# baiyang4/D-LSG-Video-Caption

Hardware: AMD Instinct MI355X
Metric: clips/sec (train step, 26x(2048+4096) feats) (higher is better)
Workload: dtype f32; 1 GPU; vocab 1000, dropout on, tf eps 0.952, batch 64/GPU; MSVD-shaped 26x(2048+4096) + 16x2048 regions; train step; batch_per_gpu=64, global_batch=64, parallelism=dp1, launch=hipGraph replay, gemm_arithmetic=fp32

## Files before the change

d-lsg-video-caption_amd/csrc/rowops.hip:

```cpp
#include <type_traits>

#include "common.hpp"
#include "dlsg.h"
#include "wordpick.hpp"

using namespace dlsg;

namespace {

constexpr int LN_THREADS = 256;
constexpr int LN_MAXPT = 8;

struct RowLnPack { dlsg_rowln_args s[DLSG_ROWLN_MAXMULTI]; };
struct RowLnBwdPack { dlsg_rowln_bwd_args s[DLSG_ROWLN_MAXMULTI]; };

__global__ __launch_bounds__(LN_THREADS) void rowln_fwd_kernel(const RowLnPack pk) {
    __shared__ float red[16];
    const dlsg_rowln_args& a = pk.s[blockIdx.y];
    const int n = a.n;
    const uint64_t seed = a.seed + (a.seed_ptr ? *a.seed_ptr : 0ull);
    float gam[LN_MAXPT], bet[LN_MAXPT];
#pragma unroll
    for (int i = 0; i < LN_MAXPT; ++i) {
        const int j = threadIdx.x + i * LN_THREADS;
// ... 272 lines not shown
    const float* xp = x + o * n * inner + in;
    const float* mp = mask ? mask + o * n * inner + in : nullptr;
    float* yp = y + o * n * inner + in;
    float m = -INFINITY;
    for (int j = lane; j < n; j += 64) {
        float v = xp[(int64_t)j * inner];
        if (mp && !(mp[(int64_t)j * inner] > 0.f)) v = -9e15f;
        m = fmaxf(m, v);
    }
    m = wave_max(m);
    float s = 0.f;
    for (int j = lane; j < n; j += 64) {
        float v = xp[(int64_t)j * inner];
        if (mp && !(mp[(int64_t)j * inner] > 0.f)) v = -9e15f;
        s += __expf(v - m);
    }
    s = wave_sum(s);
    const float inv = 1.f / s;
    for (int j = lane; j < n; j += 64) {
        float v = xp[(int64_t)j * inner];
        if (mp && !(mp[(int64_t)j * inner] > 0.f)) v = -9e15f;
        yp[(int64_t)j * inner] = __expf(v - m) * inv;
    }
}

__global__ __launch_bounds__(256) void softmax_bwd_kernel(const float* __restrict__ y, const float* __restrict__ dy,
                                                          float* __restrict__ dx, int64_t outer, int n, int inner) {
    const int lane = threadIdx.x & 63;
    const int64_t line = (int64_t)blockIdx.x * 4 + (threadIdx.x >> 6);
    if (line >= outer * inner) return;
    const int64_t o = line / inner, in = line % inner;
    const int64_t base = o * n * inner + in;
    float s = 0.f;
    for (int j = lane; j < n; j += 64) s += y[base + (int64_t)j * inner] * dy[base + (int64_t)j * inner];
    s = wave_sum(s);
    for (int j = lane; j < n; j += 64) {
        const int64_t k = base + (int64_t)j * inner;
        dx[k] = y[k] * (dy[k] - s);
    }
}

struct PwFwdSet { dlsg_lstm_pw_args a[2]; };
struct PwBwdSet { dlsg_lstm_pw_bwd_args a[2]; };

__global__ __launch_bounds__(256) void lstm_pw_fwd_kernel(const PwFwdSet set) {
    const dlsg_lstm_pw_args& a = set.a[blockIdx.z];
    const int j = blockIdx.x * blockDim.x + threadIdx.x;
    const int b = blockIdx.y;
    if (j >= a.H) return;
    const int H = a.H;
    float pre[4] = {0.f, 0.f, 0.f, 0.f};
    const float* sp = a.slabs + (int64_t)b * 4 * H + j;
    int k = 0;
    for (; k + 2 <= a.nslab; k += 2) {
        float t[2][4];
#pragma unroll
        for (int u = 0; u < 2; ++u)
#pragma unroll
            for (int g = 0; g < 4; ++g) t[u][g] = sp[(k + u) * a.slab_stride + g * H];
#pragma unroll
        for (int u = 0; u < 2; ++u)
#pragma unroll
            for (int g = 0; g < 4; ++g) pre[g] += t[u][g];
    }
    if (k < a.nslab) {
#pragma unroll
        for (int g = 0; g < 4; ++g) pre[g] += sp[k * a.slab_stride + g * H];
    }
#pragma unroll
    for (int g = 0; g < 4; ++g) {
        const int col = g * H + j;
        float s = pre[g];
        if (a.addend) s += a.addend[(int64_t)b * a.ldadd + col];
        if (a.b_ih) s += a.b_ih[col];
        if (a.b_hh) s += a.b_hh[col];
        pre[g] = s;
    }
    const float ig = sigmoidf_(pre[0]), fg = sigmoidf_(pre[1]), gg = tanhf(pre[2]), og = sigmoidf_(pre[3]);
    const float cp = a.c_prev ? a.c_prev[(int64_t)b * a.ldcp + j] : 0.f;
    const float c = fg * cp + ig * gg;
    const float h = og * tanhf(c);
    a.c[(int64_t)b * a.ldc_ + j] = c;
    if (a.h) a.h[(int64_t)b * a.ldh + j] = h;
    if (a.h2) {
        float h2 = h;
        if (a.p > 0.f) h2 *= drop_scale(a.seed + (a.seed_ptr ? *a.seed_ptr : 0ull), a.site, (uint64_t)b * H + j, a.p);
        a.h2[(int64_t)b * a.ldh2 + j] = h2;
    }
    if (a.gates) {
        float* gp = a.gates + (int64_t)b * a.ldg;
        gp[j] = ig; gp[H + j] = fg; gp[2 * H + j] = gg; gp[3 * H + j] = og;
    }
}

__global__ __launch_bounds__(256) void lstm_pw_bwd_kernel(const PwBwdSet set) {
    const dlsg_lstm_pw_bwd_args& a = set.a[blockIdx.z];
    const int j = blockIdx.x * blockDim.x + threadIdx.x;
    const int b = blockIdx.y;
    if (j >= a.H) return;
    const int H = a.H;
    const float* gp = a.gates + (int64_t)b * a.ldg;
    const float ig = gp[j], fg = gp[H + j], gg = gp[2 * H + j], og = gp[3 * H + j];
    const float c = a.c[(int64_t)b * a.ldc_ + j];
    const float cp = a.c_prev ? a.c_prev[(int64_t)b * a.ldcp + j] : 0.f;
    float dh = a.dh ? a.dh[(int64_t)b * a.lddh + j] : 0.f;
    if (a.dh2 || a.dh3 || a.dh4) {
        float d2 = a.dh2 ? a.dh2[(int64_t)b * a.lddh2 + j] : 0.f;
        if (a.dh3) d2 += a.dh3[(int64_t)b * a.lddh3 + j];
        if (a.dh4) {
            const int ns4 = a.dh4_nslab > 1 ? a.dh4_nslab : 1;
            const float* hp = a.dh4 + (int64_t)b * a.lddh4 + j;
            int k = 0;
            for (; k + 4 <= ns4; k += 4) {
                const float t0 = hp[(int64_t)k * a.dh4_slab_stride], t1 = hp[(int64_t)(k + 1) * a.dh4_slab_stride],
                            t2 = hp[(int64_t)(k + 2) * a.dh4_slab_stride], t3 = hp[(int64_t)(k + 3) * a.dh4_slab_stride];
                d2 += t0; d2 += t1; d2 += t2; d2 += t3;
            }
            for (; k < ns4; ++k) d2 += hp[(int64_t)k * a.dh4_slab_stride];
        }
        if (a.p > 0.f) d2 *= drop_scale(a.seed + (a.seed_ptr ? *a.seed_ptr : 0ull), a.site, (uint64_t)b * H + j, a.p);
        dh += d2;
    }
    const float tc = tanhf(c);
    float dc = dh * og * (1.f - tc * tc);
    if (a.dc_next) dc += a.dc_next[(int64_t)b * a.lddcn + j];
    float* dgp = a.dgates + (int64_t)b * a.lddg;
    dgp[j] = dc * gg * ig * (1.f - ig);
    dgp[H + j] = dc * cp * fg * (1.f - fg);
    dgp[2 * H + j] = dc * ig * (1.f - gg * gg);
    dgp[3 * H + j] = dh * tc * og * (1.f - og);
    if (a.dc_prev) a.dc_prev[(int64_t)b * a.lddcp + j] = dc * fg;
}

__global__ void mean_rows_fwd_kernel(const float* __restrict__ x, float* __restrict__ out, int64_t ldo, int P, int H) {
    const int b = blockIdx.y;
    const int h = blockIdx.x * blockDim.x + threadIdx.x;
    if (h >= H) return;
    float s = 0.f;
    for (int p = 0; p < P; ++p) s += x[((int64_t)b * P + p) * H + h];
    out[(int64_t)b * ldo + h] = s / P;
}
__global__ void mean_rows_bwd_kernel(const float* __restrict__ dout, int64_t lddo, float* __restrict__ dx, int P, int H,
                                     int accum) {
    const int b = blockIdx.y;
    const int h = blockIdx.x * blockDim.x + threadIdx.x;
    if (h >= H) return;
    const float g = dout[(int64_t)b * lddo + h] / P;
    for (int p = 0; p < P; ++p) {
        float* d = dx + ((int64_t)b * P + p) * H + h;
        *d = accum ? *d + g : g;
    }
}

template <bool VEC>
__global__ __launch_bounds__(256) void rows_repeat_kernel(const float* __restrict__ x, float* __restrict__ y, int n, int64_t row,
                                                          int pieces) {
    const int64_t b = blockIdx.x / pieces;
    const int piece = blockIdx.x - (int)b * pieces;
    if constexpr (VEC) {
        const int64_t row4 = row >> 2;
        const int64_t j = (int64_t)piece * 256 + threadIdx.x;
        if (j >= row4) return;
        const f32x4 v = reinterpret_cast<const f32x4*>(x + b * row)[j];
        for (int i = 0; i < n; ++i) reinterpret_cast<f32x4*>(y + (b * n + i) * row)[j] = v;
    } else {
        const int64_t j = (int64_t)piece * 256 + threadIdx.x;
        if (j >= row) return;
        const float v = x[b * row + j];
        for (int i = 0; i < n; ++i) y[(b * n + i) * row + j] = v;
    }
}

template <bool VEC>
__global__ __launch_bounds__(256) void clip_fold_kernel(const float* __restrict__ dmem, const float* __restrict__ dg, int64_t lddg,
                                                        float* __restrict__ dx, int64_t total, int n, int P, int H, int accum) {
    constexpr int W = VEC ? 4 : 1;
    typedef typename std::conditional<VEC, f32x4, float>::type vec_t;
    const int64_t e = ((int64_t)blockIdx.x * 256 + threadIdx.x) * W;
    if (e >= total) return;
    const int64_t PH = (int64_t)P * H;
    const int64_t b = e / PH, ph = e - b * PH;
    const int h = (int)(ph % H);
    const float fP = (float)P;
    const float* m = dmem + b * n * PH + ph;
    const float* g = dg ? dg + b * n * lddg + h : nullptr;
    vec_t s;
    for (int i = 0; i < n; ++i) {
        vec_t t = *reinterpret_cast<const vec_t*>(m + i * PH);
        if (g) t += *reinterpret_cast<const vec_t*>(g + i * lddg) / fP;
        s = i ? s + t : t;
    }
    vec_t* d = reinterpret_cast<vec_t*>(dx + e);
    *d = accum ? *d + s : s;
}

__global__ void embed_fwd_kernel(const float* __restrict__ E, const int64_t* __restrict__ ids, float* __restrict__ out,
                                 int64_t ldo, int W, float p, uint64_t seed, uint32_t site, int64_t row0, const uint64_t* seed_ptr) {
    if (seed_ptr) seed += *seed_ptr;
    const int r = blockIdx.x;
    embed_row(E, ids[r], out, ldo, W, r, p, seed, site, row0, blockDim.x);
}
__global__ __launch_bounds__(1024) void embed_bwd_kernel(const float* __restrict__ dout, int64_t lddo, const int64_t* __restrict__ ids,
                                                         float* __restrict__ dE, int rows, int W, float p, uint64_t seed, uint32_t site,
                                                         int64_t row0, const uint64_t* seed_ptr) {
    if (seed_ptr) seed += *seed_ptr;
    const int r = blockIdx.x, lane = threadIdx.x & 63, wv = threadIdx.x >> 6, nwv = blockDim.x >> 6;
    const int64_t id = ids[r];
    for (int base = 0; base < r; base += 512) {
        int64_t v[8];
#pragma unroll
        for (int u = 0; u < 8; ++u) {
            const int i = base + 64 * u + lane;
            v[u] = (i < r) ? ids[i] : -1;
        }
        bool hit = false;
#pragma unroll
        for (int u = 0; u < 8; ++u) hit = hit || (v[u] == id);
        if (__ballot(hit)) return;
    }
    for (int c0 = 64 * wv; c0 < W; c0 += 64 * nwv) {
        const int j = c0 + lane;
        float acc = 0.f;
        for (int base = r; base < rows; base += 512) {
            int64_t v[8];
#pragma unroll
            for (int u = 0; u < 8; ++u) {
                const int i = base + 64 * u + lane;
                v[u] = (i < rows) ? ids[i] : -1;
            }
#pragma unroll
            for (int u = 0; u < 8; ++u) {
                unsigned long long m = __ballot(v[u] == id);
                while (m) {
                    int rr[8];
#pragma unroll
                    for (int x = 0; x < 8; ++x) {
                        rr[x] = m ? base + 64 * u + (__ffsll((long long)m) - 1) : -1;
                        m &= m - 1;
                    }
                    float g[8];
#pragma unroll
                    for (int x = 0; x < 8; ++x) g[x] = (rr[x] >= 0 && j < W) ? dout[(int64_t)rr[x] * lddo + j] : 0.f;
#pragma unroll
                    for (int x = 0; x < 8; ++x)
                        if (rr[x] >= 0 && j < W) {
                            float gv = g[x];
                            if (p > 0.f) gv *= drop_scale(seed, site, (uint64_t)(row0 + rr[x]) * W + j, p);
                            acc += gv;
                        }
                }
            }
        }
        if (j < W) dE[id * W + j] += acc;
    }
}

__global__ void copy2d_kernel(const float* __restrict__ src, int64_t lds_, float* __restrict__ dst, int64_t ldd, int rows,
                              int n, int accum) {
    const int64_t total = (int64_t)rows * n;
    for (int64_t i = (int64_t)blockIdx.x * blockDim.x + threadIdx.x; i < total; i += (int64_t)gridDim.x * blockDim.x) {
        const int64_t r = i / n;
        const int j = (int)(i - r * n);
        const float v = src[r * lds_ + j];
        float* d = dst + r * ldd + j;
        *d = accum ? *d + v : v;
    }
}
__global__ void dropout_kernel(const float* __restrict__ x, int64_t ldx, float* __restrict__ y, int64_t ldy, int rows, int n,
                               float p, uint64_t seed, uint32_t site, const uint64_t* seed_ptr) {
    if (seed_ptr) seed += *seed_ptr;
    const int64_t total = (int64_t)rows * n;
    for (int64_t i = (int64_t)blockIdx.x * blockDim.x + threadIdx.x; i < total; i += (int64_t)gridDim.x * blockDim.x) {
        const int64_t r = i / n;
        const int j = (int)(i - r * n);
        y[r * ldy + j] = x[r * ldx + j] * drop_scale(seed, site, (uint64_t)i, p);
    }
}
__global__ void permute_tb_kernel(const float* __restrict__ src, float* __restrict__ dst, int T, int B, int n) {
    const int64_t total = (int64_t)T * B * n;
    for (int64_t i = (int64_t)blockIdx.x * blockDim.x + threadIdx.x; i < total; i += (int64_t)gridDim.x * blockDim.x) {
        const int j = (int)(i % n);
        const int64_t rb = i / n;
        const int t = (int)(rb % T), b = (int)(rb / T);
        dst[i] = src[((int64_t)t * B + b) * n + j];
    }
}
template <bool VEC>
__global__ __launch_bounds__(256) void gather_rows_kernel(const float* __restrict__ src, int64_t lds_, const int64_t* __restrict__ idx,
                                                          float* __restrict__ dst, int64_t ldd, int n) {
    const int pieces = (n + 4095) >> 12;
    const int r = blockIdx.x / pieces, piece = blockIdx.x - r * pieces;
    const float* s = src + idx[r] * lds_;
    float* d = dst + (int64_t)r * ldd;
    if constexpr (VEC) {
        const int n4 = n >> 2;
        const int base = piece * 1024 + threadIdx.x;
        typedef float f4 __attribute__((ext_vector_type(4)));
        f4 v[4];
#pragma unroll
        for (int u = 0; u < 4; ++u)
            if (base + u * 256 < n4) v[u] = __builtin_nontemporal_load(reinterpret_cast<const f4*>(s) + base + u * 256);
#pragma unroll
        for (int u = 0; u < 4; ++u)
            if (base + u * 256 < n4) reinterpret_cast<f4*>(d)[base + u * 256] = v[u];
    } else {
        const int hi = min(n, (piece + 1) * 4096);
        for (int j = piece * 4096 + threadIdx.x; j < hi; j += 256) d[j] = s[j];
    }
}
__global__ void fill_kernel(float* __restrict__ dst, int64_t n, float v) {
    for (int64_t i = (int64_t)blockIdx.x * blockDim.x + threadIdx.x; i < n; i += (int64_t)gridDim.x * blockDim.x) dst[i] = v;
}

template <bool WEIGHTED>
__global__ __launch_bounds__(256) void ce_ragged_kernel(const float* __restrict__ logits, const int64_t* __restrict__ targets,
                                                        const int64_t* __restrict__ lens, const float* __restrict__ weights,
                                                        float* __restrict__ dlogits, float* __restrict__ row_loss, int B, int L,
                                                        int V, int tm) {
    __shared__ float red[16];
    const int row = blockIdx.x;
    const int b = tm ? row % B : row / L, t = tm ? row / B : row % L;
    const float* x = logits + (int64_t)row * V;
    float* dx = dlogits + (int64_t)row * V;
    int64_t len = lens[b];
    if (len > L) len = L;
    if (t >= len) {
        for (int j = threadIdx.x; j < V; j += blockDim.x) dx[j] = 0.f;
        if (threadIdx.x == 0) row_loss[row] = 0.f;
        return;
    }
    int64_t ntot = 0;
    for (int i = 0; i < B; ++i) ntot += (lens[i] > L ? L : lens[i]);
    float m = -INFINITY;
    for (int j = threadIdx.x; j < V; j += blockDim.x) m = fmaxf(m, x[j]);
    m = block_max(m, red);
    float s = 0.f;
    for (int j = threadIdx.x; j < V; j += blockDim.x) s += __expf(x[j] - m);
    s = block_sum(s, red);
    const int64_t tgt = targets[(int64_t)b * L + t];
    const bool bad = tgt < 0 || tgt >= V;
    const float inv = bad ? NAN : 1.f / s;
    float invn = 1.f / (float)ntot;
    if constexpr (WEIGHTED) invn = weights[b] * invn;
    for (int j = threadIdx.x; j < V; j += blockDim.x) {
        float p = __expf(x[j] - m) * inv;
        if (j == tgt) p -= 1.f;
        dx[j] = p * invn;
    }
    if (threadIdx.x == 0) row_loss[row] = bad ? NAN : (logf(s) + m - x[tgt]) * invn;
}
__global__ __launch_bounds__(256) void sum_to_scalar_kernel(const float* __restrict__ v, int n, float* __restrict__ out) {
    __shared__ float red[16];
    float s = 0.f;
    for (int i = threadIdx.x; i < n; i += blockDim.x) s += v[i];
    s = block_sum(s, red);
    if (threadIdx.x == 0) out[0] = s;
}

__global__ __launch_bounds__(256) void log_softmax_kernel(const float* __restrict__ logits, float* __restrict__ out, int V) {
    __shared__ float red[16];
    const float* x = logits + (int64_t)blockIdx.x * V;
    float* y = out + (int64_t)blockIdx.x * V;
    float m = -INFINITY;
    for (int j = threadIdx.x; j < V; j += blockDim.x) m = fmaxf(m, x[j]);
    m = block_max(m, red);
    float s = 0.f;
    for (int j = threadIdx.x; j < V; j += blockDim.x) s += expf(x[j] - m);
    s = block_sum(s, red);
    const float lse = logf(s) + m;
    for (int j = threadIdx.x; j < V; j += blockDim.x) y[j] = x[j] - lse;
}

__global__ void gather_rows_multi_kernel(const dlsg_gather_multi_args a) {
    const int i = blockIdx.y, r = blockIdx.x;
    const int n = a.n[i];
    const float* s = a.src[i] + a.rows[r] * (int64_t)n;
    float* d = a.dst[i] + (int64_t)r * n;
    if ((n & 3) == 0) {
        for (int j = threadIdx.x * 4; j < n; j += blockDim.x * 4)
            *reinterpret_cast<f32x4*>(d + j) = *reinterpret_cast<const f32x4*>(s + j);
    } else {
        for (int j = threadIdx.x; j < n; j += blockDim.x) d[j] = s[j];
    }
}

template <bool CLIP>
__device__ __forceinline__ void adam_one(float& p, float g, float& m, float& v, float lr_bc1, float b1, float b2, float eps,
                                         float bc2s, float gscale, float coef, float clipv) {
    float gi = g * gscale;
    if (CLIP) {
        gi *= coef;
        if (clipv > 0.f) gi = fminf(fmaxf(gi, -clipv), clipv);
    }
    m = b1 * m + (1.f - b1) * gi;
    v = b2 * v + (1.f - b2) * gi * gi;
    const float denom = sqrtf(v) / bc2s + eps;
    p -= lr_bc1 * (m / denom);
}
template <int NTM, bool CLIP>
__global__ __launch_bounds__(256) void adam_kernel(float* __restrict__ p, const float* __restrict__ g, float* __restrict__ m,
                                                   float* __restrict__ v, int64_t n, float lr, float b1, float b2, float eps,
                                                   float bc1, float bc2s, float gscale, const float* __restrict__ hyper,
                                                   const int32_t* __restrict__ guard, const float* __restrict__ record, float clipv) {
    if (guard && *guard != 0) return;
    float coef = 1.f;
    if (CLIP && record) {
        if (record[DLSG_CLIP_NONFINITE] != 0.f) return;
        coef = record[DLSG_CLIP_COEF];
    }
    if (hyper) { lr = hyper[0]; bc1 = 1.f; bc2s = hyper[1]; }
    const float lr_bc1 = lr / bc1;
    const int64_t tid = (int64_t)blockIdx.x * blockDim.x + threadIdx.x, nth = (int64_t)gridDim.x * blockDim.x;
    const bool same = ((reinterpret_cast<uintptr_t>(p) ^ reinterpret_cast<uintptr_t>(g)) & 15) == 0 &&
                      ((reinterpret_cast<uintptr_t>(p) ^ reinterpret_cast<uintptr_t>(m)) & 15) == 0 &&
                      ((reinterpret_cast<uintptr_t>(p) ^ reinterpret_cast<uintptr_t>(v)) & 15) == 0;
    int64_t head = same ? (int64_t)((16 - (reinterpret_cast<uintptr_t>(p) & 15)) & 15) / 4 : n;
    if (head > n) head = n;
    const int64_t nv = (n - head) / 4;
    for (int64_t i = tid; i < head; i += nth) adam_one<CLIP>(p[i], g[i], m[i], v[i], lr_bc1, b1, b2, eps, bc2s, gscale, coef, clipv);
    f32x4* p4 = reinterpret_cast<f32x4*>(p + head);
    const f32x4* g4 = reinterpret_cast<const f32x4*>(g + head);
    f32x4* m4 = reinterpret_cast<f32x4*>(m + head);
    f32x4* v4 = reinterpret_cast<f32x4*>(v + head);
    for (int64_t i = tid; i < nv; i += nth) {
        f32x4 pp, mm, vv, gg;
        if (NTM & 4) pp = __builtin_nontemporal_load(p4 + i); else pp = p4[i];
        if (NTM & 1) { mm = __builtin_nontemporal_load(m4 + i); vv = __builtin_nontemporal_load(v4 + i); gg = __builtin_nontemporal_load(g4 + i); }
        else { mm = m4[i]; vv = v4[i]; gg = g4[i]; }
#pragma unroll
        for (int e = 0; e < 4; ++e) {
            float pe = pp[e], me = mm[e], ve = vv[e];
            adam_one<CLIP>(pe, gg[e], me, ve, lr_bc1, b1, b2, eps, bc2s, gscale, coef, clipv);
            pp[e] = pe; mm[e] = me; vv[e] = ve;
        }
        if (NTM & 2) { __builtin_nontemporal_store(mm, m4 + i); __builtin_nontemporal_store(vv, v4 + i); }
        else { m4[i] = mm; v4[i] = vv; }
        if (NTM & 8) __builtin_nontemporal_store(pp, p4 + i); else p4[i] = pp;
    }
    for (int64_t i = head + 4 * nv + tid; i < n; i += nth) adam_one<CLIP>(p[i], g[i], m[i], v[i], lr_bc1, b1, b2, eps, bc2s, gscale, coef, clipv);
}

__global__ __launch_bounds__(256) void grad_sumsq_kernel(const float* __restrict__ g, int64_t n, double* __restrict__ slots) {
    __shared__ double red[4];
    const int64_t tid = (int64_t)blockIdx.x * blockDim.x + threadIdx.x, nth = (int64_t)gridDim.x * blockDim.x;
    int64_t head = (int64_t)((16 - (reinterpret_cast<uintptr_t>(g) & 15)) & 15) / 4;
    if (head > n) head = n;
    const int64_t nv = (n - head) / 4;
    double a0 = 0.0, a1 = 0.0, a2 = 0.0, a3 = 0.0;
    for (int64_t i = tid; i < head; i += nth) { const double x = g[i]; a0 += x * x; }
    const f32x4* g4 = reinterpret_cast<const f32x4*>(g + head);
#pragma unroll 4
    for (int64_t i = tid; i < nv; i += nth) {
        const f32x4 gg = g4[i];
        const double x0 = gg[0], x1 = gg[1], x2 = gg[2], x3 = gg[3];
        a0 += x0 * x0; a1 += x1 * x1; a2 += x2 * x2; a3 += x3 * x3;
    }
    for (int64_t i = head + 4 * nv + tid; i < n; i += nth) { const double x = g[i]; a0 += x * x; }
    const double s = block256_sum_f64((a0 + a1) + (a2 + a3), red);
    if (threadIdx.x == 0) slots[blockIdx.x] = s;
}
__global__ __launch_bounds__(256) void clip_coef_kernel(const double* __restrict__ slots, int count, float gscale, float max_norm,
                                                       float* __restrict__ record, int64_t* __restrict__ skipped) {
    __shared__ double red[4];
    double a = 0.0;
// ... 28 lines not shown
    }
    if (a->rows == 0) return DLSG_OK;
    int grid = a->rows < 4096 ? a->rows : 4096;
    hipLaunchKernelGGL(rowln_fwd_kernel, dim3(grid, count), dim3(LN_THREADS), 0, ST(stream), pk);
    DLSG_CHECK_LAUNCH();
    return DLSG_OK;
}
extern "C" int dlsg_rowln_fwd(const dlsg_rowln_args* a, void* stream) { return dlsg_rowln_fwd_multi(a, 1, stream); }
extern "C" int dlsg_rowln_bwd_nblk(int rows) {
    if (rows < 1) return 1;
    if (rows <= 256) return rows;
    if (rows <= 4096) return (rows + 1) / 2 < 1024 ? (rows + 1) / 2 : 1024;
    return 1024;
}
extern "C" int dlsg_rowln_bwd_multi(const dlsg_rowln_bwd_args* a, int count, void* stream) {
    if (!a || count < 1 || count > DLSG_ROWLN_MAXMULTI) return DLSG_EINVAL;
    const int grid = dlsg_rowln_bwd_nblk(a->f.rows);
    RowLnBwdPack pk;
    for (int i = 0; i < count; ++i) {
        if (a[i].f.n < 1 || a[i].f.n > LN_THREADS * LN_MAXPT || a[i].f.rows != a[0].f.rows) return DLSG_EINVAL;
        if (a[i].dgb_part && a[i].nblk != grid) return DLSG_EINVAL;
        pk.s[i] = a[i];
    }
    if (a->f.rows == 0) return DLSG_OK;
    hipLaunchKernelGGL(rowln_bwd_kernel, dim3(grid, count), dim3(LN_THREADS), 0, ST(stream), pk);
    DLSG_CHECK_LAUNCH();
    return DLSG_OK;
}
extern "C" int dlsg_rowln_bwd(const dlsg_rowln_bwd_args* a, void* stream) { return dlsg_rowln_bwd_multi(a, 1, stream); }
static int colsum_chunks(int rows) {
    if (rows < 4096) return 1;
    const int chunks = (rows + 1023) / 1024;
    return chunks > 32 ? 32 : chunks;
}
static int colsum_launch(const float* part, int64_t ld, int rows, int n, float* out, float* out2, int split, int mode, int accum,
                         float* ws, void* stream) {
    if (!part || !out || n < 1) return DLSG_EINVAL;
    const int chunks = colsum_chunks(rows);
    const int rpc = (rows + chunks - 1) / chunks;
    const bool v4 = n % 4 == 0 && ld % 4 == 0 && (reinterpret_cast<uintptr_t>(part) & 15) == 0;
    if (chunks > 1 && ws && (v4 || !out2)) {
        if (v4) hipLaunchKernelGGL(colsum_v4_kernel, dim3((n + 63) / 64, chunks), dim3(1024), 0, ST(stream), part, ld, rows, n, out,
                                   out2, out2 ? split : n, out2 ? mode : 0, accum, rpc, ws);
        else hipLaunchKernelGGL(colsum_kernel, dim3((n + 63) / 64, chunks), dim3(1024), 0, ST(stream), part, ld, rows, n, out, accum,
                                rpc, ws);
        hipLaunchKernelGGL(colsum_finish_kernel, dim3((n + 255) / 256), dim3(256), 0, ST(stream), ws, chunks, n, out, out2,
                           out2 ? split : n, out2 ? mode : 0, accum);
        DLSG_CHECK_LAUNCH();
        return DLSG_OK;
    }
    if (chunks > 1 && !accum) {
        const int n0 = (out2 && mode == 0) ? split : n;
        hipLaunchKernelGGL(fill_kernel, dim3(1), dim3(256), 0, ST(stream), out, (int64_t)n0, 0.f);
        if (out2) hipLaunchKernelGGL(fill_kernel, dim3(1), dim3(256), 0, ST(stream), out2, (int64_t)(mode == 0 ? n - split : n), 0.f);
    }
    float* none = nullptr;
    if (v4) {
        hipLaunchKernelGGL(colsum_v4_kernel, dim3((n + 63) / 64, chunks), dim3(1024), 0, ST(stream), part, ld, rows, n, out,
                           out2, out2 ? split : n, out2 ? mode : 0, accum, rpc, none);
    } else if (!out2) {
        hipLaunchKernelGGL(colsum_kernel, dim3((n + 63) / 64, chunks), dim3(1024), 0, ST(stream), part, ld, rows, n, out, accum, rpc, none);
    } else if (mode == 0) {
        hipLaunchKernelGGL(colsum_kernel, dim3((split + 63) / 64, chunks), dim3(1024), 0, ST(stream), part, ld, rows, split, out,
                           accum, rpc, none);
        hipLaunchKernelGGL(colsum_kernel, dim3((n - split + 63) / 64, chunks), dim3(1024), 0, ST(stream), part + split, ld, rows,
                           n - split, out2, accum, rpc, none);
    } else {
        hipLaunchKernelGGL(colsum_kernel, dim3((n + 63) / 64, chunks), dim3(1024), 0, ST(stream), part, ld, rows, n, out, accum, rpc, none);
        hipLaunchKernelGGL(colsum_kernel, dim3((n + 63) / 64, chunks), dim3(1024), 0, ST(stream), part, ld, rows, n, out2, accum, rpc, none);
    }
    DLSG_CHECK_LAUNCH();
    return DLSG_OK;
}
extern "C" int dlsg_colsum_multi_ok(const float* part, int64_t ld, int rows, int n) {
    return (colsum_chunks(rows) == 1 && n % 4 == 0 && ld % 4 == 0 && (reinterpret_cast<uintptr_t>(part) & 15) == 0) ? 1 : 0;
}
extern "C" int dlsg_colsum_multi(const dlsg_colsum_desc* d, int count, void* stream) {
    if (!d || count < 1 || count > DLSG_COLSUM_MAXMULTI) return DLSG_EINVAL;
    ColsumPack pk;
    int maxn = 0;
    for (int i = 0; i < count; ++i) {
        if (!d[i].part || !d[i].out_a || d[i].n < 1 || d[i].rows < 0) return DLSG_EINVAL;
        if (!dlsg_colsum_multi_ok(d[i].part, d[i].ld, d[i].rows, d[i].n)) return DLSG_EALIGN;
        if (d[i].out_b && !d[i].dup && (d[i].split < 0 || d[i].split > d[i].n)) return DLSG_EINVAL;
        pk.d[i] = d[i];
        maxn = d[i].n > maxn ? d[i].n : maxn;
    }
    hipLaunchKernelGGL(colsum_multi_kernel, dim3((maxn + 63) / 64, count), dim3(1024), 0, ST(stream), pk);
    DLSG_CHECK_LAUNCH();
    return DLSG_OK;
}
extern "C" int64_t dlsg_colsum_ws_floats(int rows, int n) {
    const int chunks = colsum_chunks(rows);
    return chunks > 1 ? (int64_t)chunks * n : 0;
}
extern "C" int dlsg_colsum(const float* part, int64_t ld, int rows, int n, float* out, int accum, float* ws, void* stream) {
    return colsum_launch(part, ld, rows, n, out, nullptr, n, 0, accum, ws, stream);
}
extern "C" int dlsg_colsum2(const float* part, int64_t ld, int rows, int n, float* out_a, float* out_b, int split, int dup,
                            int accum, float* ws, void* stream) {
    if (!out_b || (!dup && (split < 0 || split > n))) return DLSG_EINVAL;
    return colsum_launch(part, ld, rows, n, out_a, out_b, dup ? n : split, dup ? 1 : 0, accum, ws, stream);
}
extern "C" int dlsg_softmax_fwd(const float* x, const float* mask, float* y, int64_t outer, int n, int inner, void* stream) {
    const int64_t lines = outer * inner;
    if (lines == 0) return DLSG_OK;
    hipLaunchKernelGGL(softmax_fwd_kernel, dim3((unsigned)((lines + 3) / 4)), dim3(256), 0, ST(stream), x, mask, y, outer, n,
                       inner);
    DLSG_CHECK_LAUNCH();
    return DLSG_OK;
}
extern "C" int dlsg_softmax_bwd(const float* y, const float* dy, float* dx, int64_t outer, int n, int inner, void* stream) {
    const int64_t lines = outer * inner;
    if (lines == 0) return DLSG_OK;
    hipLaunchKernelGGL(softmax_bwd_kernel, dim3((unsigned)((lines + 3) / 4)), dim3(256), 0, ST(stream), y, dy, dx, outer, n,
                       inner);
    DLSG_CHECK_LAUNCH();
    return DLSG_OK;
}
extern "C" int dlsg_lstm_pw_fwd_n(const dlsg_lstm_pw_args* a, int count, void* stream) {
    if (!a || count < 1 || count > 2 || a[0].H < 1) return DLSG_EINVAL;
    if (count == 2 && (a[1].H != a[0].H || a[1].B != a[0].B)) return DLSG_EINVAL;
    if (a[0].B == 0) return DLSG_OK;
    PwFwdSet set;
    for (int i = 0; i < 2; ++i) set.a[i] = a[i < count ? i : 0];
    hipLaunchKernelGGL(lstm_pw_fwd_kernel, dim3((a[0].H + 255) / 256, a[0].B, count), dim3(256), 0, ST(stream), set);
    DLSG_CHECK_LAUNCH();
    return DLSG_OK;
}
extern "C" int dlsg_lstm_pw_fwd(const dlsg_lstm_pw_args* a, void* stream) { return dlsg_lstm_pw_fwd_n(a, 1, stream); }
extern "C" int dlsg_lstm_pw_bwd_n(const dlsg_lstm_pw_bwd_args* a, int count, void* stream) {
    if (!a || count < 1 || count > 2 || a[0].H < 1) return DLSG_EINVAL;
    if (count == 2 && (a[1].H != a[0].H || a[1].B != a[0].B)) return DLSG_EINVAL;
    if (a[0].B == 0) return DLSG_OK;
    PwBwdSet set;
    for (int i = 0; i < 2; ++i) set.a[i] = a[i < count ? i : 0];
    hipLaunchKernelGGL(lstm_pw_bwd_kernel, dim3((a[0].H + 255) / 256, a[0].B, count), dim3(256), 0, ST(stream), set);
    DLSG_CHECK_LAUNCH();
    return DLSG_OK;
}
extern "C" int dlsg_lstm_pw_bwd(const dlsg_lstm_pw_bwd_args* a, void* stream) { return dlsg_lstm_pw_bwd_n(a, 1, stream); }
extern "C" int dlsg_mean_rows_fwd(const float* x, float* out, int64_t ldo, int B, int P, int H, void* stream) {
    if (B == 0) return DLSG_OK;
    hipLaunchKernelGGL(mean_rows_fwd_kernel, dim3((H + 255) / 256, B), dim3(256), 0, ST(stream), x, out, ldo, P, H);
    DLSG_CHECK_LAUNCH();
    return DLSG_OK;
}
extern "C" int dlsg_mean_rows_bwd(const float* dout, int64_t lddo, float* dx, int B, int P, int H, int accum, void* stream) {
    if (B == 0) return DLSG_OK;
    hipLaunchKernelGGL(mean_rows_bwd_kernel, dim3((H + 255) / 256, B), dim3(256), 0, ST(stream), dout, lddo, dx, P, H, accum);
    DLSG_CHECK_LAUNCH();
    return DLSG_OK;
}
extern "C" int dlsg_rows_repeat(const float* x, float* y, int B, int n, int64_t row, void* stream) {
    if (B < 0 || n < 1 || row < 0) return DLSG_EINVAL;
    if (B == 0 || row == 0) return DLSG_OK;
    if (!x || !y) return DLSG_EINVAL;
    const bool vec = row % 4 == 0 && ((uintptr_t)x | (uintptr_t)y) % 16 == 0;
    const int64_t pieces = ((vec ? row >> 2 : row) + 255) / 256;
    if (pieces * B > 0x7fffffff) return DLSG_EINVAL;
    const dim3 grid((unsigned)(pieces * B));
    if (vec) hipLaunchKernelGGL(rows_repeat_kernel<true>, grid, dim3(256), 0, ST(stream), x, y, n, row, (int)pieces);
    else hipLaunchKernelGGL(rows_repeat_kernel<false>, grid, dim3(256), 0, ST(stream), x, y, n, row, (int)pieces);
    DLSG_CHECK_LAUNCH();
    return DLSG_OK;
}
extern "C" int dlsg_clip_fold(const float* dmem, const float* dg, int64_t lddg, float* dx, int B, int n, int P, int H, int accum,
                              void* stream) {
    if (B < 0 || n < 1 || P < 1 || H < 1 || (dg && lddg < H)) return DLSG_EINVAL;
    if (B == 0) return DLSG_OK;
    if (!dmem || !dx) return DLSG_EINVAL;
    const int64_t total = (int64_t)B * P * H;
    const bool vec = H % 4 == 0 && ((uintptr_t)dmem | (uintptr_t)dx) % 16 == 0 && (!dg || (lddg % 4 == 0 && (uintptr_t)dg % 16 == 0));
    const int64_t blocks = ((vec ? total >> 2 : total) + 255) / 256;
    if (blocks > 0x7fffffff) return DLSG_EINVAL;
    if (vec) hipLaunchKernelGGL(clip_fold_kernel<true>, dim3((unsigned)blocks), dim3(256), 0, ST(stream), dmem, dg, lddg, dx, total, n, P, H, accum);
    else hipLaunchKernelGGL(clip_fold_kernel<false>, dim3((unsigned)blocks), dim3(256), 0, ST(stream), dmem, dg, lddg, dx, total, n, P, H, accum);
    DLSG_CHECK_LAUNCH();
    return DLSG_OK;
}
extern "C" int dlsg_embed_fwd(const float* E, const int64_t* ids, float* out, int64_t ldo, int rows, int W, float p,
                              uint64_t seed, uint32_t site, int64_t row0, const uint64_t* seed_ptr, void* stream) {
    if (rows == 0) return DLSG_OK;
    hipLaunchKernelGGL(embed_fwd_kernel, dim3(rows), dim3(128), 0, ST(stream), E, ids, out, ldo, W, p, seed, site, row0, seed_ptr);
    DLSG_CHECK_LAUNCH();
    return DLSG_OK;
}
extern "C" int dlsg_embed_bwd(const float* dout, int64_t lddo, const int64_t* ids, float* dE, int rows, int W, float p,
                              uint64_t seed, uint32_t site, int64_t row0, const uint64_t* seed_ptr, void* stream) {
    if (rows == 0) return DLSG_OK;
    const int threads = W >= 1024 ? 1024 : (W + 63) / 64 * 64;
    hipLaunchKernelGGL(embed_bwd_kernel, dim3(rows), dim3(threads), 0, ST(stream), dout, lddo, ids, dE, rows, W, p, seed, site, row0,
                       seed_ptr);
    DLSG_CHECK_LAUNCH();
    return DLSG_OK;
}
extern "C" int dlsg_copy2d(const float* src, int64_t lds_, float* dst, int64_t ldd, int rows, int n, int accum, void* stream) {
    if ((int64_t)rows * n == 0) return DLSG_OK;
    hipLaunchKernelGGL(copy2d_kernel, dim3(grid_for((int64_t)rows * n)), dim3(256), 0, ST(stream), src, lds_, dst, ldd, rows, n,
                       accum);
    DLSG_CHECK_LAUNCH();
    return DLSG_OK;
}
extern "C" int dlsg_dropout(const float* x, int64_t ldx, float* y, int64_t ldy, int rows, int n, float p, uint64_t seed,
                            uint32_t site, const uint64_t* seed_ptr, void* stream) {
    if ((int64_t)rows * n == 0) return DLSG_OK;
    hipLaunchKernelGGL(dropout_kernel, dim3(grid_for((int64_t)rows * n)), dim3(256), 0, ST(stream), x, ldx, y, ldy, rows, n, p,
                       seed, site, seed_ptr);
    DLSG_CHECK_LAUNCH();
    return DLSG_OK;
}
extern "C" int dlsg_gather_rows(const float* src, int64_t lds_, const int64_t* idx, float* dst, int64_t ldd, int rows, int n,
                                void* stream) {
    if (rows == 0 || n == 0) return DLSG_OK;
    const bool vec = n % 4 == 0 && lds_ % 4 == 0 && ldd % 4 == 0 && ((uintptr_t)src | (uintptr_t)dst) % 16 == 0;
    const dim3 grid((unsigned)((int64_t)((n + 4095) / 4096) * rows));
    if (vec) hipLaunchKernelGGL(gather_rows_kernel<true>, grid, dim3(256), 0, ST(stream), src, lds_, idx, dst, ldd, n);
    else hipLaunchKernelGGL(gather_rows_kernel<false>, grid, dim3(256), 0, ST(stream), src, lds_, idx, dst, ldd, n);
    DLSG_CHECK_LAUNCH();
    return DLSG_OK;
}
extern "C" int dlsg_fill(float* dst, int64_t n, float value, void* stream) {
    if (n == 0) return DLSG_OK;
    hipLaunchKernelGGL(fill_kernel, dim3(grid_for(n)), dim3(256), 0, ST(stream), dst, n, value);
    DLSG_CHECK_LAUNCH();
    return DLSG_OK;
}
extern "C" int dlsg_permute_tb(const float* src, float* dst, int T, int B, int n, void* stream) {
    const int64_t total = (int64_t)T * B * n;
    if (total == 0) return DLSG_OK;
    hipLaunchKernelGGL(permute_tb_kernel, dim3(grid_for(total)), dim3(256), 0, ST(stream), src, dst, T, B, n);
    DLSG_CHECK_LAUNCH();
    return DLSG_OK;
}
extern "C" int dlsg_ce_ragged(const float* logits, const int64_t* targets, const int64_t* lens, float* dlogits, float* row_loss,
                              float* loss, int B, int L, int V, int time_major, void* stream) {
    if (B * L == 0) return DLSG_OK;
    hipLaunchKernelGGL(ce_ragged_kernel<false>, dim3(B * L), dim3(256), 0, ST(stream), logits, targets, lens, nullptr, dlogits, row_loss,
                       B, L, V, time_major);
    hipLaunchKernelGGL(sum_to_scalar_kernel, dim3(1), dim3(256), 0, ST(stream), row_loss, B * L, loss);
    DLSG_CHECK_LAUNCH();
    return DLSG_OK;
}
extern "C" int dlsg_ce_ragged_weighted(const float* logits, const int64_t* targets, const int64_t* lens, const float* weights,
                                       float* dlogits, float* row_loss, float* loss, int B, int L, int V, int time_major, void* stream) {
    if (B * L == 0) return DLSG_OK;
    if (!weights) return DLSG_EINVAL;
    hipLaunchKernelGGL(ce_ragged_kernel<true>, dim3(B * L), dim3(256), 0, ST(stream), logits, targets, lens, weights, dlogits, row_loss,
                       B, L, V, time_major);
    hipLaunchKernelGGL(sum_to_scalar_kernel, dim3(1), dim3(256), 0, ST(stream), row_loss, B * L, loss);
    DLSG_CHECK_LAUNCH();
    return DLSG_OK;
}
extern "C" int dlsg_log_softmax(const float* logits, float* out, int rows, int V, void* stream) {
    if (rows == 0) return DLSG_OK;
    hipLaunchKernelGGL(log_softmax_kernel, dim3(rows), dim3(256), 0, ST(stream), logits, out, V);
    DLSG_CHECK_LAUNCH();
    return DLSG_OK;
}
extern "C" int dlsg_gather_rows_multi(const dlsg_gather_multi_args* a, void* stream) {
    if (!a || a->count < 1 || a->count > 4) return DLSG_EINVAL;
    if (a->nrows == 0) return DLSG_OK;
    hipLaunchKernelGGL(gather_rows_multi_kernel, dim3(a->nrows, a->count), dim3(256), 0, ST(stream), *a);
    DLSG_CHECK_LAUNCH();
    return DLSG_OK;
}
extern "C" int dlsg_adam(float* p, const float* g, float* m, float* v, int64_t n, float lr, float b1, float b2, float eps,
                         int step, float grad_scale, const float* hyper, const int32_t* guard, void* stream) {
    if (n == 0) return DLSG_OK;
    const float bc1 = 1.f - powf(b1, (float)step);
    const float bc2s = sqrtf(1.f - powf(b2, (float)step));
    hipLaunchKernelGGL((adam_kernel<3, false>), dim3(grid_for((n + 3) / 4, 256, 8192)), dim3(256), 0, ST(stream), p, g, m, v, n, lr, b1, b2,
                       eps, bc1, bc2s, grad_scale, hyper, guard, (const float*)nullptr, 0.f);
    DLSG_CHECK_LAUNCH();
    return DLSG_OK;
}
extern "C" int dlsg_grad_sumsq(const float* g, int64_t n, double* slots, void* stream) {
    if (n < 0 || (!g && n > 0) || !slots) return DLSG_EINVAL;
    if (reinterpret_cast<uintptr_t>(g) & 3) return DLSG_EALIGN;
    hipLaunchKernelGGL(grad_sumsq_kernel, dim3(DLSG_GRAD_SUMSQ_SLOTS), dim3(256), 0, ST(stream), g, n, slots);
    DLSG_CHECK_LAUNCH();
    return DLSG_OK;
}
extern "C" int dlsg_clip_coef(const double* slots, int count, float grad_scale, float max_norm, float* record, int64_t* skipped,
                              void* stream) {
    if (!slots || count < 1 || !record || !(max_norm >= 0.f)) return DLSG_EINVAL;
    hipLaunchKernelGGL(clip_coef_kernel, dim3(1), dim3(256), 0, ST(stream), slots, count, grad_scale, max_norm, record, skipped);
    DLSG_CHECK_LAUNCH();
    return DLSG_OK;
}
extern "C" int dlsg_adam_clipped(float* p, const float* g, float* m, float* v, int64_t n, float lr, float b1, float b2, float eps,
                                 int step, float grad_scale, const float* hyper, const int32_t* guard, const float* record,
                                 float clip_value, void* stream) {
    if (!(clip_value >= 0.f)) return DLSG_EINVAL;
    if (n == 0) return DLSG_OK;
    const float bc1 = 1.f - powf(b1, (float)step);
    const float bc2s = sqrtf(1.f - powf(b2, (float)step));
    hipLaunchKernelGGL((adam_kernel<3, true>), dim3(grid_for((n + 3) / 4, 256, 8192)), dim3(256), 0, ST(stream), p, g, m, v, n, lr, b1, b2,
                       eps, bc1, bc2s, grad_scale, hyper, guard, record, clip_value);
    DLSG_CHECK_LAUNCH();
    return DLSG_OK;
}
```

d-lsg-video-caption_amd/dlsg_amd/engine.py:

```python
import math

import torch

from .hip import GEMM_NT, GEMM_NN, GEMM_TN, F_ACCUM, F_TANH, F_BF16X3, F_FORCE128, SAMPLE_FILTER_MAXV

V_SK = 7

SITE_PSL_OBJ, SITE_PSL_MOT, SITE_LSTM, SITE_PE, SITE_SA, SITE_WORD, SITE_QUERY, SITE_ATT1, SITE_ATT2, SITE_LANG = range(1, 11)
STEP_SITE = 64
SITE_SAMPLE = 11
SAMPLE_FILTER_MAXL = 64


def _empty(ref, *shape, dtype=torch.float32):
    return torch.empty(*shape, dtype=dtype, device=ref.device)


def _zeros(ref, *shape, dtype=torch.float32):
    return torch.zeros(*shape, dtype=dtype, device=ref.device)


def _ksplit_bounds(K, nsplit, align=32):
    nsplit = max(1, min(nsplit, K // 512))
    step = ((K + nsplit - 1) // nsplit + align - 1) // align * align
    out, k = [], 0
    while k < K:
        out.append((k, min(K, k + step)))
        k += step
    return out


SKINNY_M = 128


def _bwd_bounds(K, M, nsplit):
    if M <= SKINNY_M and K >= 2048:
        return [(k, min(K, k + 1024)) for k in range(0, K, 1024)]
    return _ksplit_bounds(K, nsplit, 128 if M <= SKINNY_M else 32)


def _nsplit_for(M, N, nseg, target=384, cap=16):
    tiles = (1 if M <= SKINNY_M else (M + 63) // 64) * ((N + 63) // 64)
    n = max(1, target // max(1, tiles * nseg))
    return max(1, min(n, cap // max(1, nseg)))


def seg_gemm_nt(ops, segs, M, N, ref):
    ns = 1 if M <= SKINNY_M else _nsplit_for(M, N, len(segs))
    groups = []
    for x, W in segs:
        for k0, k1 in _ksplit_bounds(x.shape[1], ns, 128 if M <= SKINNY_M else 32):
            groups.append((x[:, k0:k1], W[:, k0:k1]))
    slabs = _empty(ref, len(groups), M, N)
    ops.gemm(GEMM_NT, [(a, b, slabs[i]) for i, (a, b) in enumerate(groups)])
    return slabs


def gemm_nn_split(ops, dy, W, out, ref, accum=False):
    M, Nn = dy.shape
    Kin = W.shape[1]
    ns = _nsplit_for(M, Kin, 1)
    bounds = _ksplit_bounds(Nn, ns, 128 if M <= SKINNY_M else 32)
    if len(bounds) == 1:
        ops.gemm(GEMM_NN, [(dy, W, out)], flags=F_ACCUM if accum else 0)
        return
    slabs = _empty(ref, len(bounds), M, Kin)
    ops.gemm(GEMM_NN, [(dy[:, k0:k1], W[k0:k1, :], slabs[i]) for i, (k0, k1) in enumerate(bounds)])
    ops.slab_reduce(slabs, out, flags=F_ACCUM if accum else 0)


DEEP_TN_CHUNKS = 8


def _accum_flag(ops, gout):
    seen = getattr(ops, 'grad_written', None)
    if seen is None:
        return F_ACCUM
    key = (gout.data_ptr(), tuple(gout.shape), tuple(gout.stride()))
    if key in seen:
        return F_ACCUM
    seen.add(key)
    return 0


def _accum_always(ops, gout):
    seen = getattr(ops, 'grad_written', None)
    if seen is not None:
        seen.add((gout.data_ptr(), tuple(gout.shape), tuple(gout.stride())))
    return F_ACCUM


def gemm_tn_deep(ops, items, ref):
    deep = [it for it in items if it[0].shape[0] >= 8192]
    for dy, x, gout in items:
        if dy.shape[0] < 8192:
            ops.gemm(GEMM_TN, [(dy, x, gout)], flags=_accum_flag(ops, gout))
    if deep and getattr(ops, 'stream_k', False) and all(ops.gemm(GEMM_TN, [it], flags=F_ACCUM, plan_only=True) == V_SK for it in deep):
        parts = {0: [], F_ACCUM: []}
        for it in deep:
            parts[_accum_flag(ops, it[2])].append(it)
        for fl, part in parts.items():
            for i0 in range(0, len(part), 16):
                ops.gemm(GEMM_TN, part[i0:i0 + 16], flags=fl)
        return
    by_shape = {}
    for it in deep:
        by_shape.setdefault((it[0].shape, it[1].shape), []).append(it)
    ks = DEEP_TN_CHUNKS
    per_launch = max(1, min(2, 16 // ks))
    for grp in by_shape.values():
        for i0 in range(0, len(grp), per_launch):
            part = grp[i0:i0 + per_launch]
            rows = part[0][0].shape[0]
            step = ((rows + ks - 1) // ks + 31) // 32 * 32
            bounds = [(k, min(rows, k + step)) for k in range(0, rows, step)]
            assert len(bounds) * len(part) <= 16
            slabs = [_empty(ref, len(bounds), gout.shape[0], gout.shape[1]) for _, _, gout in part]
            ops.gemm(GEMM_TN, [(dy[k0:k1], x[k0:k1], sl[i]) for (dy, x, _), sl in zip(part, slabs)
                               for i, (k0, k1) in enumerate(bounds)])
            for (_, _, gout), sl in zip(part, slabs):
                ops.slab_reduce(sl, gout, flags=_accum_always(ops, gout))


def _accum_flag_peek(ops, gout):
    seen = getattr(ops, 'grad_written', None)
    if seen is None or (gout.data_ptr(), tuple(gout.shape), tuple(gout.stride())) in seen:
        return F_ACCUM
    return 0


def gemm_nn_multi(ops, dy, Ws, out, ref):
    M, Nn = dy.shape
    widths = [W.shape[1] for W in Ws]
    tot = sum(widths)
    assert out.shape[1] == tot
    ns = _nsplit_for(M, tot, 1)
    ns = max(1, min(ns, 16 // len(Ws)))
    bounds = _bwd_bounds(Nn, M, ns)
    slabs = _empty(ref, len(bounds), M, tot)
    groups, c0 = [], 0
    for W, wd in zip(Ws, widths):
        for i, (k0, k1) in enumerate(bounds):
            groups.append((dy[:, k0:k1], W[k0:k1, :], slabs[i][:, c0:c0 + wd]))
        c0 += wd
    ops.gemm(GEMM_NN, groups)
    ops.slab_reduce(slabs, out)


def gemm_nn_multi_slabs(ops, dy, Ws, width, ref):
    M, Nn = dy.shape
    widths = [W.shape[1] for W in Ws]
    tot = sum(widths)
    assert tot <= width
    ns = _nsplit_for(M, tot, 1)
    ns = max(1, min(ns, 16 // len(Ws)))
    bounds = _bwd_bounds(Nn, M, ns)
    if M <= SKINNY_M and len(set(widths)) > 1:
        wmin = min(widths)
        if all(wd % wmin == 0 for wd in widths) and (tot // wmin) * len(bounds) <= 16:
            Ws = [W[:, c:c + wmin] for W, wd in zip(Ws, widths) for c in range(0, wd, wmin)]
            widths = [wmin] * len(Ws)
    slabs = _empty(ref, len(bounds), M, width)
    groups, c0 = [], 0
    for W, wd in zip(Ws, widths):
        for i, (k0, k1) in enumerate(bounds):
            groups.append((dy[:, k0:k1], W[k0:k1, :], slabs[i][:, c0:c0 + wd]))
        c0 += wd
    ops.gemm(GEMM_NN, groups)
    return slabs


def tn_grouped(ops, items, defer=None):
    if defer is not None:
        defer.extend(items)
        return
    by_m = {}
    for dy, x, gout in items:
        by_m.setdefault((dy.shape[1], dy.shape[0]), []).append((dy, x, gout))
    for grp in by_m.values():
        waves, seen = [[]], [set()]
        for it in grp:
            key = (it[2].data_ptr(), tuple(it[2].shape))
            for w_, sn in zip(waves, seen):
                if key not in sn and len(w_) < 16:
                    w_.append(it); sn.add(key)
                    break
            else:
                waves.append([it]); seen.append({key})
        for w_ in waves:
            first = [it for it in w_ if _accum_flag_peek(ops, it[2]) == 0]
            rest = [it for it in w_ if _accum_flag_peek(ops, it[2]) != 0]
            for it in first:
                _accum_flag(ops, it[2])
            if first:
                ops.gemm(GEMM_TN, first, flags=0)
            if rest:
                ops.gemm(GEMM_TN, rest, flags=F_ACCUM)


def gemm_bucketed(ops, mode, groups, flags=0):
    by_m = {}
    for g in groups:
        by_m.setdefault(g[2].shape[-2], []).append(g)
    for grp in by_m.values():
        for i in range(0, len(grp), 16):
            ops.gemm(mode, grp[i:i + 16], flags=flags)


def lin(ops, x, W, out, bias=None, tanh=False, accum=False, skip_if=None):
    ops.gemm(GEMM_NT, [(x, W, out)], flags=(F_TANH if tanh else 0) | (F_ACCUM if accum else 0), bias=bias, skip_if=skip_if)


class Grads(object):

    def __init__(self, named_params, arena, offsets):
        self.arena, self.offsets = arena, offsets
        self.views = {}
        for name, p in named_params:
            o = offsets[name]
            self.views[name] = arena[o:o + p.numel()].view(p.shape)

    def __getitem__(self, name):
        return self.views[name]


def ln_grads(ops, part, G, prefix, n):
    p2 = part.view(-1, 2 * n)
    ops.colsum2(p2, G[prefix + '.weight'], G[prefix + '.bias'], split=n, accum=True)


def region_projections(ops, mods, regions):
    B, T, O, R = regions.shape
    rows = B * T * O
    r2 = regions.view(rows, R)
# ... 424 lines not shown
    so = _empty(ref, B * T, H)
    lin(ops, att, sa.output_layer[0].weight, so)
    psa = sa.dropout if training else 0.0
    if psa > 0:
        ops.dropout(so, so, psa, seed, SITE_SA)
    res = _empty(ref, B * T, H); st_s = _empty(ref, B * T, 2)
    ops.rowln_fwd(so, m.layernorm_sa.weight, m.layernorm_sa.bias, res, st_s)
    s.update(x=x, st_l=st_l, Kp=Kp, Qp=Qp, Vp=Vp, w=w, att=att, so=so, st_s=st_s, scale=scale, psa=psa, pe=pe)
    return res


def _bilstm_steps_bwd(ops, gates, cst, dout3, Whh, dG, B, T, H, ref):
    dcrec = [_empty(ref, B, H), _empty(ref, B, H)]
    ns_r = max(1, min(_nsplit_for(B, 2 * H, 1), 8))
    rb = _bwd_bounds(4 * H, B, ns_r)
    slabs = None
    for step in range(T - 1, -1, -1):
        tt = [step, T - 1 - step]
        tp = [step - 1, T - step]
        last = step == T - 1
        ops.lstm_pw_bwd_multi([dict(gates=gates[d][:, tt[d]], c=cst[d][:, tt[d]], dgates=dG[d][:, tt[d]], B=B, H=H,
                                    c_prev=cst[d][:, tp[d]] if step > 0 else None,
                                    dh=dout3[:, tt[d], d * H:(d + 1) * H],
                                    dh4=None if last else slabs[:, :, d * H:(d + 1) * H],
                                    dc_next=None if last else dcrec[d], dc_prev=dcrec[d]) for d in range(2)])
        if step > 0:
            slabs = _empty(ref, len(rb), B, 2 * H)
            groups = []
            for d in range(2):
                dg = dG[d][:, tt[d]]
                for i, (k0, k1) in enumerate(rb):
                    groups.append((dg[:, k0:k1], Whh[d][k0:k1, :], slabs[i][:, d * H:(d + 1) * H]))
            ops.gemm(GEMM_NN, groups)


def encvis_bwd(ops, m, pfx, frames2d, B, T, sv, G, dres, training, seed):
    H = m.hidden_size
    ref = frames2d
    s = sv[pfx]
    name = pfx
    ln = m.layernorm_lstm
    out2 = s['out']
    D2 = 2 * H
    dout = _empty(ref, B * T, D2)
    if m.baseline:
        tn_grouped(ops, [(dres, s['hl'], G[name + '.out_try.weight'])], sv.get('tn_defer'))
        ops.colsum(dres, G[name + '.out_try.bias'], accum=True)
        dhl = _empty(ref, B * T, D2)
        ops.gemm(GEMM_NN, [(dres, m.out_try.weight, dhl)])
        nb = ops.rowln_bwd_nblk(B * T)
        part = _empty(ref, nb, 2, D2)
        ops.rowln_bwd(dhl, out2, ln.weight, ln.bias, dout, stats=s['st_l'], p1=s['pd'], site1=SITE_LSTM, seed=seed,
                      dgb_part=part)
        ln_grads(ops, part, G, name + '.layernorm_lstm', D2)
    else:
        sa = m.self_attention
        nb = ops.rowln_bwd_nblk(B * T)
        part = _empty(ref, nb, 2, H)
        dso = _empty(ref, B * T, H)
        ops.rowln_bwd(dres, s['so'], m.layernorm_sa.weight, m.layernorm_sa.bias, dso, stats=s['st_s'], dgb_part=part)
        ln_grads(ops, part, G, name + '.layernorm_sa', H)
        if s['psa'] > 0:
            ops.dropout(dso, dso, s['psa'], seed, SITE_SA)
        att, w, Kp, Qp, Vp, x, scale = s['att'], s['w'], s['Kp'], s['Qp'], s['Vp'], s['x'], s['scale']
        tn_grouped(ops, [(dso, att, G[name + '.self_attention.output_layer.0.weight'])], sv.get('tn_defer'))
        datt = _empty(ref, B * T, D2)
        ops.gemm(GEMM_NN, [(dso, sa.output_layer[0].weight, datt)])
        datt3 = datt.view(B, T, D2)
        dK = _empty(ref, B * T, D2); dQ = _empty(ref, B * T, D2); dV = _empty(ref, B * T, D2)
        if ops.sa_core_supported(T, D2):
            ops.sa_core_bwd(w, Kp.view(B, T, D2), Qp.view(B, T, D2), Vp.view(B, T, D2), datt3, dK.view(B, T, D2),
                            dQ.view(B, T, D2), dV.view(B, T, D2), scale)
        else:
            dw = _empty(ref, B, T, T)
            ops.gemm(GEMM_NT, [(datt3, Vp.view(B, T, D2), dw)])
            ops.gemm(GEMM_TN, [(w, datt3, dV.view(B, T, D2))])
            dlg = _empty(ref, B, T, T)
            ops.softmax_bwd(w, dw, dlg, B * T, T, 1)
            ops.gemm(GEMM_NN, [(dlg, Qp.view(B, T, D2), dK.view(B, T, D2))], alpha=scale)
            ops.gemm(GEMM_TN, [(dlg, Kp.view(B, T, D2), dQ.view(B, T, D2))], alpha=scale)
        dx = _empty(ref, B * T, D2)
        sl = _empty(ref, 3, B * T, D2)
        ops.gemm(GEMM_NN, [(dK, sa.K.weight, sl[0]), (dQ, sa.Q.weight, sl[1]), (dV, sa.V.weight, sl[2])])
        ops.slab_reduce(sl, dx)
        tn_grouped(ops, [(dK, x, G[name + '.self_attention.K.weight']), (dQ, x, G[name + '.self_attention.Q.weight']),
                         (dV, x, G[name + '.self_attention.V.weight'])], sv.get('tn_defer'))
        nb = ops.rowln_bwd_nblk(B * T)
        part = _empty(ref, nb, 2, D2)
        ops.rowln_bwd(dx, out2, ln.weight, ln.bias, dout, stats=s['st_l'], pe=s['pe'], p1=s['pd'], site1=SITE_LSTM,
                      p2=0.2 if training else 0.0, site2=SITE_PE, seed=seed, dgb_part=part)
        ln_grads(ops, part, G, name + '.layernorm_lstm', D2)
    lstm = m.lstm
    Wih = [lstm.weight_ih_l0, lstm.weight_ih_l0_reverse]
    Whh = [lstm.weight_hh_l0, lstm.weight_hh_l0_reverse]
    sfx = ['', '_reverse']
    dout3 = dout.view(B, T, D2)
    gates, cst, hprev = s['gates'], s['cst'], s['hprev']
    dG = [_empty(ref, B, T, 4 * H), _empty(ref, B, T, 4 * H)]
    if getattr(ops, 'bilstm_supported', None) is not None and getattr(ops, 'persistent_bilstm_bwd', True) and ops.bilstm_supported(B, T, H):
        ops.bilstm_bwd(gates, cst, dout3, Whh, dG)
    else:
        _bilstm_steps_bwd(ops, gates, cst, dout3, Whh, dG, B, T, H, ref)
    de = _empty(ref, B * T, H)
    e = s['e']
    tn_grouped(ops, [(dG[d].view(B * T, 4 * H), src, G[name + '.lstm.' + wn + sfx[d]])
                     for d in range(2) for src, wn in ((e, 'weight_ih_l0'), (hprev[d].view(B * T, H), 'weight_hh_l0'))],
               sv.get('tn_defer'))
    dgs = [dG[d].view(B * T, 4 * H) for d in range(2)]
    kh = (4 * H) // 2
    if kh % 32 == 0:
        sl = _empty(ref, 4, B * T, H)
        ops.gemm(GEMM_NN, [(dgs[d][:, i * kh:(i + 1) * kh], Wih[d][i * kh:(i + 1) * kh, :], sl[2 * d + i]) for d in range(2) for i in range(2)])
        ops.slab_reduce(sl, de)
    else:
        for d in range(2):
            ops.gemm(GEMM_NN, [(dgs[d], Wih[d], de)], flags=F_ACCUM if d else 0)
    for d in range(2):
        ops.colsum2(dgs[d], G[name + '.lstm.bias_ih_l0' + sfx[d]], G[name + '.lstm.bias_hh_l0' + sfx[d]], accum=True)
    tn_grouped(ops, [(de, frames2d, G[name + '.linear_embed.weight'])], sv.get('tn_defer'))
    ops.colsum(de, G[name + '.linear_embed.bias'], accum=True)


class DecPlan(object):

    def __init__(self, dec, n_global):
        self.H, self.W = dec.visual_hidden_size, dec.word_size
        self.Q, self.D = dec.query_hidden_size, dec.decode_hidden_size
        self.G = n_global
        self.ns = 2 if dec.multi_modal else 1
        self.q_lang = (0, self.D)
        self.q_glob = (self.D, self.D + self.G)
        self.q_word = (self.D + self.G, self.D + self.G + self.W)
        self.l_ctx = [(i * self.H, (i + 1) * self.H) for i in range(self.ns)]
        self.l_q = (self.ns * self.H, self.ns * self.H + self.Q)


def _att_modules(dec):
    return [dec.context_att] + ([dec.context_att_2] if dec.multi_modal else [])


def dec_prepare(ops, dec, mems, sv, training, seed):
    s = sv['dec'] = {}
    gsrc = sv['dec_gsrc']
    ref = mems[0]
    B = ref.shape[0]
    H = dec.visual_hidden_size
    plan = DecPlan(dec, H * len(gsrc))
    Q = plan.Q
    if sv.get('step_feats') is not None:
        gfeat = sv['step_feats']
        assert gfeat.shape == (B, plan.G), (tuple(gfeat.shape), (B, plan.G))
    else:
        gfeat = _empty(ref, B, plan.G)
        for i, g in enumerate(gsrc):
            ops.mean_rows_fwd(g, gfeat[:, i * H:(i + 1) * H])
    Wq = dec.query_lstm.weight_ih
    gq = _empty(ref, B, 4 * Q)
    lin(ops, gfeat, Wq[:, plan.q_glob[0]:plan.q_glob[1]], gq)
    atts = _att_modules(dec)
    m2s = [mem.reshape(mem.shape[0] * mem.shape[1], H) for mem in mems]
    Kc = [_empty(ref, m2.shape[0], H) for m2 in m2s]
    Vc = [_empty(ref, m2.shape[0], H) for m2 in m2s]
    kps = [_empty(ref, m2.shape[0], Q) for m2 in m2s]
    vps = [_empty(ref, m2.shape[0], H) for m2 in m2s]
    gemm_bucketed(ops, GEMM_NT, [g for att, m2, K, V in zip(atts, m2s, Kc, Vc) for g in ((m2, att.K.weight, K), (m2, att.V.weight, V))])
    gemm_bucketed(ops, GEMM_NN, [(K, att.Q.weight, kp) for att, K, kp in zip(atts, Kc, kps)])
    gemm_bucketed(ops, GEMM_NT, [(V, att.output_layer[0].weight, vp) for att, V, vp in zip(atts, Vc, vps)])
    Kp = [kp.view(mem.shape[0], mem.shape[1], Q) for kp, mem in zip(kps, mems)]
    Vp = [vp.view(mem.shape[0], mem.shape[1], H) for vp, mem in zip(vps, mems)]
    s.update(plan=plan, gfeat=gfeat, gq=gq, K=Kc, V=Vc, Kp=Kp, Vp=Vp, mems=mems)
    return s


def dec_step(ops, dec, s, t, ref, training, seed, B, word_dropout=True, sample=None):
    plan = s['plan']
    H, Q, D = plan.H, plan.Q, plan.D
    ql, ll = dec.query_lstm, dec.lang_lstm
    pd = dec.p_drop if training else 0.0
    site = STEP_SITE * (t + 1)
    segs = [(s['WE'][t], ql.weight_ih[:, plan.q_word[0]:plan.q_word[1]])]
    if t > 0 or s.get('warm', False):
        segs += [(s['LHP'][t], ql.weight_ih[:, plan.q_lang[0]:plan.q_lang[1]]), (s['QH'][t], ql.weight_hh)]
    slabs = seg_gemm_nt(ops, segs, B, 4 * Q, ref)
    ns = plan.ns
    lnq = dec.query_lstm_layernorm
    atts = _att_modules(dec)
    ops.dec_mid_fwd(slabs, s['gq'], ql.bias_ih, ql.bias_hh, s['QC'][t], s['QC'][t + 1], s['QH'][t + 1], s['GQ'][t],
                    (lnq.weight, lnq.bias), s['QCUR'][t], s['ST_Q'][t], pd, site + SITE_QUERY, s['Kp'], s['Vp'],
                    [(a.output_layer[2].weight, a.output_layer[2].bias) for a in atts],
                    [s['CPRE'][i][t] for i in range(ns)], [s['CTX'][i][t] for i in range(ns)],
                    [s['ST_C'][i][t] for i in range(ns)], s['ALPHA'][t],
                    [a.dropout if training else 0.0 for a in atts], [site + SITE_ATT1 + i for i in range(ns)],
                    1.0 / math.sqrt(H), seed=seed, **({'kv_div': s['kv_div']} if s.get('kv_div', 1) > 1 else {}))
    segs = [(s['CTX'][i][t], ll.weight_ih[:, plan.l_ctx[i][0]:plan.l_ctx[i][1]]) for i in range(ns)]
    segs.append((s['QCUR'][t], ll.weight_ih[:, plan.l_q[0]:plan.l_q[1]]))
    if t > 0 or s.get('warm', False):
        segs.append((s['LHP'][t], ll.weight_hh))
    slabs = seg_gemm_nt(ops, segs, B, 4 * D, ref)
    lnl = dec.lang_lstm_layernorm
    ops.dec_tail_fwd(slabs, ll.bias_ih, ll.bias_hh, s['LC'][t], s['LC'][t + 1], s['LHP'][t + 1], s['GL'][t],
                     (lnl.weight, lnl.bias), s['DOUT'][t], s['ST_L'][t], pd, site + SITE_LANG, seed=seed,
                     **({'sample': sample} if sample is not None else {}))


def plan_D(s):
    return s['plan'].D


def dec_logits(ops, dec, s, t0, t1, skip_if=None):
    plan = s['plan']
    D = plan.D
    B = s['LHP'].shape[1]
    V = dec.vocab_size
    n = (t1 - t0) * B
    lin(ops, s['DOUT'][t0:t1].view(n, D), dec.word_restore.weight, s['LOGITS'][t0:t1].view(n, V), dec.word_restore.bias,
        skip_if=skip_if)


def dec_alloc(dec, s, ref, B, L):
    plan = s['plan']
    H, W, Q, D, ns = plan.H, plan.W, plan.Q, plan.D, plan.ns
    V = dec.vocab_size
    P = s['Kp'][0].shape[1]
    zst = _zeros(ref, (L + 1) * B * (2 * D + 2 * Q))
    o = 0
    for key, wd in (('LHP', D), ('QH', Q), ('QC', Q), ('LC', D)):
        s[key] = zst[o:o + (L + 1) * B * wd].view(L + 1, B, wd)
        o += (L + 1) * B * wd
    s['WE'] = _empty(ref, L + 1, B, W)
    s['IDS'] = _zeros(ref, L + 1, B, dtype=torch.int64)
    s['QCUR'] = _empty(ref, L, B, Q)
    s['ST_Q'] = _empty(ref, L, B, 2)
    s['CPRE'] = [_empty(ref, L, B, H) for _ in range(ns)]
    s['CTX'] = [_empty(ref, L, B, H) for _ in range(ns)]
    s['ST_C'] = [_empty(ref, L, B, 2) for _ in range(ns)]
    s['GQ'] = _empty(ref, L, B, 4 * Q)
    s['GL'] = _empty(ref, L, B, 4 * D)
    s['ALPHA'] = _empty(ref, L, B, ns * P)
    s['DOUT'] = _empty(ref, L, B, D)
    s['ST_L'] = _empty(ref, L, B, 2)
    s['LOGITS'] = _empty(ref, L, B, V)


def dec_begin(ops, dec, mems, sv, L, training, seed):
    s = dec_prepare(ops, dec, mems, sv, training, seed)
    ref = mems[0]
    B = ref.shape[0]
    dec_alloc(dec, s, ref, B, L)
    s['IDS'][0].fill_(dec.vocab('<start>'))
    s['pw'] = dec.p_drop if training else 0.0
    return s, ref, B, dec.word_embed.weight, s['IDS'], s['pw']


def dec_fwd(ops, dec, mems, sv, captions, L, coins, training, seed, dev_coins=None):
    s, ref, B, E, ids, pw = dec_begin(ops, dec, mems, sv, L, training, seed)
    if dev_coins is not None:
        ops.embed_fwd(E, ids[0], s['WE'][0], p=pw, seed=seed, site=SITE_WORD, row0=0)
        pre = captions is not None and L > 1
        if pre:
            ids[1:L].copy_(captions[:, :L - 1].t())
            ops.embed_fwd(E, ids[1:L].reshape(-1), s['WE'][1:L].view((L - 1) * B, -1), p=pw, seed=seed, site=SITE_WORD, row0=B)
        fused_sample = pre and getattr(ops, 'dec_tail_sample_supported', None) is not None and \
            ops.dec_tail_sample_supported(dec.vocab_size, plan_D(s))
        for t in range(L):
            if fused_sample and t + 1 < L:
                dec_step(ops, dec, s, t, ref, training, seed, B,
                         sample=dict(coins=dev_coins, t=t, W=dec.word_restore.weight, b=dec.word_restore.bias, E=E, ids_out=ids[t + 1],
                                     we_out=s['WE'][t + 1], p=pw, site=SITE_WORD, row0=(t + 1) * B))
                continue
            dec_step(ops, dec, s, t, ref, training, seed, B)
            if t + 1 < L:
                dec_logits(ops, dec, s, t, t + 1, skip_if=dev_coins[t:t + 1])
                ops.select_embed(s['LOGITS'][t], captions, t, dev_coins, E, ids[t + 1], s['WE'][t + 1], p=pw, seed=seed,
                                 site=SITE_WORD, row0=(t + 1) * B, prefilled=pre)
        dec_logits(ops, dec, s, 0, L)
        return s
    if captions is not None:
        tf_steps = [i for i in range(L) if coins[i]]
        for i in tf_steps:
            ids[i + 1].copy_(captions[:, i])
    ops.embed_fwd(E, ids.view(-1), s['WE'].view((L + 1) * B, -1), p=pw, seed=seed, site=SITE_WORD)
    for t in range(L):
        dec_step(ops, dec, s, t, ref, training, seed, B)
        if not coins[t]:
            dec_logits(ops, dec, s, t, t + 1)
            ops.argmax(s['LOGITS'][t], ids[t + 1])
            ops.embed_fwd(E, ids[t + 1], s['WE'][t + 1], p=pw, seed=seed, site=SITE_WORD, row0=(t + 1) * B)
    if any(coins[t] for t in range(L)):
        dec_logits(ops, dec, s, 0, L)
    return s


def check_sample_options(L, top_k=0, top_p=1.0, min_len=0, no_repeat_ngram=0, vocab_size=None):
    if top_k < 0 or int(top_k) != top_k:
        raise ValueError('top_k (%r) must be an integer >= 0 (0: off)' % (top_k,))
    if not 0.0 < top_p <= 1.0:
        raise ValueError('top_p (%r) must be in (0, 1] (1: off)' % (top_p,))
    if not 0 <= min_len <= L:
        raise ValueError('min_len (%r) must be in [0, max_words = %d]' % (min_len, L))
    if no_repeat_ngram < 0:
        raise ValueError('no_repeat_ngram (%r) must not be negative' % (no_repeat_ngram,))
    on = top_k > 0 or top_p < 1.0 or min_len > 0 or no_repeat_ngram > 0
    if on and L > SAMPLE_FILTER_MAXL:
        raise ValueError('filtered sampling keeps at most %d words of history, max_words is %d' % (SAMPLE_FILTER_MAXL, L))
    if on and vocab_size is not None and vocab_size > SAMPLE_FILTER_MAXV:
        raise ValueError('filtered sampling holds a row of logits in LDS: vocabulary %d > %d' % (vocab_size, SAMPLE_FILTER_MAXV))
    return on


def dec_sample(ops, dec, mems, sv, L, training, seed, temperature, top_k=0, top_p=1.0, min_len=0, no_repeat_ngram=0):
    filtered = check_sample_options(L, top_k, top_p, min_len, no_repeat_ngram, dec.vocab_size)
    s, ref, B, E, ids, pw = dec_begin(ops, dec, mems, sv, L, training, seed)
    s['LOGP'] = _empty(ref, L, B)
    s['LENS'] = torch.full((B,), L, dtype=torch.int64, device=ref.device)
    if filtered:
        s['KEPT'] = torch.empty(L, B, dtype=torch.int32, device=ref.device)
    end = dec.vocab('<end>')
    ops.embed_fwd(E, ids[0], s['WE'][0], p=pw, seed=seed, site=SITE_WORD, row0=0)
    for t in range(L):
        dec_step(ops, dec, s, t, ref, training, seed, B)
        dec_logits(ops, dec, s, t, t + 1)
        if filtered:
            ops.sample_filter_embed(s['LOGITS'][t], E, ids[t + 1], s['WE'][t + 1], s['LOGP'][t], s['LENS'], t, end,
                                    temperature=temperature, p=pw, seed=seed, site=SITE_WORD, site_sample=SITE_SAMPLE,
                                    row0=(t + 1) * B, top_k=top_k, top_p=top_p, min_len=min_len, no_repeat_ngram=no_repeat_ngram,
                                    hist=ids[1:], kept=s['KEPT'][t])
            continue
        ops.sample_embed(s['LOGITS'][t], E, ids[t + 1], s['WE'][t + 1], s['LOGP'][t], s['LENS'], t, end, temperature=temperature,
                         p=pw, seed=seed, site=SITE_WORD, site_sample=SITE_SAMPLE, row0=(t + 1) * B)
    return s


def dec_outputs(ops, s, alpha=True):
    def batch_major(x):
        y = _empty(x, x.shape[1], x.shape[0], x.shape[2])
        ops.permute_tb(x, y)
        return y
    return batch_major(s['LOGITS']), batch_major(s['ALPHA']) if alpha else torch.empty(0, device=s['ALPHA'].device)


def dec_bwd(ops, dec, sv, G, dlogits_tm, seed, training, dalpha_tm=None):
    s = sv['dec']
    plan = s['plan']
    H, W, Q, D, ns = plan.H, plan.W, plan.Q, plan.D, plan.ns
    L, B, V = dlogits_tm.shape
    ref = dlogits_tm
    ql, ll = dec.query_lstm, dec.lang_lstm
    pd = dec.p_drop if training else 0.0
    n = L * B
    dl2 = dlogits_tm.view(n, V)
    tn_grouped(ops, [(dl2, s['DOUT'].view(n, D), G['decoder.word_restore.weight'])], sv.get('tn_defer'))
    ops.colsum(dl2, G['decoder.word_restore.bias'], accum=True)
    ddout = _empty(ref, n, D)
    k32 = V // 32 * 32
    if V - k32 and k32 >= 4096 and getattr(ops, 'stream_k', False):
        ops.gemm(GEMM_NN, [(dl2[:, :k32], dec.word_restore.weight[:k32], ddout)])
        ops.gemm(GEMM_NN, [(dl2[:, k32:], dec.word_restore.weight[k32:], ddout)], flags=F_ACCUM)
    else:
        ops.gemm(GEMM_NN, [(dl2, dec.word_restore.weight, ddout)])
    lnl = dec.lang_lstm_layernorm
    nb = ops.rowln_bwd_nblk(n)
    part = _empty(ref, nb, 2, D)
    dLHo = _empty(ref, L, B, D)
    ops.rowln_bwd(ddout, s['LHP'][1:].view(n, D), lnl.weight, lnl.bias, dLHo.view(n, D), stats=s['ST_L'].view(n, 2),
                  post_tanh=1, dgb_part=part)
    ln_grads(ops, part, G, 'decoder.lang_lstm_layernorm', D)

    dGQ = _empty(ref, L, B, 4 * Q)
    dGL = _empty(ref, L, B, 4 * D)
    dQC = _zeros(ref, B, Q)
    dLC = _zeros(ref, B, D)
    dLHrec = _empty(ref, B, D)
    P = s['Kp'][0].shape[1]
    dCPRE = [_empty(ref, L, B, H) for _ in range(ns)]
    dS = _empty(ref, L, B, ns * P)
    atts = _att_modules(dec)
    part_q = _empty(ref, L, B, 2, Q)
    part_c = [_empty(ref, L, B, 2, H) for _ in range(ns)]
    lnq = dec.query_lstm_layernorm
    lnc_g = [att.output_layer[2].weight for att in atts]
    p_att = [att.dropout if training else 0.0 for att in atts]
    scale = 1.0 / math.sqrt(H)
    Wl_in = ll.weight_ih
    Wq_rec = [ql.weight_hh, ql.weight_ih[:, plan.q_lang[0]:plan.q_lang[1]]]
    wx = ns * H + Q + D
    ql_slabs = None
    for t in range(L - 1, -1, -1):
        site = STEP_SITE * (t + 1)
        rec = t < L - 1
        ops.lstm_pw_bwd(s['GL'][t], s['LC'][t + 1], dGL[t], B, D, c_prev=s['LC'][t], dh2=dLHo[t],
                        dh3=dLHrec if rec else None, dh4=ql_slabs[:, :, Q:] if rec else None, dc_next=dLC, dc_prev=dLC,
                        p=pd, site=site + SITE_LANG, seed=seed)
        xl_slabs = gemm_nn_multi_slabs(ops, dGL[t], [Wl_in, ll.weight_hh] if t > 0 else [Wl_in], wx, ref)
        ops.dec_mid_bwd(xl_slabs, dLHrec if t > 0 else None, [s['CPRE'][i][t] for i in range(ns)],
                        [s['ST_C'][i][t] for i in range(ns)], lnc_g, [part_c[i][t] for i in range(ns)],
                        [dCPRE[i][t] for i in range(ns)], p_att, [site + SITE_ATT1 + i for i in range(ns)], s['Kp'], s['Vp'],
                        s['ALPHA'][t], dalpha_tm[t] if dalpha_tm is not None else None, dS[t], s['QH'][t + 1], s['ST_Q'][t],
                        lnq.weight, part_q[t], pd, site + SITE_QUERY, ql_slabs[:, :, :Q] if rec else None, s['GQ'][t],
                        s['QC'][t + 1], s['QC'][t], dQC, dGQ[t], scale, seed=seed)
        if t > 0:
            ql_slabs = gemm_nn_multi_slabs(ops, dGQ[t], Wq_rec, Q + D, ref)
    dKp = [torch.empty_like(k) for k in s['Kp']]
    dVp = [torch.empty_like(v) for v in s['Vp']]
    ops.decatt_cache_grads(s['ALPHA'], dS, s['QCUR'], dCPRE, dKp, dVp)
    ln_grads(ops, part_q.view(L * B, 2, Q), G, 'decoder.query_lstm_layernorm', Q)
    att_names = ['decoder.context_att', 'decoder.context_att_2']
    for i in range(ns):
        ln_grads(ops, part_c[i].view(L * B, 2, H), G, att_names[i] + '.output_layer.2', H)
    dgq2, dgl2 = dGQ.view(n, 4 * Q), dGL.view(n, 4 * D)
    Gq_ih, Gl_ih = G['decoder.query_lstm.weight_ih'], G['decoder.lang_lstm.weight_ih']
    dgq_sum = _empty(ref, B, 4 * Q)
    ops.slab_reduce(dGQ, dgq_sum)
    lhp, qh = s['LHP'][:L].view(n, D), s['QH'][:L].view(n, Q)
    tn_grouped(ops, [(dgq2, lhp, Gq_ih[:, plan.q_lang[0]:plan.q_lang[1]]),
                     (dgq2, s['WE'][:L].view(n, W), Gq_ih[:, plan.q_word[0]:plan.q_word[1]]),
                     (dgq2, qh, G['decoder.query_lstm.weight_hh'])] +
               [(dgl2, s['CTX'][i].view(n, H), Gl_ih[:, plan.l_ctx[i][0]:plan.l_ctx[i][1]]) for i in range(ns)] +
               [(dgl2, s['QCUR'].view(n, Q), Gl_ih[:, plan.l_q[0]:plan.l_q[1]]),
                (dgl2, lhp, G['decoder.lang_lstm.weight_hh'])], sv.get('tn_defer'))
    gq_glob = Gq_ih[:, plan.q_glob[0]:plan.q_glob[1]]
    ops.gemm(GEMM_TN, [(dgq_sum, s['gfeat'], gq_glob)], flags=_accum_always(ops, gq_glob))
    ops.colsum2(dgq2, G['decoder.query_lstm.bias_ih'], G['decoder.query_lstm.bias_hh'], accum=True)
    ops.colsum2(dgl2, G['decoder.lang_lstm.bias_ih'], G['decoder.lang_lstm.bias_hh'], accum=True)
    dWE = _empty(ref, n, W)
    Wword = ql.weight_ih[:, plan.q_word[0]:plan.q_word[1]]
    if n >= 512 and 4 * Q >= 2048:
        kb = [(k, min(4 * Q, k + 1024)) for k in range(0, 4 * Q, 1024)]
        sl = _empty(ref, len(kb), n, W)
        ops.gemm(GEMM_NN, [(dgq2[:, k0:k1], Wword[k0:k1], sl[i]) for i, (k0, k1) in enumerate(kb)])
        ops.slab_reduce(sl, dWE)
    else:
        ops.gemm(GEMM_NN, [(dgq2, Wword, dWE)])
    ops.embed_bwd(dWE, s['IDS'][:L].view(-1), G['decoder.word_embed.weight'], p=s['pw'], seed=seed, site=SITE_WORD)
    dgfeat = _empty(ref, B, plan.G)
    gemm_nn_split(ops, dgq_sum, ql.weight_ih[:, plan.q_glob[0]:plan.q_glob[1]], dgfeat, ref)
    m2s = [mem.reshape(mem.shape[0] * mem.shape[1], H) for mem in s['mems']]
    dkps = [dKp[i].view(m2s[i].shape[0], Q) for i in range(ns)]
    dvps = [dVp[i].view(m2s[i].shape[0], H) for i in range(ns)]
    dKs = [_empty(ref, m2.shape[0], H) for m2 in m2s]
    dVs = [_empty(ref, m2.shape[0], H) for m2 in m2s]
    dms = [_empty(ref, m2.shape[0], H) for m2 in m2s]
    R = range(ns)
    tn_grouped(ops, [g for i in R for g in ((s['K'][i], dkps[i], G[att_names[i] + '.Q.weight']),
                                            (dvps[i], s['V'][i], G[att_names[i] + '.output_layer.0.weight']))], sv.get('tn_defer'))
    gemm_bucketed(ops, GEMM_NT, [(dkps[i], atts[i].Q.weight, dKs[i]) for i in R])
    gemm_bucketed(ops, GEMM_NN, [(dvps[i], atts[i].output_layer[0].weight, dVs[i]) for i in R])
    tn_grouped(ops, [g for i in R for g in ((dKs[i], m2s[i], G[att_names[i] + '.K.weight']),
                                            (dVs[i], m2s[i], G[att_names[i] + '.V.weight']))], sv.get('tn_defer'))
    gemm_bucketed(ops, GEMM_NN, [(dKs[i], atts[i].K.weight, dms[i]) for i in R])
    gemm_bucketed(ops, GEMM_NN, [(dVs[i], atts[i].V.weight, dms[i]) for i in R], flags=F_ACCUM)
    dmems = [dms[i].view(s['mems'][i].shape) for i in R]
    return dmems, dgfeat
```

d-lsg-video-caption_amd/dlsg_amd/hip.py:

```python
import ctypes as C
import math
import os

import torch

from . import abi

_HERE = os.path.dirname(os.path.abspath(__file__))
LIB_PATH = os.path.join(_HERE, 'libdlsg_hip.so')

_D = abi.defines
ABI_VERSION = _D['DLSG_ABI_VERSION']
MAXG = _D['DLSG_GEMM_MAXG']
SAMPLE_FILTER_MAXV = _D['DLSG_SAMPLE_FILTER_MAXV']
GEMM_NT, GEMM_NN, GEMM_TN = _D['DLSG_GEMM_NT'], _D['DLSG_GEMM_NN'], _D['DLSG_GEMM_TN']
F_ACCUM, F_BIAS, F_TANH = _D['DLSG_GEMM_ACCUM'], _D['DLSG_GEMM_BIAS'], _D['DLSG_GEMM_TANH']
F_FORCE64, F_FORCE128, F_TILE256, F_BF16X3 = (_D['DLSG_GEMM_' + n] for n in ('FORCE64', 'FORCE128', 'TILE256', 'BF16X3'))
F_SK, F_NOSK, F_SK_BM128, F_SK_BM256, F_SK_BN128, F_SK_NOXMAP = (_D['DLSG_GEMM_' + n] for n in (
    'SK', 'NOSK', 'SK_BM128', 'SK_BM256', 'SK_BN128', 'SK_NOXMAP'))
GRAD_SUMSQ_SLOTS = _D['DLSG_GRAD_SUMSQ_SLOTS']
CLIP_NORM, CLIP_COEF, CLIP_NONFINITE, CLIP_RECORD_FLOATS = (_D['DLSG_CLIP_' + n] for n in ('NORM', 'COEF', 'NONFINITE', 'RECORD_FLOATS'))
ENS_MAX = _D['DLSG_ENS_MAX']
METRICS_STAGE = _D['DLSG_METRICS_STAGE']
F_SK_GIVEAWAY = _D['DLSG_GEMM_SK_GIVEAWAY']

i64, u32, u64, f32 = C.c_int64, C.c_uint32, C.c_uint64, C.c_float


def load_library(path=LIB_PATH):
    if not os.path.exists(path):
        raise RuntimeError('libdlsg_hip.so not built (%s): run `python -c "import __graft_entry__ as g; g.build()"` '
                           'or `make -C d-lsg-video-caption_amd/csrc`; there is no fallback path' % path)
    lib = C.CDLL(path)
    for name, (restype, argtypes) in abi.functions.items():
        fn = getattr(lib, name)
        fn.restype, fn.argtypes = restype, argtypes
    if lib.dlsg_abi_version() != ABI_VERSION:
        raise RuntimeError('libdlsg_hip.so ABI mismatch: library %d, include/dlsg.h %d (rebuild: make -C d-lsg-video-caption_amd/csrc)'
                           % (lib.dlsg_abi_version(), ABI_VERSION))
    return lib




def _p(t):
    return None if t is None else C.c_void_p(t.data_ptr())


def _chkc(t):
    if not t.is_contiguous():
        raise ValueError('fused decoder-step kernels take dense row-major buffers')


def _seed(seed):
    if torch.is_tensor(seed):
        return 0, C.c_void_p(seed.data_ptr())
    return int(seed), None


def cider_tables(tb):
    def p(t):
        return t.data_ptr() if t.numel() else None
    return abi.dlsg_cider_tables(p(tb.gram_keys), p(tb.gram_idf), p(tb.clip_off), p(tb.ref_off), p(tb.ref_norm), p(tb.ref_len),
                                 p(tb.ent_keys), p(tb.ent_w), tb.gram_keys.numel(), tb.log_n, tb.sigma, tb.n_clips, tb.V, tb.n, 0)


def host_to_device(values, dtype, device):
    t = values.to(dtype) if torch.is_tensor(values) else torch.as_tensor(values, dtype=dtype)
    device = torch.device(device)
    if device.type != 'cuda' or t.is_cuda:
        return t.to(device)
    return t.contiguous().pin_memory().to(device, non_blocking=True)


def copy_to_device(dst, values, dtype=None):
    t = values.to(dtype or dst.dtype) if torch.is_tensor(values) else torch.as_tensor(values, dtype=dtype or dst.dtype)
    if dst.is_cuda and not t.is_cuda:
        t = t.contiguous().pin_memory()
    dst.copy_(t.view(dst.shape), non_blocking=True)


def normalised_weights(weights):
    w = [float(x) for x in weights]
    if not w or not all(math.isfinite(x) and x > 0.0 for x in w):
        raise ValueError('ensemble weights must be finite and positive, not %r' % (list(weights),))
    tot = math.fsum(w)
    return [x / tot for x in w]


def _chk2(t):
    assert t.dim() == 2 and (t.stride(1) == 1 or t.size(1) == 1) and t.dtype == torch.float32, (t.shape, t.stride())
    return t


class HipOps(object):

    name = 'hip'

    def __init__(self):
        self.lib = load_library()
        if not torch.cuda.is_available():
            raise RuntimeError('dlsg_amd needs an MI355X (gfx950) device: torch.cuda.is_available() is False and '
                               'there is no CPU fallback')
        self.prof = None
        self.extra_flags = 0
        self.prof_min_flops = 2e9
        self.flop_count = None
        self._tail_ws = {}

    def _prof_begin(self):
        if self.prof is None:
            return None
        e0 = torch.cuda.Event(enable_timing=True)
        e0.record()
        return e0

    def _prof_end(self, key, e0, work, shape='', operand_bytes=None):
        if e0 is None:
            return
        e1 = torch.cuda.Event(enable_timing=True)
        e1.record()
        self.prof.setdefault(key, []).append((e0, e1, work, shape, operand_bytes))

    def prof_summary(self):
        out = {}
        for key, rec in (self.prof or {}).items():
            shapes, samples = {}, {}
            for a, b, w, shp, ob in rec:
                d = shapes.setdefault(shp, dict(launches=0, ms_total=0.0, work_total=0.0, operand_bytes=ob))
                d['launches'] += 1; d['work_total'] += float(w)
                samples.setdefault(shp, []).append(a.elapsed_time(b))
            for shp, ms in samples.items():
                ms = sorted(ms)
                med = ms[len(ms) // 2] if len(ms) % 2 else 0.5 * (ms[len(ms) // 2 - 1] + ms[len(ms) // 2])
                shapes[shp]['ms_total'] = med * len(ms)
            out[key] = dict(launches=len(rec), ms_total=sum(d['ms_total'] for d in shapes.values()),
                            work_total=float(sum(r[2] for r in rec)), shapes=shapes)
        return out

    @staticmethod
    def _stream():
        return C.c_void_p(torch.cuda.current_stream().cuda_stream)

    launches = 0

    def _check(self, rc, what):
        self.launches += 1
        if rc != 0:
            raise RuntimeError('%s failed with code %d' % (what, rc))

    stream_k = True
    sk_cu_budget = 0

    _gemm_ws = {}
    _capture_streams = {}

    @classmethod
    def capture_stream(cls, dev):
        dev = torch.device(dev)
        idx = dev.index if dev.index is not None else torch.cuda.current_device()
        st = cls._capture_streams.get(idx)
        if st is None:
            st = cls._capture_streams[idx] = torch.cuda.Stream(device=idx)
        return st

    def _gemm_workspace(self, dev):
        key = (dev.index, torch.cuda.current_stream(dev).cuda_stream)
        ws = HipOps._gemm_ws.get(key)
        if ws is None:
            n = int(self.lib.dlsg_gemm_ws_bytes())
            if n <= 0:
                raise RuntimeError('dlsg_gemm_ws_bytes() failed: no device?')
            if torch.cuda.is_current_stream_capturing():
                return None
            ws = HipOps._gemm_ws[key] = torch.zeros((n + 3) // 4, dtype=torch.float32, device=dev)
        return ws

    def device_cus(self):
        n = int(self.lib.dlsg_gemm_ws_bytes())
        return max(0, (n - 16384) // (2 * 256 * 256 * 4))

    def comm_rehearsal(self, view, workgroups, passes):
        self._check(self.lib.dlsg_comm_rehearsal(_p(view), i64(view.numel()), int(workgroups), int(passes), self._stream()),
                    'dlsg_comm_rehearsal')

    def gemm(self, mode, groups, alpha=1.0, flags=0, bias=None, skip_if=None, plan_only=False):
        a = abi.dlsg_gemm_args()
        A0, B0, C0 = groups[0][:3]
        batched = A0.dim() == 3
        if batched:
            nb = C0.size(0)
            a.bsa, a.bsb, a.bsc = A0.stride(0), B0.stride(0), C0.stride(0)
        else:
            nb = 1
            a.bsa = a.bsb = a.bsc = 0
        M = C0.shape[-2]
        N = max(g[2].shape[-1] for g in groups)
        a.mode, a.M, a.N, a.ldc = mode, M, N, C0.stride(-2)
        a.ngroups, a.nbatch, a.alpha = len(groups), nb, alpha
        gbias = any(len(g) > 3 and g[3] is not None for g in groups)
        a.flags = flags | self.extra_flags | (F_BIAS if (bias is not None or gbias) else 0)
        a.bias = _p(bias)
        a.skip_if = _p(skip_if)
        if (self.stream_k or (flags & F_SK)) and not ((flags | self.extra_flags) & F_NOSK):
            ws = self._gemm_workspace(C0.device)
            if ws is not None:
                a.ws, a.ws_bytes = _p(ws), ws.numel() * 4
                a.cu_budget = int(self.sk_cu_budget)
        assert len(groups) <= MAXG
        for i, grp_ in enumerate(groups):
            A, B, Cc = grp_[:3]
            Ng = Cc.shape[-1]
            if mode == GEMM_TN:
                K = A.shape[-2]
                assert A.shape[-1] == M and B.shape[-2] == K and B.shape[-1] == Ng, (A.shape, B.shape, Cc.shape)
            elif mode == GEMM_NN:
                K = A.shape[-1]
                assert A.shape[-2] == M and B.shape[-2] == K and B.shape[-1] == Ng, (A.shape, B.shape, Cc.shape)
            else:
                K = A.shape[-1]
                assert A.shape[-2] == M and B.shape[-1] == K and B.shape[-2] == Ng, (A.shape, B.shape, Cc.shape)
            for t in (A, B, Cc):
                assert t.dtype == torch.float32 and (t.stride(-1) == 1 or t.size(-1) == 1), (t.shape, t.stride())
            assert Cc.shape[-2] == M
            if batched:
                assert (A.stride(0), B.stride(0), Cc.stride(0)) == (a.bsa, a.bsb, a.bsc)
            g = a.g[i]
            g.A, g.B, g.C = _p(A), _p(B), _p(Cc)
            g.lda, g.ldb, g.K, g.N = A.stride(-2), B.stride(-2), K, (Ng if Ng != N else 0)
            g.bias = _p(grp_[3]) if len(grp_) > 3 else None
            g.ldc = Cc.stride(-2) if Cc.stride(-2) != a.ldc else 0
        if plan_only:
            return int(self.lib.dlsg_gemm_variant(C.byref(a)))
        e0 = None
        if self.flop_count is not None:
            self.flop_count += 2.0 * M * nb * sum(grp_[2].shape[-1] * a.g[i].K for i, grp_ in enumerate(groups))
        if self.prof is not None:
            flops = 2.0 * M * nb * sum(grp_[2].shape[-1] * a.g[i].K for i, grp_ in enumerate(groups))
            if flops >= self.prof_min_flops:
                e0 = self._prof_begin()
        self._check(self.lib.dlsg_gemm(C.byref(a), self._stream()), 'dlsg_gemm')
        if e0 is not None:
            x3 = bool(a.flags & F_BF16X3)
            if x3:
                tiles_l = ((M + 127) // 128) * ((N + 127) // 128) * nb * len(groups)
                if a.flags & (F_FORCE64 | F_FORCE128):
                    variant = '64x64' if a.flags & F_FORCE64 else '128x128'
                elif M <= 64 and mode != GEMM_TN and N >= 64:
                    variant = 'skinny_64x32'
                else:
# ... 525 lines not shown

    def bilstm_supported(self, B, T, H):
        return self.persistent_bilstm and bool(self.lib.dlsg_bilstm_supported(B, T, H))

    def bilstm_fwd(self, xg, w_hh, b_ih, b_hh, out, hprev, c, gates):
        B, T, H2 = out.shape
        H = H2 // 2
        a = abi.dlsg_bilstm_args()
        dev = out.device
        hx = torch.empty(int(self.lib.dlsg_bilstm_hx_floats(T, H)), dtype=torch.float32, device=dev)
        flags = torch.empty(int(self.lib.dlsg_bilstm_flag_words(T, H)), dtype=torch.int32, device=dev)
        self._bilstm_err = self._persist_word(dev)
        for d in range(2):
            for t in (xg[d], w_hh[d], hprev[d], c[d], gates[d]):
                _chkc(t) if t is not xg[d] else _chk2(t)
            a.xg[d], a.w_hh[d], a.b_ih[d], a.b_hh[d] = xg[d].data_ptr(), w_hh[d].data_ptr(), b_ih[d].data_ptr(), b_hh[d].data_ptr()
            a.hprev[d], a.c[d], a.gates[d] = hprev[d].data_ptr(), c[d].data_ptr(), gates[d].data_ptr()
        _chkc(out)
        a.ldxg = xg[0].stride(0)
        assert xg[1].stride(0) == a.ldxg
        a.out, a.hx, a.flags, a.err = _p(out), _p(hx), _p(flags), _p(self._bilstm_err)
        a.B, a.T, a.H = B, T, H
        self._check(self.lib.dlsg_bilstm_fwd(C.byref(a), self._stream()), 'dlsg_bilstm_fwd')
        return self._bilstm_err

    def bilstm_bwd(self, gates, c, dout, w_hh, dgates):
        B, T, H2 = dout.shape
        H = H2 // 2
        a = abi.dlsg_bilstm_bwd_args()
        dev = dout.device
        nx = int(self.lib.dlsg_bilstm_bwd_x_floats(T, H))
        gx = torch.empty(nx, dtype=torch.float32, device=dev)
        px = torch.empty(nx, dtype=torch.float32, device=dev)
        flags = torch.empty(2 * int(self.lib.dlsg_bilstm_flag_words(T, H)), dtype=torch.int32, device=dev)
        self._bilstm_err = self._persist_word(dev)
        _chkc(dout)
        for d in range(2):
            for t in (gates[d], c[d], w_hh[d], dgates[d]):
                _chkc(t)
            a.gates[d], a.c[d], a.w_hh[d], a.dgates[d] = gates[d].data_ptr(), c[d].data_ptr(), w_hh[d].data_ptr(), dgates[d].data_ptr()
        a.dout, a.gx, a.px, a.flags, a.err = _p(dout), _p(gx), _p(px), _p(flags), _p(self._bilstm_err)
        a.B, a.T, a.H = B, T, H
        self._check(self.lib.dlsg_bilstm_bwd(C.byref(a), self._stream()), 'dlsg_bilstm_bwd')
        return self._bilstm_err

    def lstm_seq_supported(self, L, n, H):
        return bool(self.lib.dlsg_lstm_seq_supported(L, min(n, 256), H))

    def _lstm_seq(self, level, W, b_ih=None, b_hh=None, **t):
        ref = next(v for v in t.values() if v is not None)
        n, L = ref.shape[0], ref.shape[1]
        H = W.shape[1]
        dev = W.device
        chunk = next((c for c in (256, 192, 128, 64) if self.lib.dlsg_lstm_seq_supported(L, min(n, c), H)), 0)
        if not chunk:
            raise RuntimeError('dlsg_lstm_seq does not take L = %d, H = %d on this device (H in {64, 512}, >= H / 8 compute units '
                               'per 64 sequences)' % (L, H))
        self._lstm_seq_err = self._persist_word(dev)
        _chkc(W)
        for name, v in t.items():
            if v is not None:
                _chkc(v)
                assert v.dtype == torch.float32 and v.shape[:2] == (n, L) and v.shape[2] in (H, 4 * H), (name, v.shape)
        for lo in range(0, n, chunk):
            hi = min(n, lo + chunk)
            a = abi.dlsg_lstm_seq_args()
            nx = int(self.lib.dlsg_lstm_seq_x_floats(L, hi - lo, H))
            xbuf = torch.empty(nx, dtype=torch.float32, device=dev)
            xbuf2 = torch.empty(nx, dtype=torch.float32, device=dev) if level == 1 else None
            flags = torch.empty(int(self.lib.dlsg_lstm_seq_flag_words(L, hi - lo, H)), dtype=torch.int32, device=dev)
            for name, v in t.items():
                setattr(a, name, _p(None if v is None else v[lo:hi]))
            a.W, a.xbuf, a.xbuf2, a.flags, a.err = _p(W), _p(xbuf), _p(xbuf2), _p(flags), _p(self._lstm_seq_err)
            a.b_ih, a.b_hh = _p(b_ih), _p(b_hh)
            a.L, a.n, a.H, a.batch_major = L, hi - lo, H, 1
            self._check(self.lib.dlsg_lstm_seq(C.byref(a), level, self._stream()), 'dlsg_lstm_seq(level %d)' % level)
        return self._lstm_seq_err

    def lstm_seq_fwd(self, xin, W, b_ih, b_hh, As, Hs, Cs, Hprev):
        return self._lstm_seq(0, W, b_ih, b_hh, addend=xin, As=As, Hs=Hs, Cs=Cs, Hprev=Hprev)

    def lstm_seq_bwd(self, As, Cs, W, dHs, dAs, dCs, DA, DH, DC):
        return self._lstm_seq(1, W, As=As, Cs=Cs, dHs=dHs, dAs=dAs, dCs=dCs, DA=DA, DH=DH, DC=DC)

    def lstm_seq_bwd2(self, As, Cs, W, DH, DC, ubar, gA, gC, gDH, gDHprev, gDC):
        return self._lstm_seq(2, W, As=As, Cs=Cs, DH=DH, DC=DC, addend=ubar, gA=gA, gC=gC, gDH=gDH, gDC=gDC, gDHprev=gDHprev)

    @staticmethod
    def _pw_fwd_args(a, slabs, c, B, H, addend=None, b_ih=None, b_hh=None, c_prev=None, h=None, h2=None, gates=None,
                     p=0.0, site=0, seed=0):
        if slabs is not None:
            a.slabs, a.nslab, a.slab_stride = _p(slabs), slabs.size(0), slabs.stride(0)
        else:
            a.slabs, a.nslab, a.slab_stride = None, 0, 0
        a.addend, a.ldadd = _p(addend), (addend.stride(0) if addend is not None else 0)
        a.b_ih, a.b_hh = _p(b_ih), _p(b_hh)
        a.c_prev, a.ldcp = _p(c_prev), (c_prev.stride(0) if c_prev is not None else 0)
        a.c, a.ldc_ = _p(c), c.stride(0)
        a.h, a.ldh = _p(h), (h.stride(0) if h is not None else 0)
        a.h2, a.ldh2 = _p(h2), (h2.stride(0) if h2 is not None else 0)
        a.gates, a.ldg = _p(gates), (gates.stride(0) if gates is not None else 0)
        a.B, a.H, a.p, a.site = B, H, p, site
        a.seed, a.seed_ptr = _seed(seed)

    def lstm_pw_fwd(self, slabs, c, B, H, **kw):
        a = abi.dlsg_lstm_pw_args()
        self._pw_fwd_args(a, slabs, c, B, H, **kw)
        self._check(self.lib.dlsg_lstm_pw_fwd(C.byref(a), self._stream()), 'dlsg_lstm_pw_fwd')

    def lstm_pw_fwd_multi(self, calls):
        arr = (abi.dlsg_lstm_pw_args * len(calls))()
        for a, kw in zip(arr, calls):
            self._pw_fwd_args(a, **kw)
        self._check(self.lib.dlsg_lstm_pw_fwd_n(arr, len(calls), self._stream()), 'dlsg_lstm_pw_fwd_n')

    @staticmethod
    def _pw_bwd_args(a, gates, c, dgates, B, H, c_prev=None, dh=None, dh2=None, dc_next=None, dc_prev=None, p=0.0,
                     site=0, seed=0, dh3=None, dh4=None):
        a.gates, a.ldg, a.c, a.ldc_ = _p(gates), gates.stride(0), _p(c), c.stride(0)
        a.c_prev, a.ldcp = _p(c_prev), (c_prev.stride(0) if c_prev is not None else 0)
        a.dh, a.lddh = _p(dh), (dh.stride(0) if dh is not None else 0)
        a.dh2, a.lddh2 = _p(dh2), (dh2.stride(0) if dh2 is not None else 0)
        a.dh3, a.lddh3 = _p(dh3), (dh3.stride(0) if dh3 is not None else 0)
        if dh4 is not None and dh4.dim() == 3:
            a.dh4, a.lddh4, a.dh4_nslab, a.dh4_slab_stride = _p(dh4), dh4.stride(1), dh4.size(0), dh4.stride(0)
        else:
            a.dh4, a.lddh4 = _p(dh4), (dh4.stride(0) if dh4 is not None else 0)
        a.dc_next, a.lddcn = _p(dc_next), (dc_next.stride(0) if dc_next is not None else 0)
        a.dgates, a.lddg = _p(dgates), dgates.stride(0)
        a.dc_prev, a.lddcp = _p(dc_prev), (dc_prev.stride(0) if dc_prev is not None else 0)
        a.B, a.H, a.p, a.site = B, H, p, site
        a.seed, a.seed_ptr = _seed(seed)

    def lstm_pw_bwd(self, gates, c, dgates, B, H, **kw):
        a = abi.dlsg_lstm_pw_bwd_args()
        self._pw_bwd_args(a, gates, c, dgates, B, H, **kw)
        self._check(self.lib.dlsg_lstm_pw_bwd(C.byref(a), self._stream()), 'dlsg_lstm_pw_bwd')

    def lstm_pw_bwd_multi(self, calls):
        arr = (abi.dlsg_lstm_pw_bwd_args * len(calls))()
        for a, kw in zip(arr, calls):
            self._pw_bwd_args(a, **kw)
        self._check(self.lib.dlsg_lstm_pw_bwd_n(arr, len(calls), self._stream()), 'dlsg_lstm_pw_bwd_n')

    def mean_rows_fwd(self, x, out):
        B, P, H = x.shape
        self._check(self.lib.dlsg_mean_rows_fwd(_p(x), _p(out), i64(out.stride(0)), B, P, H, self._stream()), 'mean_rows_fwd')

    def mean_rows_bwd(self, dout, dx, accum=False):
        B, P, H = dx.shape
        self._check(self.lib.dlsg_mean_rows_bwd(_p(dout), i64(dout.stride(0)), _p(dx), B, P, H, int(accum), self._stream()),
                    'mean_rows_bwd')

    def rows_repeat(self, x, y, n):
        B = x.shape[0]
        assert x.is_contiguous() and y.is_contiguous() and y.shape[0] == B * n and y.shape[1:] == x.shape[1:], (x.shape, y.shape, n)
        self._check(self.lib.dlsg_rows_repeat(_p(x), _p(y), B, int(n), i64(x.numel() // max(B, 1)), self._stream()), 'rows_repeat')

    def clip_fold(self, dmem, dg, dx, n, accum=False):
        B, P, H = dx.shape
        assert dmem.is_contiguous() and dx.is_contiguous() and dmem.shape == (B * n, P, H), (dmem.shape, dx.shape, n)
        assert dg is None or (dg.shape == (B * n, H) and dg.stride(1) == 1), (dg.shape, dg.stride())
        self._check(self.lib.dlsg_clip_fold(_p(dmem), _p(dg) if dg is not None else None, i64(dg.stride(0) if dg is not None else 0),
                                            _p(dx), B, int(n), P, H, int(accum), self._stream()), 'clip_fold')

    def embed_fwd(self, E, ids, out, p=0.0, seed=0, site=0, row0=0):
        rows, W = out.shape
        sd, sp = _seed(seed)
        self._check(self.lib.dlsg_embed_fwd(_p(E), _p(ids), _p(out), i64(out.stride(0)), rows, W, f32(p), u64(sd), u32(site),
                                            i64(row0), sp, self._stream()), 'embed_fwd')

    def select_embed(self, logits, captions, t, coins, E, ids_out, out, p=0.0, seed=0, site=0, row0=0, prefilled=False):
        rows, V = logits.shape
        sd, sp = _seed(seed)
        self._check(self.lib.dlsg_select_embed(_p(logits), i64(logits.stride(0)), V, _p(captions), captions.shape[1], int(t),
                                               _p(coins), _p(E), _p(ids_out), _p(out), i64(out.stride(0)), rows, out.shape[1],
                                               f32(p), u64(sd), u32(site), i64(row0), sp, int(bool(prefilled)), self._stream()), 'select_embed')

    def embed_bwd(self, dout, ids, dE, p=0.0, seed=0, site=0, row0=0):
        rows, W = dout.shape
        sd, sp = _seed(seed)
        self._check(self.lib.dlsg_embed_bwd(_p(dout), i64(dout.stride(0)), _p(ids), _p(dE), rows, W, f32(p), u64(sd),
                                            u32(site), i64(row0), sp, self._stream()), 'embed_bwd')

    def argmax(self, logits, ids):
        rows, V = logits.shape
        self._check(self.lib.dlsg_argmax(_p(logits), i64(logits.stride(0)), _p(ids), rows, V, self._stream()), 'argmax')

    def _sample_args(self, logits, E, ids_out, out, logp, lens, t, end_id, temperature, p, seed, site, site_sample, row0):
        rows, V = logits.shape
        assert E.shape[0] >= V and E.is_contiguous() and ids_out.numel() == rows and logp.numel() == rows and lens.numel() == rows
        assert ids_out.dtype == torch.int64 and lens.dtype == torch.int64 and out.shape == (rows, E.shape[1])
        sd, sp = _seed(seed)
        vp = C.c_void_p
        return (vp(logits.data_ptr()), i64(logits.stride(0)), V, f32(temperature), vp(E.data_ptr()), vp(ids_out.data_ptr()),
                vp(out.data_ptr()), i64(out.stride(0)), out.shape[1], vp(logp.data_ptr()), vp(lens.data_ptr()), int(t), i64(end_id),
                rows, f32(p), u64(sd), u32(site), u32(site_sample), i64(row0), sp)

    def sample_embed(self, logits, E, ids_out, out, logp, lens, t, end_id, temperature=1.0, p=0.0, seed=0, site=0, site_sample=0,
                     row0=0):
        args = self._sample_args(logits, E, ids_out, out, logp, lens, t, end_id, temperature, p, seed, site, site_sample, row0)
        self._check(self.lib.dlsg_sample_embed(*args, self._stream()), 'sample_embed')

    def sample_filter_embed(self, logits, E, ids_out, out, logp, lens, t, end_id, temperature=1.0, p=0.0, seed=0, site=0, site_sample=0,
                            row0=0, top_k=0, top_p=1.0, min_len=0, no_repeat_ngram=0, hist=None, kept=None):
        rows, V = logits.shape
        if V > SAMPLE_FILTER_MAXV:
            raise ValueError('sample_filter_embed holds a row of logits in LDS: vocabulary %d > %d' % (V, SAMPLE_FILTER_MAXV))
        args = self._sample_args(logits, E, ids_out, out, logp, lens, t, end_id, temperature, p, seed, site, site_sample, row0)
        assert kept is None or (kept.dtype == torch.int32 and kept.numel() == rows and kept.is_contiguous())
        if no_repeat_ngram > 0 and t > 0:
            assert hist is not None and hist.dtype == torch.int64 and hist.shape[0] >= t and hist.shape[1] == rows and \
                hist.stride(1) == 1, 'hist: the rows\' earlier words, (>= t, rows) int64'
        self._check(self.lib.dlsg_sample_filter_embed(
            *args, int(top_k), f32(top_p), int(min_len), int(no_repeat_ngram), _p(hist) if hist is not None else None,
            i64(hist.stride(0) if hist is not None else 0), _p(kept) if kept is not None else None, self._stream()),
            'sample_filter_embed')

    def copy2d(self, src, dst, accum=False):
        rows, n = src.shape
        self._check(self.lib.dlsg_copy2d(_p(src), i64(src.stride(0)), _p(dst), i64(dst.stride(0)), rows, n, int(accum),
                                         self._stream()), 'copy2d')

    def dropout(self, x, y, p, seed, site):
        rows, n = x.shape
        sd, sp = _seed(seed)
        self._check(self.lib.dlsg_dropout(_p(x), i64(x.stride(0)), _p(y), i64(y.stride(0)), rows, n, f32(p), u64(sd),
                                          u32(site), sp, self._stream()), 'dropout')

    def fill(self, t, value):
        assert t.is_contiguous()
        self._check(self.lib.dlsg_fill(_p(t), i64(t.numel()), f32(value), self._stream()), 'fill')

    def crit_embed_mix(self, proj_tm, ids, W, bias, eps, h):
        ng, B, L, _ = h.shape
        self._check(self.lib.dlsg_crit_embed_mix(_p(proj_tm), _p(ids), _p(W), _p(bias), _p(eps), _p(h), ng, B, L, W.shape[1],
                                                 self._stream()), 'crit_embed_mix')

    def crit_embed_mix_bwd(self, ch, eps, dhr, dhf_tm):
        ng, B, L, _ = ch.shape
        self._check(self.lib.dlsg_crit_embed_mix_bwd(_p(ch), _p(eps), _p(dhr), _p(dhf_tm), ng, B, L, self._stream()), 'crit_embed_mix_bwd')

    def crit_vocab_scatter(self, dhr, ids, dW):
        _chkc(dhr); _chkc(ids); _chkc(dW)
        self._check(self.lib.dlsg_crit_vocab_scatter(_p(dhr), _p(ids), _p(dW), ids.numel(), dW.shape[1], self._stream()), 'crit_vocab_scatter')

    def crit_relu_taps(self, x, ref, bias, bias_scale, y, taps):
        n, L, _ = x.shape
        for t in (x, ref, y, taps):
            _chkc(t)
        self._check(self.lib.dlsg_crit_relu_taps(_p(x), _p(ref), _p(bias), f32(bias_scale), _p(y), _p(taps), n, L, self._stream()),
                    'crit_relu_taps')

    def crit_relu_taps_bwd(self, dy, dtaps, ref, dx):
        n, L, _ = dy.shape
        for t in (dy, dtaps, ref, dx):
            _chkc(t)
        self._check(self.lib.dlsg_crit_relu_taps_bwd(_p(dy), _p(dtaps), _p(ref), _p(dx), n, L, self._stream()), 'crit_relu_taps_bwd')

    def _cln_args(self, x, gamma, pre_tanh, eps, p_pre, site_pre, p_post, site_post, seed, row0):
        a = abi.dlsg_cln_args()
        G = len(x)
        rows, N = x[0].shape
        for g in range(G):
            _chkc(x[g]); _chkc(gamma[g])
            assert x[g].shape == (rows, N) and x[g].dtype == torch.float32
            a.x[g], a.gamma[g] = _p(x[g]), _p(gamma[g])
        a.rows, a.N, a.groups, a.pre_tanh, a.eps = rows, N, G, int(pre_tanh), eps
        a.p_pre, a.site_pre, a.p_post, a.site_post, a.row0 = p_pre, site_pre, p_post, site_post, row0
        a.seed, a.seed_ptr = _seed(seed)
        a.acc_lo = a.acc_hi = 0
        return a

    def _cln_ws(self, a, dev):
        return torch.empty(a.groups * int(self.lib.dlsg_cln_ws_floats(a.rows, a.N)), dtype=torch.float32, device=dev)

    @staticmethod
    def _cln_dys(a, dys):
        a.ndy = len(dys)
        for k, lst in enumerate(dys):
            for g, t in enumerate(lst):
                _chkc(t)
                a.dy[k][g] = _p(t)

    def cln_fwd(self, x, gamma, beta, y, pre_tanh, eps=1e-5, p_pre=0.0, site_pre=0, p_post=0.0, site_post=0, seed=0, row0=0):
        a = self._cln_args(x, gamma, pre_tanh, eps, p_pre, site_pre, p_post, site_post, seed, row0)
        for g in range(len(x)):
            _chkc(y[g])
            a.beta[g], a.y[g] = _p(beta[g]), _p(y[g])
        self._check(self.lib.dlsg_cln_fwd(C.byref(a), self._stream()), 'cln_fwd')

    def cln_ws_rows(self, rows, N):
        return int(self.lib.dlsg_cln_ws_floats(rows, N)) // (2 * N)

    def cln_bwd(self, x, gamma, dys, dx, dgamma, dbeta, pre_tanh, eps=1e-5, p_pre=0.0, site_pre=0, p_post=0.0, site_post=0, seed=0,
                row0=0, acc=None, extra=None, defer_ws=None):
        a = self._cln_args(x, gamma, pre_tanh, eps, p_pre, site_pre, p_post, site_post, seed, row0)
        self._cln_dys(a, dys)
        for g in range(len(x)):
            _chkc(dx[g])
            a.dx[g] = _p(dx[g])
            if dgamma and defer_ws is None:
                a.dgamma[g], a.dbeta[g] = _p(dgamma[g]), _p(dbeta[g])
                if extra is not None:
                    _chkc(extra[g])
                    a.extra[g] = _p(extra[g])
        if acc is not None:
            a.acc_lo, a.acc_hi = acc
        if defer_ws is not None:
            _chkc(defer_ws)
            assert tuple(defer_ws.shape) == (len(x), 2, self.cln_ws_rows(a.rows, a.N), a.N), defer_ws.shape
            ws, a.defer = defer_ws, 1
        else:
            ws = self._cln_ws(a, x[0].device) if dgamma else None
        a.ws = _p(ws)
        self._check(self.lib.dlsg_cln_bwd(C.byref(a), self._stream()), 'cln_bwd')

    def cln_bwd2(self, x, gamma, dys, U, gx, gdy, gpart, pre_tanh, eps=1e-5, p_pre=0.0, site_pre=0, p_post=0.0, site_post=0, seed=0,
                 row0=0, defer_ws=None):
        a = self._cln_args(x, gamma, pre_tanh, eps, p_pre, site_pre, p_post, site_post, seed, row0)
        self._cln_dys(a, dys)
        for g in range(len(x)):
            for t in (U[g], gx[g], gdy[g]):
                _chkc(t)
            a.U[g], a.gx[g], a.gdy[g] = _p(U[g]), _p(gx[g]), _p(gdy[g])
            if defer_ws is None:
                _chkc(gpart[g])
                a.gpart[g] = _p(gpart[g])
        if defer_ws is not None:
            _chkc(defer_ws)
            assert tuple(defer_ws.shape) == (len(x), 2, self.cln_ws_rows(a.rows, a.N), a.N), defer_ws.shape
            ws, a.defer = defer_ws, 1
        else:
            ws = self._cln_ws(a, x[0].device)
        a.ws = _p(ws)
        self._check(self.lib.dlsg_cln_bwd2(C.byref(a), self._stream()), 'cln_bwd2')

    def _sa_args(self, KQV, smask, scale, acc=None):
        a = abi.dlsg_crit_sa_args()
        _chkc(KQV); _chkc(smask)
        a.KQV, a.smask = _p(KQV), _p(smask)
        a.n, a.L, a.B, a.scale = KQV.shape[0], KQV.shape[1], smask.shape[0], scale
        a.acc_lo, a.acc_hi = acc if acc is not None else (0, 0)
        return a

    def crit_sa_fwd(self, KQV, smask, w, ctx, scale):
        a = self._sa_args(KQV, smask, scale)
        _chkc(w); _chkc(ctx)
        a.w, a.ctx = _p(w), _p(ctx)
        self._check(self.lib.dlsg_crit_sa_fwd(C.byref(a), self._stream()), 'crit_sa_fwd')

    def crit_sa_bwd(self, KQV, smask, w, dctx, dKQV, scale, acc=None):
        a = self._sa_args(KQV, smask, scale, acc)
        for t in (w, dctx, dKQV):
            _chkc(t)
        a.w, a.dctx, a.dKQV = _p(w), _p(dctx), _p(dKQV)
        self._check(self.lib.dlsg_crit_sa_bwd(C.byref(a), self._stream()), 'crit_sa_bwd')

    def crit_sa_bwd2(self, KQV, smask, w, dctx, U, Uctx, gKQV, scale):
        a = self._sa_args(KQV, smask, scale)
        for t in (w, dctx, U, Uctx, gKQV):
            _chkc(t)
        a.w, a.dctx, a.U, a.Uctx, a.gKQV = _p(w), _p(dctx), _p(U), _p(Uctx), _p(gKQV)
        self._check(self.lib.dlsg_crit_sa_bwd2(C.byref(a), self._stream()), 'crit_sa_bwd2')

    @staticmethod
    def _set2(st_, **kw):
        for name, pair in kw.items():
            if pair is None:
                continue
            arr = getattr(st_, name)
            for h in range(2):
                _chkc(pair[h])
                arr[h] = _p(pair[h])

    def _pattn_args(self, a_, e, smask, scale, acc=None):
        a = abi.dlsg_crit_pattn_args()
        self._set2(a, a=a_, e=e)
        _chkc(smask)
        a.smask = _p(smask)
        a.n, a.L, a.B, a.T, a.scale = a_[0].shape[0], a_[0].shape[1], smask.shape[0], e[0].shape[1], scale
        a.acc_lo, a.acc_hi = acc if acc is not None else (0, 0)
        return a

    def crit_pattn_fwd(self, a_, e, smask, P, wgt, aggpre, scale):
# ... 266 lines not shown
```

d-lsg-video-caption_amd/dlsg_amd/model.py:

```python
import math
import os
import random

import torch
import torch.nn as nn

from . import abi
from . import engine as E
from .graphs import capture_segments, stage, expand_rows, GreedyGraph, SampleGraph, BeamGraph, NBestBeamGraph
from .modules import CapGnnEncoder, Decoder, EncoderVisual

_ALIGN = 64


def _default_ops():
    from .hip import HipOps
    return HipOps()


class _ArenaModule(nn.Module):

    def __init__(self):
        super().__init__()
        self._ops_obj = None
        self._flat = None
        self._gflat = None
        self._offsets = None

    def __getstate__(self):
        st = dict(self.__dict__)
        st['_ops_obj'] = None
        if 'rng' in st:
            st['rng'] = None
        for k in ('_flat', '_gflat', '_offsets', '_G'):
            st[k] = None
        return st

    def __setstate__(self, st):
        self.__dict__.update(st)
        if 'rng' in st:
            self.rng = random

    @property
    def ops(self):
        if self._ops_obj is None:
            self._ops_obj = _default_ops()
        return self._ops_obj

    def set_ops(self, ops):
        self._ops_obj = ops
        return self

    def _arena_ok(self):
        if self._flat is None:
            return False
        for name, p in self.named_parameters():
            o = self._offsets[name]
            if p.device != self._flat.device or p.data_ptr() != self._flat.data_ptr() + 4 * o:
                return False
        return True

    def flatten_parameters_(self):
        dec = getattr(self, 'decoder', None)
        if dec is not None and getattr(dec, '_owner', None) is None:
            import weakref
            object.__setattr__(dec, '_owner', weakref.ref(self))
        if self._arena_ok():
            return
        named = list(self.named_parameters())
        dev = named[0][1].device
        offsets, tot = {}, 0
        for name, p in named:
            offsets[name] = tot
            tot += (p.numel() + _ALIGN - 1) // _ALIGN * _ALIGN
        flat = torch.zeros(tot, dtype=torch.float32, device=dev)
        for name, p in named:
            view = flat[offsets[name]:offsets[name] + p.numel()].view(p.shape)
            view.copy_(p.data)
            p.data = view
        self._flat, self._offsets = flat, offsets
        self._gflat = torch.zeros(tot, dtype=torch.float32, device=dev)
        self._G = E.Grads(named, self._gflat, offsets)

    def grad_views(self):
        return self._G


class _HipModel(_ArenaModule):

    def __init__(self):
        super().__init__()
        self.rng = random
        self.seed_counter = 0
        self.fused_o2v = True
        self.gemm_precision = 'fp32'

    def __setattr__(self, name, value):
        super().__setattr__(name, value)
        if name == 'decoder' and isinstance(value, nn.Module):
            import weakref
            object.__setattr__(value, '_owner', weakref.ref(self))

    @staticmethod
    def check_kernel_limits(args, attended_rows, what):
        for k in ('query_hidden_size', 'decode_hidden_size', 'visual_hidden_size'):
            if getattr(args, k) > 2048:
                raise ValueError('%s = %d: the fused decoder step supports widths up to 2048' % (k, getattr(args, k)))
        if attended_rows > 72:
            raise ValueError('%s = %d: the fused decoder step attends over at most 72 rows per stream' % (what, attended_rows))

    stream_k_in_backward = True
    sk_backward_cu_budget = 0

    def _gemm_flags(self, backward):
        from .hip import F_BF16X3, F_NOSK
        mode = self.gemm_precision
        assert mode in ('fp32', 'x3_bwd', 'x3_all'), mode
        fl = F_BF16X3 if (mode == 'x3_all' or (mode == 'x3_bwd' and backward)) else 0
        if backward and not self.stream_k_in_backward:
            fl |= F_NOSK
        return fl

    def _gemm_policy(self, backward):
        ops = self.ops
        ops.extra_flags = self._gemm_flags(backward)
        ops.sk_cu_budget = self.sk_backward_cu_budget if backward else 0
        if backward:
            ops.grad_written = set()

    merge_weight_grads = True
    _defer_ok = True
    _flush_at_buckets = False

    def next_seed(self):
        self.seed_counter += 1
        return (0x5DEECE66D * self.seed_counter + 0xB) & 0xFFFFFFFFFFFF

    seq_per_clip_ok = False

    def _memories(self, frames, regions, training, seed, sv):
        raise NotImplementedError

    def _engine_backward(self, sv, dlogits_tm, dobj, dmot, dalpha_tm, training, seed, on_bucket=None, seq_per_clip=1):
        raise NotImplementedError

    def _public(self, x, proposals, alpha):
        return x, 0, 0, 0

    def _check_seq_per_clip(self, seq_per_clip, clips, captions):
        n = int(seq_per_clip)
        if n != 1 and not self.seq_per_clip_ok:
            raise ValueError('seq_per_clip > 1 (several captions per clip on one encoder pass) is implemented for CapGnnModel '
                             'only, not for %s' % type(self).__name__)
        if n < 1:
            raise ValueError('seq_per_clip must be >= 1, not %r' % (seq_per_clip,))
        if captions is not None and captions.shape[0] != n * clips:
            raise ValueError('%d caption rows for %d clips with seq_per_clip = %d: expected %d (rows b*n .. b*n+n-1 belong to clip b)'
                             % (captions.shape[0], clips, n, n * clips))
        return n

    def _encoder_pass(self, frames, regions, training, seed, sv, n=1):
        ops = self.ops
        self._gemm_policy(False)
        if getattr(ops, 'colsum_defer', None) is not None:
            ops.colsum_defer = None
        frames = frames.contiguous().float()
        regions = regions.contiguous().float()
        props = self._memories(frames, regions, training, seed, sv)
        sv['frames'], sv['regions'], sv['enc_out'] = frames, regions, props
        mems = props
        if n != 1:
            mems = [torch.empty((x.shape[0] * n,) + tuple(x.shape[1:]), dtype=torch.float32, device=x.device) for x in props]
            for x, y in zip(props, mems):
                ops.rows_repeat(x, y, n)
        sv['dec_gsrc'] = list(mems)
        return props, mems

    def _engine_forward(self, frames, regions, captions, L, coins, training, seed, sv, dev_coins=None, outputs=True, seq_per_clip=1):
        n = self._check_seq_per_clip(seq_per_clip, frames.shape[0], captions)
        props, mems = self._encoder_pass(frames, regions, training, seed, sv, n)
        s = E.dec_fwd(self.ops, self.decoder, list(mems), sv, captions, L, coins, training, seed, dev_coins)
        if not outputs:
            return None
        logits, alpha = E.dec_outputs(self.ops, s, alpha=self.decoder.multi_modal)
        return logits, props[0], props[-1], alpha

    @torch.no_grad()
    def _greedy_ids(self, frames, regions, seed, L=None):
        L = self.decoder.max_words if L is None else L
        sv = {}
        self._engine_forward(frames, regions, None, L, [False] * L, False, seed, sv)
        return sv['dec']['IDS'][1:].t().contiguous(), sv['enc_out']

    def forward(self, visual_feats, region_feats, caption, max_words=None, teacher_forcing_ratio=1.0, seq_per_clip=1):
        n = self._check_seq_per_clip(seq_per_clip, visual_feats.shape[0], caption)
        self.flatten_parameters_()
        dec = self.decoder
        infer = caption is None
        L = dec.max_words if max_words is None else max_words
        if infer and n != 1:
            raise ValueError('seq_per_clip > 1 needs captions; for several decoded captions per clip use sample() or beam_search()')
        if infer and dec.beam_size != 1:
            from .beam import beam_infer
            return beam_infer(self, visual_feats, region_feats)
        coins = self._draw_coins(L, infer, teacher_forcing_ratio)
        seed = self.next_seed()
        if infer:
            ids, props = self._greedy_ids(visual_feats, region_feats, seed, L)
            return self._public(ids, props, [])
        params = [p for _, p in self.named_parameters()]
        if torch.is_grad_enabled() and any(p.requires_grad for p in params):
            out = _ModelFn.apply(self, visual_feats, region_feats, caption, L, coins, seed, n, *params)
        else:
            with torch.no_grad():
                out = self._engine_forward(visual_feats, region_feats, caption, L, coins, self.training, seed, {}, seq_per_clip=n)
        return self._public(out[0], out[1:3], out[3])

    def sample(self, visual_feats, region_feats, n=1, temperature=1.0, seed=None, share_encoder=False, top_k=0, top_p=1.0,
               min_len=0, no_repeat_ngram=0, return_kept=False):
        raise NotImplementedError('sampled decoding (self-critical training) is implemented for CapGnnModel only')

    def beam_search(self, visual_feats, region_feats, beam_size=None, n_best=None, length_penalty=0.0, no_repeat_ngram=0, min_len=0,
                    num_groups=1, diversity_penalty=0.0):
        from .beam import beam_search
        return beam_search(self, visual_feats, region_feats, beam_size, n_best=n_best, length_penalty=length_penalty,
                           no_repeat_ngram=no_repeat_ngram, min_len=min_len, num_groups=num_groups, diversity_penalty=diversity_penalty)

    def sample_without_replacement(self, visual_feats, region_feats, n=5, temperature=1.0, seed=None, min_len=0, no_repeat_ngram=0,
                                   return_threshold=False):
        from .beam import stochastic_nbest
        return stochastic_nbest(self, visual_feats, region_feats, n=n, temperature=temperature, seed=seed, min_len=min_len,
                                no_repeat_ngram=no_repeat_ngram, return_threshold=return_threshold)

    def constrained_beam_search(self, visual_feats, region_feats, constraints, beam_size=None, n_best=None, length_penalty=0.0,
                                no_repeat_ngram=0, min_len=0, return_met=False):
        from .beam import constrained_nbest
        return constrained_nbest(self, visual_feats, region_feats, constraints, n_best=n_best, length_penalty=length_penalty,
                                 no_repeat_ngram=no_repeat_ngram, min_len=min_len, beam_size=beam_size, return_met=return_met)

    def _draw_coins(self, L, infer, tf_ratio):
        if infer:
            return [False] * L
        return [self.rng.random() < tf_ratio for _ in range(L)]


class _ModelFn(torch.autograd.Function):
    @staticmethod
    def forward(ctx, model, frames, regions, captions, L, coins, seed, seq_per_clip, *params):
        sv = {}
        training = model.training
        outs = model._engine_forward(frames, regions, captions, L, coins, training, seed, sv, seq_per_clip=seq_per_clip)
        ctx.model, ctx.sv, ctx.seed, ctx.training, ctx.seq_per_clip = model, sv, seed, training, seq_per_clip
        ctx.nparams = len(params)
        return outs

    @staticmethod
    def backward(ctx, dlogits, dobj, dmot, dalpha):
        model, ops = ctx.model, ctx.model.ops
        Bn, L, V = dlogits.shape
        dl_tm = torch.empty(L, Bn, V, dtype=torch.float32, device=dlogits.device)
        ops.permute_tb(dlogits.contiguous(), dl_tm)
        da_tm = None
        if dalpha is not None and dalpha.numel() > 0:
            da_tm = torch.empty(L, Bn, dalpha.shape[-1], dtype=torch.float32, device=dlogits.device)
            ops.permute_tb(dalpha.contiguous(), da_tm)
        model._engine_backward(ctx.sv, dl_tm, dobj, dmot, da_tm, ctx.training, ctx.seed, seq_per_clip=ctx.seq_per_clip)
        G = model.grad_views()
        grads = []
        for name, p in model.named_parameters():
            grads.append(G[name].clone() if (name not in model.unused_parameters and p.requires_grad) else None)
        ctx.sv = None
        return (None,) * 8 + tuple(grads)


class CapGnnModel(_HipModel):

    @property
    def unused_parameters(self):
        names = ['encoder.obj_encoder.att_l2l_norm.weight', 'encoder.obj_encoder.att_l2l_norm.bias',
                 'encoder.motion_encoder.att_l2l_norm.weight', 'encoder.motion_encoder.att_l2l_norm.bias',
                 'decoder.context_layernorm.weight', 'decoder.context_layernorm.bias']
        if not self.encoder.obj_encoder.has_obj:
            for e in ('obj_encoder', 'motion_encoder'):
                names += ['encoder.%s.obj_visual_norm.1.weight' % e, 'encoder.%s.obj_visual_norm.1.bias' % e]
        return frozenset(names)

    seq_per_clip_ok = True

    def __init__(self, args, vocab):
        super().__init__()
        self.check_kernel_limits(args, args.num_proposals, 'num_proposals')
        self.use_visual_gan = args.use_visual_gan
        self.encoder = CapGnnEncoder(args)
        self.decoder = Decoder(args, vocab, multi_modal=True)

    def update_beam_size(self, beam_size):
        self.decoder.update_beam_size(beam_size)

    def load_encoder(self, model, model_path):
        if model_path is not None:
            model.load_state_dict(torch.load(model_path, map_location=next(self.parameters()).device))
        self.encoder = model.encoder
        self.decoder.word_embed = model.decoder.word_embed
        for param in self.decoder.word_embed.parameters():
            param.requires_grad = False
        self._flat = None

    def _encode(self, frames, regions, training, seed, sv):
        ops, enc = self.ops, self.encoder
        B, T, F = frames.shape
        A = enc.a_feature_size
        f2 = frames.view(B * T, F)
        pre, extra = {}, []
        oe = enc.obj_encoder
        if oe.use_embed:
            pre['encoder.obj_encoder'] = torch.empty(B * T, oe.visual_embed.weight.shape[0], dtype=torch.float32, device=frames.device)
            extra.append((f2[:, :A], oe.visual_embed.weight, pre['encoder.obj_encoder'], oe.visual_embed.bias))
        mot_in = E.encvis_fwd(ops, enc.motion_pre_encoder, 'encoder.motion_pre_encoder', f2, B, T, sv, training, seed, extra=extra)
        E.tun_frames_multi(ops, [(enc.obj_encoder, 'encoder.obj_encoder', f2[:, :A]), (enc.motion_encoder, 'encoder.motion_encoder', mot_in)],
                           regions, sv, pre)
        ys = [None, None]
        if regions.shape[2] >= 5 and enc.obj_encoder.obj_embed.weight.shape == enc.motion_encoder.obj_embed.weight.shape:
            ys = E.region_projections(ops, [enc.obj_encoder, enc.motion_encoder], regions)
        E.tun_graph(ops, [(enc.obj_encoder, 'encoder.obj_encoder', ys[0]), (enc.motion_encoder, 'encoder.motion_encoder', ys[1])],
                    regions, sv, self.fused_o2v)
        obj, mot = E.tun_latent_multi(ops, [(enc.obj_encoder, 'encoder.obj_encoder', E.SITE_PSL_OBJ),
                                            (enc.motion_encoder, 'encoder.motion_encoder', E.SITE_PSL_MOT)], regions, sv, training, seed)
        return obj, mot

    def _memories(self, frames, regions, training, seed, sv):
        return list(self._encode(frames, regions, training, seed, sv))

    def _public(self, x, proposals, alpha):
        return x, proposals[0], proposals[-1], alpha

    def _engine_backward(self, sv, dlogits_tm, dobj, dmot, dalpha_tm, training, seed, on_bucket=None, seq_per_clip=1):
        ops, enc = self.ops, self.encoder
        n = int(seq_per_clip)
        self._gemm_policy(True)
        G = self._G
        ops.fill(self._gflat, 0.0)
        if self.merge_weight_grads and self._defer_ok:
            sv['tn_defer'] = []
        collect = hasattr(ops, 'colsum_flush')
        if collect:
            ops.colsum_defer = []
        frames, regions = sv['frames'], sv['regions']
        B, T, F = frames.shape
        H = self.decoder.visual_hidden_size
        dmems, dgfeat = E.dec_bwd(ops, self.decoder, sv, G, dlogits_tm, seed, training, dalpha_tm)

        def bucket(key):
            if on_bucket:
                if self._flush_at_buckets:
                    if sv.get('tn_defer'):
                        E.tn_grouped(ops, sv['tn_defer'])
                        sv['tn_defer'] = []
                    if collect:
                        ops.colsum_flush(keep_collecting=True)
                on_bucket(key)
        bucket('decoder')
        dob, dmo = dmems
        if n == 1:
            ops.mean_rows_bwd(dgfeat[:, :H], dob, accum=True)
            ops.mean_rows_bwd(dgfeat[:, H:], dmo, accum=True)
        else:
            folded = []
            for i, dm in enumerate(dmems):
                dx = torch.empty((B,) + tuple(dm.shape[1:]), dtype=torch.float32, device=dm.device)
                ops.clip_fold(dm, dgfeat[:, i * H:(i + 1) * H], dx, n)
                folded.append(dx)
            dob, dmo = folded
        if dobj is not None:
            ops.copy2d(dobj.reshape(-1, H), dob.view(-1, H), accum=True)
        if dmot is not None:
            ops.copy2d(dmot.reshape(-1, H), dmo.view(-1, H), accum=True)
        f2 = frames.view(B * T, F)
        deep = []
        mot, obj = (enc.motion_encoder, 'encoder.motion_encoder'), (enc.obj_encoder, 'encoder.obj_encoder')
        E.tun_bwd_head_multi(ops, [(mot[0], mot[1], dmo), (obj[0], obj[1], dob)], regions, sv, G, training, seed)
        E.tun_graph_bwd(ops, [mot, obj], regions, sv, G)
        dmot_in = E.tun_bwd_tail(ops, mot[0], mot[1], regions, sv, G, defer_dw=deep)
        E.encvis_bwd(ops, enc.motion_pre_encoder, 'encoder.motion_pre_encoder', f2, B, T, sv, G, dmot_in, training, seed)
        bucket('encoder.motion_pre_encoder')
        E.tun_bwd_tail(ops, obj[0], obj[1], regions, sv, G, defer_dw=deep)
        if on_bucket and self._flush_at_buckets and len(deep) == 2:
            bucket(('encoder.motion_encoder:rest', 'encoder.obj_encoder:rest'))
            for item, (_, pfx) in zip(deep, (mot, obj)):
                E.gemm_tn_deep(ops, [item], frames)
                on_bucket(pfx + ':obj_embed.weight')
            if collect:
                ops.colsum_flush()
            return
        E.gemm_tn_deep(ops, deep, frames)
        if 'tn_defer' in sv:
            E.tn_grouped(ops, sv.pop('tn_defer'))
        if collect:
            ops.colsum_flush()
        if on_bucket:
            on_bucket(('encoder.motion_encoder', 'encoder.obj_encoder'))

    @torch.no_grad()
    def sample(self, visual_feats, region_feats, n=1, temperature=1.0, seed=None, share_encoder=False, top_k=0, top_p=1.0,
               min_len=0, no_repeat_ngram=0, return_kept=False):
        L = self.decoder.max_words
        filtered = E.check_sample_options(L, top_k, top_p, min_len, no_repeat_ngram, self.decoder.vocab_size)
        if return_kept and not filtered:
            raise ValueError('return_kept needs one of top_k, top_p, min_len, no_repeat_ngram switched on')
        self.flatten_parameters_()
        if seed is None:
            seed = self.next_seed()
        if not share_encoder:
            visual_feats, region_feats, n = expand_rows(visual_feats, n), expand_rows(region_feats, n), 1
        sv = {}
        _, mems = self._encoder_pass(visual_feats, region_feats, self.training, seed, sv, int(n))
        s = E.dec_sample(self.ops, self.decoder, list(mems), sv, L, self.training, seed, temperature, top_k=top_k, top_p=top_p,
                         min_len=min_len, no_repeat_ngram=no_repeat_ngram)
        out = s['IDS'][1:].t().contiguous(), s['LOGP'].t().contiguous(), s['LENS']
        return out + (s['KEPT'].t().contiguous(),) if return_kept else out


class CapBaseline1(_HipModel):
    unused_parameters = frozenset(['decoder.context_layernorm.weight', 'decoder.context_layernorm.bias'])

    def __init__(self, args, vocab):
        super().__init__()
        self.check_kernel_limits(args, args.max_frames, 'max_frames (baseline decoders attend over the frame nodes)')
        self.use_visual_gan = args.use_visual_gan
        self.encoder = EncoderVisual(args, baseline=True)
        self.decoder = Decoder(args, vocab, multi_modal=False, baseline=True)

    def update_beam_size(self, beam_size):
        self.decoder.update_beam_size(beam_size)

    def _memories(self, frames, regions, training, seed, sv):
        B, T, F = frames.shape
        enc = E.encvis_fwd(self.ops, self.encoder, 'encoder', frames.view(B * T, F), B, T, sv, training, seed)
        return [enc.view(B, T, -1)]

    def _engine_backward(self, sv, dlogits_tm, dobj, dmot, dalpha_tm, training, seed, on_bucket=None, seq_per_clip=1):
        ops = self.ops
        self._gemm_policy(True)
        G = self._G
        ops.fill(self._gflat, 0.0)
        frames = sv['frames']
        B, T, F = frames.shape
        dmems, dgfeat = E.dec_bwd(ops, self.decoder, sv, G, dlogits_tm, seed, training, None)
        denc = dmems[0]
        ops.mean_rows_bwd(dgfeat, denc, accum=True)
        E.encvis_bwd(ops, self.encoder, 'encoder', frames.view(B * T, F), B, T, sv, G, denc.view(B * T, -1), training, seed)
        if on_bucket:
            on_bucket(('decoder', 'encoder'))


class CapBaselineModel(_HipModel):

    @property
    def unused_parameters(self):
        names = ['decoder.context_layernorm.weight', 'decoder.context_layernorm.bias', 'linear_baseline.weight',
                 'linear_baseline.bias']
        for n, _ in self.encoder.obj_encoder.named_parameters():
            names.append('encoder.obj_encoder.' + n)
        me = 'encoder.motion_encoder.'
        names += [me + 'att_l2l_norm.weight', me + 'att_l2l_norm.bias', me + 'v2l_layer.theta',
                  me + 'v2l_layer.out_norm.1.weight', me + 'v2l_layer.out_norm.1.bias']
        if not self.encoder.motion_encoder.has_obj:
            names += [me + 'obj_visual_norm.1.weight', me + 'obj_visual_norm.1.bias']
        return frozenset(names)

    def __init__(self, args, vocab):
        super().__init__()
        self.check_kernel_limits(args, args.max_frames, 'max_frames (baseline decoders attend over the frame nodes)')
        self.use_visual_gan = args.use_visual_gan
        self.encoder = CapGnnEncoder(args, baseline=True)
        self.linear_baseline = nn.Linear(args.visual_hidden_size * 2, args.visual_hidden_size)
        self.decoder = Decoder(args, vocab, multi_modal=False, baseline=True)

    def update_beam_size(self, beam_size):
        self.decoder.update_beam_size(beam_size)

    def _memories(self, frames, regions, training, seed, sv):
        ops, enc = self.ops, self.encoder
        B, T, F = frames.shape
        f2 = frames.view(B * T, F)
        mot_in = E.encvis_fwd(ops, enc.motion_pre_encoder, 'encoder.motion_pre_encoder', f2, B, T, sv, training, seed)
        mot = E.tun_fwd(ops, enc.motion_encoder, 'encoder.motion_encoder', mot_in, regions, sv, training, seed,
                        E.SITE_PSL_MOT, self.fused_o2v)
        return [mot.view(B, T, -1)]

    def _engine_backward(self, sv, dlogits_tm, dobj, dmot, dalpha_tm, training, seed, on_bucket=None, seq_per_clip=1):
        ops, enc = self.ops, self.encoder
        self._gemm_policy(True)
        G = self._G
        ops.fill(self._gflat, 0.0)
        frames, regions = sv['frames'], sv['regions']
        B, T, F = frames.shape
        dmems, dgfeat = E.dec_bwd(ops, self.decoder, sv, G, dlogits_tm, seed, training, None)
        dmo = dmems[0]
        ops.mean_rows_bwd(dgfeat, dmo, accum=True)
        dmot_in = E.tun_bwd(ops, enc.motion_encoder, 'encoder.motion_encoder', regions, sv, G, dmo, training, seed)
        E.encvis_bwd(ops, enc.motion_pre_encoder, 'encoder.motion_pre_encoder', frames.view(B * T, F), B, T, sv, G, dmot_in,
                     training, seed)
        if on_bucket:
            on_bucket(('decoder', 'linear_baseline', 'encoder.obj_encoder', 'encoder.motion_pre_encoder', 'encoder.motion_encoder'))


def _h2d(values, dtype, device):
    from .hip import host_to_device
    return host_to_device(values, dtype, device)


def _copy_h2d(dst, values):
    from .hip import copy_to_device
    copy_to_device(dst, values)


def ss_epsilon(epoch, ss_factor=20):
    return max(0.6, ss_factor / (ss_factor + math.exp(epoch / ss_factor)))


def multistep_lr(epoch, base_lr=1.6e-4, milestones=(4, 7), gamma=0.5):
    return base_lr * gamma ** sum(1 for m in milestones if epoch >= m)


class Trainer(object):

    def __init__(self, model, lr=1.6e-4, betas=(0.5, 0.9), eps=1e-8, process_group=None, world_size=1, use_graphs=False,
                 device_coins=None, graph_fallback=False, comm='auto', check_every=100, rehearse_ranks=0, max_grad_norm=None,
                 clip_grad_value=None, label_smoothing=0.0, teacher=None, distill_weight=0.0):
        assert comm in ('auto', 'rccl', 'torch'), comm
        eps_ls, alpha = float(label_smoothing), float(distill_weight)
        if not 0.0 <= eps_ls < 1.0:
            raise ValueError('label_smoothing must be in [0, 1), not %r' % (label_smoothing,))
        if not 0.0 <= alpha <= 1.0:
            raise ValueError('distill_weight must be in [0, 1], not %r' % (distill_weight,))
        if (alpha > 0.0) != (teacher is not None):
            raise ValueError('distill_weight > 0 needs a teacher, and a teacher needs distill_weight > 0 (got %r, %s)'
                             % (distill_weight, 'a teacher' if teacher is not None else 'no teacher'))
        if teacher is not None:
            from .ensemble import Ensemble, _device
            if not isinstance(teacher, Ensemble):
                teacher = Ensemble([teacher])
            if any(m is model for m in teacher.members):
                raise ValueError('the trained model is a member of its own teacher: distil from a copy (copy.deepcopy)')
            v0, v = model.decoder.vocab, teacher.decoder.vocab
            if len(v0) != len(v) or v0.word2idx != v.word2idx or v0.idx2word != v.idx2word:
                raise ValueError("the teacher's vocabulary differs from the model's")
            if _device(teacher.members[0]) != _device(model):
                raise ValueError('the teacher is on %s, the model on %s' % (_device(teacher.members[0]), _device(model)))
        self.label_smoothing, self.teacher, self.distill_weight = eps_ls, teacher, alpha
        self._soft = eps_ls > 0.0 or teacher is not None
        self._teacher_flats = []
        self.last_loss_parts = None
        if max_grad_norm is not None and clip_grad_value is not None:
            raise ValueError('max_grad_norm and clip_grad_value exclude each other: set at most one')
        if max_grad_norm is not None and not float(max_grad_norm) >= 0.0:
            raise ValueError('max_grad_norm must be >= 0, not %r' % (max_grad_norm,))
        if clip_grad_value is not None and not (0.0 < float(clip_grad_value) < float('inf')):
            raise ValueError('clip_grad_value must be a positive finite number, not %r' % (clip_grad_value,))
        self.max_grad_norm = None if max_grad_norm is None else float(max_grad_norm)
        self.clip_grad_value = None if clip_grad_value is None else float(clip_grad_value)
        self._clip = max_grad_norm is not None or clip_grad_value is not None
        self._clip_slots = self._clip_rec = self._skipped = None
        self.last_grad_norm = self.skipped_steps = None
        self.comm = comm
        self.check_every = check_every
        self._rccl = None
        self._comm_stream = None
        self._comm_pending = False
        self.model = model
        self.lr, self.betas, self.eps = lr, betas, eps
        self.t = 0
        self.world_size = world_size
        self.pg = process_group
        self.use_graphs = use_graphs
        self.device_coins = use_graphs if device_coins is None else device_coins
        self.graph_fallback = graph_fallback
        self.force_graph_cuts = False
        self.force_collectives = False
        self.rehearse_cotenant = None
        self.rehearse_ranks = int(rehearse_ranks)
        self._works = []
        self._graphs = None
        self._contact_checked = False
        self._hook_mode, self._hook_sv = False, None
        self._weighted_mode = False
        self._spc_mode = 1
        self.m = self.v = None
        if world_size > 1 or self.rehearse_ranks > 1:
            assert world_size == 1 or not self.rehearse_ranks, 'rehearse_ranks is for one-rank runs'
            self._use_multi_rank_schedule()
            self.force_collectives = self.force_collectives or self.rehearse_ranks > 1
        self._bind()

    COMM_CUS = 32

    def _use_multi_rank_schedule(self):
        model = self.model
        if hasattr(model.ops, 'persistent_bilstm_bwd'):
            model.ops.persistent_bilstm_bwd = False
        model.stream_k_in_backward = True
        model.sk_backward_cu_budget = 0

    def _bind(self):
        model = self.model
        model.flatten_parameters_()
        old_m, old_v = self.m, self.v
        self.m = torch.zeros_like(model._flat)
        self.v = torch.zeros_like(model._flat)
        if old_m is not None and old_m.shape == self.m.shape and old_m.device == self.m.device:
            self.m.copy_(old_m); self.v.copy_(old_v)
        self._arena = model._flat
        self._graphs = None
        self._bind_teacher()
        self._ranges = {}
        frozen = []
        for name, p in model.named_parameters():
            key = name.split('.')[0] if not name.startswith('encoder.') or not hasattr(model.encoder, 'obj_encoder') \
                else '.'.join(name.split('.')[:2])
            o = model._offsets[name]
            end = o + (p.numel() + _ALIGN - 1) // _ALIGN * _ALIGN
            lo, hi = self._ranges.get(key, (o, end))
            self._ranges[key] = (min(lo, o), max(hi, end))
            if not p.requires_grad:
                frozen.append((o, end))
            if name.endswith('_encoder.obj_embed.weight') and key != name:
                self._ranges[key + ':obj_embed.weight'] = (o, end)
        for key in [k for k in self._ranges if k.endswith(':obj_embed.weight')]:
            mod = key[:-len(':obj_embed.weight')]
            (wlo, whi), (mlo, mhi) = self._ranges[key], self._ranges[mod]
            if wlo == mlo:
                self._ranges[mod + ':rest'] = (whi, mhi)
            else:
                del self._ranges[key]
        self._frozen = tuple(frozen)
        self._train_ranges = self._minus_frozen(0, model._flat.numel())
        if self._clip:
            dev = model._flat.device
            slots = abi.defines['DLSG_GRAD_SUMSQ_SLOTS'] * max(1, len(self._train_ranges))
            if self._clip_slots is None or self._clip_slots.numel() != slots or self._clip_slots.device != dev:
                self._clip_slots = torch.zeros(slots, dtype=torch.float64, device=dev)
            if self._clip_rec is None or self._clip_rec.device != dev:
                self._clip_rec = torch.zeros(abi.defines['DLSG_CLIP_RECORD_FLOATS'], dtype=torch.float32, device=dev)
                old = self._skipped
                self._skipped = torch.zeros(1, dtype=torch.int64, device=dev)
                if old is not None:
                    self._skipped.copy_(old)
                self.last_grad_norm = self._clip_rec[abi.defines['DLSG_CLIP_NORM']]
                self.skipped_steps = self._skipped[0]

    def _minus_frozen(self, lo, hi):
        out, cur = [], lo
        for a, b in self._frozen:
            if b <= lo or a >= hi:
                continue
            if a > cur:
                out.append((cur, a))
            cur = max(cur, b)
        if cur < hi:
            out.append((cur, hi))
        return out

    def _bind_teacher(self):
        if self.teacher is not None:
            for m in self.teacher.members:
                m.flatten_parameters_()
            self._teacher_flats = [(m, m._flat) for m in self.teacher.members]

    def _check_binding(self):
        model = self.model
        model.flatten_parameters_()
        if self.teacher is not None:
            for m in self.teacher.members:
                m.flatten_parameters_()
            if any(m._flat is not flat for m, flat in self._teacher_flats):
                self._graphs = None
                self._bind_teacher()
        frozen = tuple((model._offsets[n], model._offsets[n] + (p.numel() + _ALIGN - 1) // _ALIGN * _ALIGN)
                       for n, p in model.named_parameters() if not p.requires_grad)
        if self._arena is not model._flat or frozen != self._frozen:
            self._bind()

    def _clip_grads(self):
        if not self._clip:
            return
        model, ops = self.model, self.model.ops
        n = abi.defines['DLSG_GRAD_SUMSQ_SLOTS']
        for i, (lo, hi) in enumerate(self._train_ranges):
            ops.grad_sumsq(model._gflat[lo:hi], self._clip_slots[i * n:(i + 1) * n])
        ops.clip_coef(self._clip_slots, 1.0 / self.world_size, float('inf') if self.max_grad_norm is None else self.max_grad_norm,
                      self._clip_rec, self._skipped)

    def _adam(self, step, hyper=None, ranges=None):
        model, ops = self.model, self.model.ops
        for lo, hi in (self._train_ranges if ranges is None else ranges):
            if self._clip:
                ops.adam_clipped(model._flat[lo:hi], model._gflat[lo:hi], self.m[lo:hi], self.v[lo:hi], self.lr, self.betas[0],
                                 self.betas[1], self.eps, step, 1.0 / self.world_size, hyper=hyper, record=self._clip_rec,
                                 clip_value=self.clip_grad_value or 0.0)
                continue
            ops.adam(model._flat[lo:hi], model._gflat[lo:hi], self.m[lo:hi], self.v[lo:hi], self.lr, self.betas[0],
                     self.betas[1], self.eps, step, 1.0 / self.world_size, hyper=hyper)

    def optimizer_state_dict(self):
        model = self.model
        state = {}
        names = [n for n, _ in model.named_parameters()]
        for i, (name, p) in enumerate(model.named_parameters()):
            if name in model.unused_parameters or not p.requires_grad or self.t == 0:
                continue
            o = model._offsets[name]
            state[i] = {'step': torch.tensor(float(self.t)),
                        'exp_avg': self.m[o:o + p.numel()].view(p.shape).clone(),
                        'exp_avg_sq': self.v[o:o + p.numel()].view(p.shape).clone()}
        group = {'lr': self.lr, 'betas': tuple(self.betas), 'eps': self.eps, 'weight_decay': 0, 'amsgrad': False,
                 'maximize': False, 'foreach': None, 'capturable': False, 'differentiable': False, 'fused': None,
                 'decoupled_weight_decay': False, 'params': list(range(len(names)))}
        return {'state': state, 'param_groups': [group]}

    def load_optimizer_state_dict(self, sd):
        model = self.model
        model.flatten_parameters_()
        self.m.zero_()
        self.v.zero_()
        steps = set()
        for i, (name, p) in enumerate(model.named_parameters()):
            st = sd['state'].get(i, sd['state'].get(str(i)))
            if st is None:
                continue
            o = model._offsets[name]
            self.m[o:o + p.numel()].view(p.shape).copy_(st['exp_avg'])
            self.v[o:o + p.numel()].view(p.shape).copy_(st['exp_avg_sq'])
            steps.add(int(float(st['step'])))
        if len(steps) > 1:
            raise ValueError('per-parameter step counts differ (%s): not a state this trainer can resume' % sorted(steps))
# ... 30 lines not shown
        import torch.distributed as dist
        dev = self.model._flat.device
        side = self._side_stream()
        t = torch.full((4096,), float(rank), dtype=torch.float32, device=dev)
        ev = torch.cuda.Event()
        ev.record()
        side.wait_event(ev)
        self._rccl.allreduce([t], side)
        side.synchronize()
        want = self.world_size * (self.world_size - 1) / 2.0
        ok = bool((t == want).all().item())
        every = [None] * self.world_size
        dist.all_gather_object(every, (rank, ok, float(t[0].item())), group=self.pg)
        bad = [(r, v) for r, o, v in every if not o]
        if bad:
            raise RuntimeError('RCCL first-contact check failed: the all-reduced rank pattern should be %g everywhere; wrong on ranks %s'
                               % (want, ', '.join('%d (got %g)' % rv for rv in bad)))

    def _side_stream(self):
        if self._comm_stream is None:
            self._comm_stream = torch.cuda.Stream(device=self.model._flat.device)
        return self._comm_stream

    def _allreduce(self, key):
        mode = self._comm_mode()
        ranges = [r for k in (key if isinstance(key, tuple) else (key,)) for r in self._minus_frozen(*self._ranges[k])]
        views = [self.model._gflat[lo:hi] for lo, hi in ranges]
        if mode == 'torch':
            import torch.distributed as dist
            for v in views:
                self._works.append(dist.all_reduce(v, group=self.pg, async_op=True))
            return
        if mode == 'none':
            return
        comm = self._rccl_comm()
        side = self._side_stream()
        ev = torch.cuda.Event()
        ev.record()
        side.wait_event(ev)
        comm.allreduce(views, side)
        if self.rehearse_cotenant and self.world_size == 1:
            co = self.rehearse_cotenant
            with torch.cuda.stream(side):
                for v in views:
                    self.model.ops.comm_rehearsal(v, int(co.get('workgroups', self.COMM_CUS)), int(co['passes']))
        self._comm_pending = True

    def _reduce_guard(self):
        mode = self._comm_mode()
        if mode == 'none':
            return
        mk = getattr(self.model.ops, 'guard_word', None)
        if mk is None:
            return
        word = mk(self.model._flat.device)
        if mode == 'torch':
            import torch.distributed as dist
            self._works.append(dist.all_reduce(word, op=dist.ReduceOp.MAX, group=self.pg, async_op=True))
            return
        comm = self._rccl_comm()
        side = self._side_stream()
        ev = torch.cuda.Event()
        ev.record()
        side.wait_event(ev)
        comm.allreduce_max_word(word, side)
        self._comm_pending = True

    def _join_comm(self):
        if self._comm_pending:
            ev = torch.cuda.Event()
            ev.record(self._comm_stream)
            torch.cuda.current_stream().wait_event(ev)
            self._comm_pending = False

    def collectives_info(self):
        mode = self._comm_mode()
        info = {'mode': {'none': 'none (one rank)', 'rccl': 'RCCL through the C ABI (dlsg_allreduce_bucket), side stream',
                         'torch': 'torch.distributed all_reduce(async_op=True) issued by the host'}[mode],
                'where': None if mode == 'none' else ('inside the step\'s hipGraph' if (mode == 'rccl' and self.use_graphs and
                                                      self._graphs is not None and len(self._graphs) == 1)
                                                     else ('between hipGraph segments' if self.use_graphs and self._graphs is not None
                                                           else 'between eager launches')),
                'graph_replays_per_step': len(self._graphs) if (self.use_graphs and self._graphs is not None) else 0,
                'buckets_MB': {k: round(4e-6 * sum(hi - lo for lo, hi in self._minus_frozen(*r)), 1) for k, r in self._ranges.items()}}
        if self._rccl is not None:
            info['rccl_version'] = self._rccl.rccl_version
        return info

    def check(self):
        ops = self.model.ops
        chk = getattr(ops, 'check_persistent', None)
        if chk is None:
            return
        w = ops.persist_word_or_none()
        code = int(w.item()) if w is not None else 0
        if self._rccl is not None:
            ae = self._rccl.async_error()
            if ae:
                import sys
                sys.stderr.write('dlsg_amd.Trainer: RCCL reports asynchronous error %d on this rank (ncclCommGetAsyncError)\n' % ae)
                code = code or 100 + ae
        if self.world_size > 1:
            from .comm import _agree_min
            code = _agree_min(code, self.pg, negate=True)
        if code:
            self._graphs = None
            if code >= 100:
                raise RuntimeError('RCCL asynchronous error %d on at least one rank (ncclCommGetAsyncError): the gradient exchange '
                                   'of the steps since the last check is not to be trusted' % (code - 100))
            if w is not None and int(w.item()) == 0:
                w.fill_(code)
            chk(code=code)

    def close(self):
        self.check()
        if self._rccl is not None:
            torch.cuda.synchronize()
            self._rccl.close()
            self._rccl = None

    def _schedule(self, frames, regions, captions, cap_lens, coins, seed, dev_coins, on_bucket, extra_dlogits=None, seq_weights=None,
                  seq_per_clip=1):
        model, ops = self.model, self.model.ops
        L = captions.shape[1]
        sv = {}
        training = model.training
        model._flush_at_buckets = self._comm_mode() != 'none' or self.force_graph_cuts
        teachers = ()
        if self.teacher is not None:
            teachers = self.teacher.teacher_logits(frames, regions, captions, seq_per_clip=seq_per_clip)
        model._engine_forward(frames, regions, captions, L, coins, training, seed, sv, dev_coins, outputs=False, seq_per_clip=seq_per_clip)
        s = sv['dec']
        Bn = captions.shape[0]
        dl = torch.empty_like(s['LOGITS'])
        row_loss = torch.empty((3 if self._soft else 1) * L * Bn, dtype=torch.float32, device=dl.device)
        loss = torch.empty(3 if self._soft else 1, dtype=torch.float32, device=dl.device)
        if self._soft:
            from .ensemble import MODES
            ops.ce_ragged_soft(s['LOGITS'], captions, cap_lens, dl, row_loss, loss, time_major=True, smoothing=self.label_smoothing,
                               weights=seq_weights, teachers=teachers,
                               teacher_weights=self.teacher.weights if teachers else None,
                               mode=MODES[self.teacher.mode] if teachers else 0, alpha=self.distill_weight)
            self.last_loss_parts = loss
            loss = loss[0:1]
        elif seq_weights is None:
            ops.ce_ragged(s['LOGITS'], captions, cap_lens, dl, row_loss, loss, time_major=True)
        else:
            ops.ce_ragged_weighted(s['LOGITS'], captions, cap_lens, seq_weights, dl, row_loss, loss, time_major=True)
        if extra_dlogits is not None:
            sv['loss_dev'] = loss
            g = extra_dlogits(s['LOGITS'], sv)
            V = dl.shape[-1]
            ops.copy2d(g.contiguous().view(-1, V), dl.view(-1, V), accum=True)
        model._engine_backward(sv, dl, None, None, None, training, seed, on_bucket=on_bucket, seq_per_clip=seq_per_clip)
        return loss

    def _hyper(self):
        b1, b2 = self.betas
        return [self.lr / (1.0 - b1 ** self.t), math.sqrt(1.0 - b2 ** self.t)]

    @torch.no_grad()
    def step(self, frames, regions, captions, cap_lens, tf_ratio, max_len=26, extra_dlogits=None, seed=None, seq_weights=None,
             seq_per_clip=1):
        model, ops = self.model, self.model.ops
        n_seq = model._check_seq_per_clip(seq_per_clip, frames.shape[0], captions)
        self._check_binding()
        captions = captions[:, :max_len].contiguous()
        if not (torch.is_tensor(cap_lens) and cap_lens.device == captions.device and cap_lens.dtype == torch.int64):
            cap_lens = _h2d(cap_lens, torch.int64, captions.device)
        L = captions.shape[1]
        coins = model._draw_coins(L, False, tf_ratio)
        seed = model.next_seed() if seed is None else int(seed)
        self.t += 1
        hook = extra_dlogits is not None
        weighted = seq_weights is not None
        if weighted and not (torch.is_tensor(seq_weights) and seq_weights.device == captions.device
                             and seq_weights.dtype == torch.float32):
            seq_weights = _h2d(seq_weights, torch.float32, captions.device)
        if self.use_graphs and (self._graphs is None or (self._hook_mode == hook and self._weighted_mode == weighted
                                                         and self._spc_mode == n_seq)):
            loss = self._step_graphs(frames, regions, captions, cap_lens, coins, seed, extra_dlogits, seq_weights, n_seq)
        else:
            loss = self._eager_step(frames, regions, captions, cap_lens, coins, seed, counted=True, extra_dlogits=extra_dlogits,
                                    seq_weights=seq_weights, seq_per_clip=n_seq)
        if self.check_every and self.t % self.check_every == 0:
            self.check()
        return loss

    def _eager_step(self, frames, regions, captions, cap_lens, coins, seed, counted=False, extra_dlogits=None, seq_weights=None,
                    seq_per_clip=1):
        model, ops = self.model, self.model.ops
        if not counted:
            self.t += 1
        dev_coins = None
        if self.device_coins:
            dev_coins = _h2d([int(c) for c in coins], torch.int32, captions.device)
        self._works = []
        loss = self._schedule(frames, regions, captions, cap_lens, coins, seed, dev_coins, self._allreduce, extra_dlogits, seq_weights,
                              seq_per_clip)
        self._reduce_guard()
        for w in self._works:
            w.wait()
        self._join_comm()
        if not self._clip and not self._soft:
            self._adam(self.t)
            return loss
        hyper = _h2d(self._hyper(), torch.float32, captions.device)
        self._clip_grads()
        self._adam(self.t, hyper=hyper)
        return loss

    def _capture(self, frames, regions, captions, cap_lens, hook=False, weighted=False, seq_per_clip=1):
        dev = frames.device
        L = captions.shape[1]
        self._hook_mode, self._hook_sv = hook, None
        self._weighted_mode = weighted
        self._spc_mode = seq_per_clip
        st = self._static = dict(frames=frames.clone(), regions=regions.clone(), captions=captions.clone(),
                                 lens=cap_lens.clone())
        st['weights'] = torch.ones(captions.shape[0], dtype=torch.float32, device=dev) if weighted else None
        Lp = (L + 1) // 2 * 2
        st['scalars'] = torch.zeros(Lp + 4, dtype=torch.int32, device=dev)
        st['coins'] = st['scalars'][:L]
        st['coins'].fill_(1)
        st['seed'] = st['scalars'][Lp:Lp + 2].view(torch.int64)
        st['hyper'] = st['scalars'][Lp + 2:Lp + 4].view(torch.float32)
        mode = self._comm_mode()
        cuts = mode == 'torch' or self.force_graph_cuts
        if mode == 'rccl':
            self._rccl_comm()

        def warmup():
            self._schedule(st['frames'], st['regions'], st['captions'], st['lens'], None, st['seed'], st['coins'],
                           self._allreduce if mode == 'rccl' else None, seq_weights=st['weights'], seq_per_clip=seq_per_clip)
            if mode == 'rccl':
                self._reduce_guard()
            self._join_comm()
            if self._comm_stream is not None:
                self._comm_stream.synchronize()

        def body(hard_cut):
            def cut(key):
                if mode != 'torch':
                    self._allreduce(key)
                    if cuts:
                        self._join_comm()
                if cuts:
                    hard_cut(key if mode == 'torch' else None)

            def placeholder(logits, sv):
                def alloc():
                    st['extra'] = torch.zeros_like(logits)
                hard_cut('hook', alloc)
                self._hook_sv = (logits, sv)
                return st['extra']

            loss = self._schedule(st['frames'], st['regions'], st['captions'], st['lens'], None, st['seed'], st['coins'], cut,
                                  placeholder if hook else None, st['weights'], seq_per_clip)
            if mode != 'torch':
                self._reduce_guard()
                self._join_comm()
                self._clip_grads()
                self._adam(1, hyper=st['hyper'])
            return loss

        try:
            graphs, loss = capture_segments(dev, body, warmup)
        except BaseException:
            self._graphs = None
            self._comm_pending = False
            raise
        self._graphs, self._loss = graphs, loss
        st['parts'] = self.last_loss_parts
        self._adam_in_graph = mode != 'torch'

    def _capture_agreed(self, frames, regions, captions, cap_lens, hook, weighted=False, seq_per_clip=1):
        err = None
        try:
            self._capture(frames, regions, captions, cap_lens, hook, weighted, seq_per_clip)
        except Exception as e:
            err = e
        if self.world_size > 1:
            from .comm import _agree_min
            if _agree_min(0 if err is not None else 1, self.pg) == 0 and err is None:
                err = RuntimeError('hipGraph capture failed on another rank')
                self._graphs = None
        return err

    @torch.no_grad()
    def forward_only(self, frames, regions, captions, tf_ratio, max_len=26, time_major=False, seq_per_clip=1):
        if not (self.use_graphs and self._graphs is not None and self._hook_mode and self._hook_sv is not None
                and self.model.training and self._spc_mode == int(seq_per_clip)):
            return None
        st = self._static
        captions = captions[:, :max_len].contiguous()
        if (frames.shape, regions.shape, captions.shape) != (st['frames'].shape, st['regions'].shape, st['captions'].shape):
            return None
        self._check_binding()
        model = self.model
        coins = model._draw_coins(captions.shape[1], False, tf_ratio)
        seed = model.next_seed()
        for k, src in (('frames', frames), ('regions', regions), ('captions', captions)):
            stage(st[k], src)
        self._send_scalars(coins, seed, None)
        self._graphs[0][0].replay()
        logits_tm, sv = self._hook_sv
        enc_out = sv['enc_out'] if self._spc_mode != 1 else sv['dec_gsrc']
        return (logits_tm if time_major else logits_tm.transpose(0, 1)), enc_out[0], enc_out[1], \
# ... 72 lines not shown
```

include/dlsg.h:

```cpp
#ifndef DLSG_H
#define DLSG_H
#include <stdint.h>
#ifdef __cplusplus
extern "C" {
#endif

#define DLSG_ABI_VERSION 8
int dlsg_abi_version(void);

#define DLSG_OK 0
#define DLSG_EINVAL (-1)
#define DLSG_ELAUNCH (-2)
#define DLSG_EALIGN (-3)
#define DLSG_ENOCOMM (-4)
int dlsg_struct_size(int which);

#define DLSG_GEMM_NT 0
#define DLSG_GEMM_NN 1
#define DLSG_GEMM_TN 2
#define DLSG_GEMM_MAXG 16
#define DLSG_GEMM_ACCUM 1
#define DLSG_GEMM_BIAS 2
#define DLSG_GEMM_TANH 4
#define DLSG_GEMM_FORCE64 256
// ... 129 lines not shown
    const float* adj; const float* ov; const float* theta;
    float* dov; float* dtheta_part; float* part;
    int32_t B, T, P, H;
    float p; uint32_t site;
    uint64_t seed; const uint64_t* seed_ptr;
} dlsg_latent_psl_bwd_args;
int dlsg_latent_psl_bwd(const dlsg_latent_psl_bwd_args* a, void* stream);
int dlsg_latent_psl_bwd_multi(const dlsg_latent_psl_bwd_args* a, int count, void* stream);

typedef struct {
    const float* K; const float* Q; const float* V; const float* mask;
    float* w; float* out;
    int32_t B, T, D; float scale;
} dlsg_sa_core_args;
int dlsg_sa_core_fwd(const dlsg_sa_core_args* a, void* stream);
typedef struct {
    const float* w; const float* K; const float* Q; const float* V; const float* dout;
    float* dK; float* dQ; float* dV;
    int32_t B, T, D; float scale;
} dlsg_sa_core_bwd_args;
int dlsg_sa_core_bwd(const dlsg_sa_core_bwd_args* a, void* stream);

int dlsg_softmax_fwd(const float* x, const float* mask, float* y, int64_t outer, int n, int inner, void* stream);
int dlsg_softmax_bwd(const float* y, const float* dy, float* dx, int64_t outer, int n, int inner, void* stream);

typedef struct {
    const float* Kp[2]; const float* Vp[2];
    const float* q; int64_t ldq;
    float* c[2]; int64_t ldc;
    float* alpha;
    int32_t B, P, Q, H, nstream;
    float scale;
} dlsg_decatt_args;
int dlsg_decatt_fwd(const dlsg_decatt_args* a, void* stream);
typedef struct {
    dlsg_decatt_args f;
    const float* dc[2]; int64_t lddc;
    const float* dalpha;
    float* dKp[2]; float* dVp[2];
    float* dq; int64_t lddq; int32_t accum_dq;
} dlsg_decatt_bwd_args;
int dlsg_decatt_bwd(const dlsg_decatt_bwd_args* a, void* stream);

typedef struct {
    const float* slabs; int32_t nslab; int32_t pad_; int64_t slab_stride;
    const float* addend; int64_t ldadd;
    const float* b_ih; const float* b_hh;
    const float* c_prev;
    float* c; float* h; float* gates;
    const float* lnq_g; const float* lnq_b;
    float* qcur; float* st_q;
    float p_q; uint32_t site_q;
    const float* Kp[2]; const float* Vp[2];
    const float* lnc_g[2]; const float* lnc_b[2];
    float* cpre[2]; float* ctx[2]; float* st_c[2];
    float* alpha;
    float p_att[2]; uint32_t site_att[2];
    int32_t B, Q, H, P, nstream;
    float scale, eps;
    int32_t kv_div;
    uint64_t seed; const uint64_t* seed_ptr;
    int32_t sched;
} dlsg_dec_mid_args;
int dlsg_dec_mid_fwd(const dlsg_dec_mid_args* a, void* stream);
typedef struct {
    const float* slabs; int32_t nslab; int32_t pad_; int64_t slab_stride;
    const float* b_ih; const float* b_hh;
    const float* c_prev; float* c; float* hd; float* gates;
    const float* ln_g; const float* ln_b;
    float* dout; float* st_l;
    float p; uint32_t site;
    int32_t B, D;
    float eps;
    uint64_t seed; const uint64_t* seed_ptr;
    const int32_t* s_coins; int32_t s_t; int32_t s_V;
    const float* s_W; const float* s_b;
    const float* s_E; int32_t s_Wd; uint32_t s_site;
    int64_t* s_ids; float* s_we; int64_t s_ldwe;
    int64_t s_row0; float s_p; float pad2_;
    int32_t* s_ws; int32_t s_split; int32_t pad3_;
} dlsg_dec_tail_args;
#define DLSG_DEC_TAIL_MAX_SPLIT 8
#define DLSG_DEC_TAIL_WS_WORDS 32
int dlsg_dec_tail_fwd(const dlsg_dec_tail_args* a, void* stream);
int dlsg_dec_tail_split(int32_t B, int32_t cus);
typedef struct {
    const float* slabs; int32_t nslab; int32_t write_rec; int64_t slab_stride;
    float* dlh_rec;
    const float* cpre[2]; const float* st_c[2]; const float* lnc_g[2];
    float* part_c[2];
    float* dcpre[2];
    float p_att[2]; uint32_t site_att[2];
    const float* Kp[2]; const float* Vp[2];
    const float* alpha; const float* dalpha;
    float* ds;
    const float* qh; const float* st_q; const float* lnq_g;
    float* part_q;
    float p_q; uint32_t site_q;
    const float* rec_slabs; int32_t rec_nslab; int32_t pad_; int64_t rec_slab_stride; int64_t rec_ld;
    const float* gates; const float* c; const float* c_prev;
    float* dc;
    float* dgates;
    int32_t B, Q, H, D, P, nstream;
    float scale; float pad2_;
    uint64_t seed; const uint64_t* seed_ptr;
    int32_t sched;
} dlsg_dec_mid_bwd_args;
int dlsg_dec_mid_bwd(const dlsg_dec_mid_bwd_args* a, void* stream);
typedef struct {
    const float* alpha; const float* ds;
    const float* qcur;
    const float* dcpre[2];
    float* dKp[2]; float* dVp[2];
    int32_t L, B, Q, H, P, nstream;
} dlsg_decatt_cache_grads_args;
int dlsg_decatt_cache_grads(const dlsg_decatt_cache_grads_args* a, void* stream);

typedef struct {
    const float* slabs; int32_t nslab; int32_t pad_; int64_t slab_stride;
    const float* addend; int64_t ldadd;
    const float* b_ih; const float* b_hh;
    const float* c_prev; int64_t ldcp;
    float* c; int64_t ldc_;
    float* h; int64_t ldh;
    float* h2; int64_t ldh2;
    float* gates; int64_t ldg;
    int32_t B, H;
    float p; uint32_t site; uint64_t seed;
    const uint64_t* seed_ptr;
} dlsg_lstm_pw_args;
int dlsg_lstm_pw_fwd(const dlsg_lstm_pw_args* a, void* stream);
int dlsg_lstm_pw_fwd_n(const dlsg_lstm_pw_args* a, int count, void* stream);
typedef struct {
    const float* gates; int64_t ldg;
    const float* c; int64_t ldc_;
    const float* c_prev; int64_t ldcp;
    const float* dh; int64_t lddh;
    const float* dh2; int64_t lddh2;
    const float* dh3; int64_t lddh3;
    const float* dh4; int64_t lddh4;
    int32_t dh4_nslab; int32_t pad4_; int64_t dh4_slab_stride;
    const float* dc_next; int64_t lddcn;
    float* dgates; int64_t lddg;
    float* dc_prev; int64_t lddcp;
    int32_t B, H;
    float p; uint32_t site; uint64_t seed;
    const uint64_t* seed_ptr;
} dlsg_lstm_pw_bwd_args;
int dlsg_lstm_pw_bwd(const dlsg_lstm_pw_bwd_args* a, void* stream);
int dlsg_lstm_pw_bwd_n(const dlsg_lstm_pw_bwd_args* a, int count, void* stream);

int dlsg_mean_rows_fwd(const float* x, float* out, int64_t ldo, int B, int P, int H, void* stream);
int dlsg_mean_rows_bwd(const float* dout, int64_t lddo, float* dx, int B, int P, int H, int accum, void* stream);
int dlsg_rows_repeat(const float* x, float* y, int B, int n, int64_t row, void* stream);
int dlsg_clip_fold(const float* dmem, const float* dg, int64_t lddg, float* dx, int B, int n, int P, int H, int accum, void* stream);
int dlsg_embed_fwd(const float* E, const int64_t* ids, float* out, int64_t ldo, int rows, int W, float p, uint64_t seed,
                   uint32_t site, int64_t row0, const uint64_t* seed_ptr, void* stream);
int dlsg_embed_bwd(const float* dout, int64_t lddo, const int64_t* ids, float* dE, int rows, int W, float p,
                   uint64_t seed, uint32_t site, int64_t row0, const uint64_t* seed_ptr, void* stream);
int dlsg_select_embed(const float* logits, int64_t ld, int V, const int64_t* captions, int L, int t, const int32_t* coins,
                      const float* E, int64_t* ids_out, float* out, int64_t ldo, int rows, int W, float p, uint64_t seed,
                      uint32_t site, int64_t row0, const uint64_t* seed_ptr, int prefilled, void* stream);
int dlsg_argmax(const float* logits, int64_t ld, int64_t* ids, int rows, int V, void* stream);
int dlsg_sample_embed(const float* logits, int64_t ld, int V, float temperature, const float* E, int64_t* ids_out, float* out,
                      int64_t ldo, int W, float* logp, int64_t* lens, int t, int64_t end_id, int rows, float p, uint64_t seed,
                      uint32_t site_word, uint32_t site_sample, int64_t row0, const uint64_t* seed_ptr, void* stream);
#define DLSG_SAMPLE_FILTER_MAXV 32768
int dlsg_sample_filter_embed(const float* logits, int64_t ld, int V, float temperature, const float* E, int64_t* ids_out, float* out,
                             int64_t ldo, int W, float* logp, int64_t* lens, int t, int64_t end_id, int rows, float p, uint64_t seed,
                             uint32_t site_word, uint32_t site_sample, int64_t row0, const uint64_t* seed_ptr, int top_k, float top_p,
                             int min_len, int no_repeat_ngram, const int64_t* hist, int64_t hist_stride, int32_t* kept, void* stream);
int dlsg_copy2d(const float* src, int64_t lds, float* dst, int64_t ldd, int rows, int n, int accum, void* stream);
int dlsg_dropout(const float* x, int64_t ldx, float* y, int64_t ldy, int rows, int n, float p, uint64_t seed,
                 uint32_t site, const uint64_t* seed_ptr, void* stream);
int dlsg_fill(float* dst, int64_t n, float value, void* stream);
int dlsg_gather_rows(const float* src, int64_t lds, const int64_t* idx, float* dst, int64_t ldd, int rows, int n, void* stream);
int dlsg_permute_tb(const float* src, float* dst, int T, int B, int n, void* stream);

#define DLSG_CRIT_C 512
#define DLSG_CRIT_LMAX 32
#define DLSG_CRIT_TMAX 8

int dlsg_crit_embed_mix(const float* proj_tm, const int64_t* ids, const float* W, const float* bias, const float* eps, float* h,
                        int ng, int B, int L, int V, void* stream);
int dlsg_crit_embed_mix_bwd(const float* ch, const float* eps, float* dhr, float* dhf_tm, int ng, int B, int L, void* stream);
int dlsg_crit_vocab_scatter(const float* dhr, const int64_t* ids, float* dW, int rows, int V, void* stream);

int dlsg_crit_relu_taps(const float* x, const float* ref, const float* bias, float bias_scale, float* y, float* taps, int n, int L,
                        void* stream);
int dlsg_crit_relu_taps_bwd(const float* dy, const float* dtaps, const float* ref, float* dx, int n, int L, void* stream);

#define DLSG_CLN_MAXG 4
typedef struct {
    const float* x[DLSG_CLN_MAXG]; const float* gamma[DLSG_CLN_MAXG]; const float* beta[DLSG_CLN_MAXG];
    float* y[DLSG_CLN_MAXG];
    const float* dy[3][DLSG_CLN_MAXG]; float* dx[DLSG_CLN_MAXG];
    float* dgamma[DLSG_CLN_MAXG]; float* dbeta[DLSG_CLN_MAXG]; const float* extra[DLSG_CLN_MAXG];
    const float* U[DLSG_CLN_MAXG]; float* gx[DLSG_CLN_MAXG]; float* gdy[DLSG_CLN_MAXG]; float* gpart[DLSG_CLN_MAXG];
    float* ws;
    int32_t rows, N, groups, pre_tanh, ndy, acc_lo, acc_hi;
    int32_t defer;
    float eps, p_pre, p_post; uint32_t site_pre, site_post, pad2_;
    uint64_t seed; const uint64_t* seed_ptr; int64_t row0;
} dlsg_cln_args;
int64_t dlsg_cln_ws_floats(int rows, int N);
int dlsg_cln_fwd(const dlsg_cln_args* a, void* stream);
int dlsg_cln_bwd(const dlsg_cln_args* a, void* stream);
int dlsg_cln_bwd2(const dlsg_cln_args* a, void* stream);

typedef struct {
    const float* KQV; const float* smask; float* w; float* ctx;
    const float* dctx; float* dKQV;
    const float* U; float* Uctx; float* gKQV;
    int32_t n, B, L, acc_lo, acc_hi, pad_;
    float scale, pad2_;
} dlsg_crit_sa_args;
int dlsg_crit_sa_fwd(const dlsg_crit_sa_args* a, void* stream);
int dlsg_crit_sa_bwd(const dlsg_crit_sa_args* a, void* stream);
int dlsg_crit_sa_bwd2(const dlsg_crit_sa_args* a, void* stream);

typedef struct {
    const float* a[2]; const float* e[2]; const float* smask;
    float* P[2]; float* wgt[2]; float* aggpre[2];
    const float* d_agg[2]; const float* d_wgt[2]; float* da[2]; float* de[2];
    const float* Ua[2]; float* Uagg[2]; float* Uwgt[2]; float* ga[2]; float* ge[2];
    int32_t n, B, L, T, acc_lo, acc_hi;
    float scale, pad_;
} dlsg_crit_pattn_args;
int dlsg_crit_pattn_fwd(const dlsg_crit_pattn_args* a, void* stream);
int dlsg_crit_pattn_bwd(const dlsg_crit_pattn_args* a, void* stream);
int dlsg_crit_pattn_bwd2(const dlsg_crit_pattn_args* a, void* stream);

typedef struct {
    const float* words; const float* theta; const float* gamma; const float* beta; const float* fusion;
    float* adj; float* u; float* sent; float* fus;
    const float* d_fus; float* dwords; float* part;
    const float* U; float* Ufus; float* gwords; float* gpart;
    int32_t n, L, acc_lo, acc_hi;
    float eps, p; uint32_t site, pad_;
    uint64_t seed; const uint64_t* seed_ptr; int64_t row0;
} dlsg_crit_tsum_args;
int dlsg_crit_tsum_fwd(const dlsg_crit_tsum_args* a, void* stream);
int dlsg_crit_tsum_bwd(const dlsg_crit_tsum_args* a, void* stream);
int dlsg_crit_tsum_bwd2(const dlsg_crit_tsum_args* a, void* stream);

typedef struct {
    const float* v[2]; const float* s[2]; const float* wc[2]; const float* bc[2]; const float* wgt[2]; const float* fus;
    float* pair[2]; float* score[2]; float* both; float* out;
    const float* d_out; float* d_fus; float* c_spre[2]; float* c_vpre[2]; float* d_wgt[2]; float* part_wc[2]; float* dbc;
    const float* Uspre[2]; const float* Uwgt[2]; const float* Ufus;
    float* scratch;
    int32_t n, B, T, ng, acc_lo, acc_hi;
} dlsg_crit_score_args;
int dlsg_crit_score_fwd(const dlsg_crit_score_args* a, void* stream);
int dlsg_crit_score_bwd(const dlsg_crit_score_args* a, void* stream);
int dlsg_crit_score_bwd2(const dlsg_crit_score_args* a, void* stream);

int dlsg_crit_gp(const float* g, const float* gG, const float* out, float* stats, float* vseed, float* gsc, float* q, int B, int L,
                 void* stream);

int dlsg_crit_topk(const float* alpha, int64_t sa, int64_t lda, int na, const float* smask, int64_t* idx, int B, int L, int P, int T,
                   void* stream);
int dlsg_crit_unselect(const float* src, const int64_t* idx, float* dst, int rows_src, int rows_dst, int per, int n, void* stream);

#define DLSG_CRIT_REDUCE_MAX 16
typedef struct {
    const float* src; int64_t stride; int64_t n; int32_t nslab; float scale;
    float* out;
} dlsg_crit_reduce_desc;
int dlsg_crit_reduce(const dlsg_crit_reduce_desc* d, int count, void* stream);

#define DLSG_CRIT_COLSUM_MAX 48
typedef struct {
    const float* part; int64_t ld; int32_t rows, n;
    const float* part_b; int64_t ld_b; int32_t rows_b, pad_;
    float* out; float* out_b;
    float scale, pad2_;
} dlsg_crit_colsum_desc;
int dlsg_crit_colsum(const dlsg_crit_colsum_desc* d, int count, void* stream);

int dlsg_ce_ragged(const float* logits, const int64_t* targets, const int64_t* lens, float* dlogits, float* row_loss,
                   float* loss, int B, int L, int V, int time_major, void* stream);
int dlsg_ce_ragged_weighted(const float* logits, const int64_t* targets, const int64_t* lens, const float* weights, float* dlogits,
                            float* row_loss, float* loss, int B, int L, int V, int time_major, void* stream);
int dlsg_ce_ragged_soft(const float* logits, const int64_t* targets, const int64_t* lens, const float* weights, float* dlogits,
                        float* row_loss, float* loss, int B, int L, int V, int time_major, float smoothing, float alpha,
                        const float* const* teacher, const int64_t* teacher_ld, const float* w, const float* logw, int M, int mode,
                        void* stream);
typedef struct {
    const uint64_t* gram_keys; const double* gram_idf;
    const int64_t* clip_off; const int64_t* ref_off; const double* ref_norm; const int32_t* ref_len;
    const uint64_t* ent_keys; const double* ent_w;
    int64_t n_grams;
    double log_n, sigma;
    int32_t n_clips, vocab, n, pad_;
} dlsg_cider_tables;
int dlsg_cider_d(const int64_t* ids, int64_t ld, int rows, int L, const int32_t* clip_idx, int64_t end_id,
                 const dlsg_cider_tables* t, double* scores, void* stream);
int dlsg_scst_advantage(const double* rewards, const int64_t* lens, const double* greedy, int B, int n, float* adv, double* stats,
                        void* stream);
int dlsg_cider_consensus(const int64_t* ids, int64_t ld, int B, int n, int L, int64_t end_id,
                         const dlsg_cider_tables* t, const float* scores, double temperature,
                         double* util, double* expected, int64_t* order, void* stream);
#define DLSG_METRICS_STAGE 2048
int dlsg_caption_metrics(const int64_t* ids, int64_t ld, int rows, int L, const int32_t* clip_idx, int64_t end_id,
                         const int64_t* clip_off, const int64_t* ref_off, const uint16_t* ref_words, int n_clips, int vocab,
                         const double* weights, const double* base, double* scores, int32_t* stats, double* reward, void* stream);
int dlsg_caption_corpus(const int32_t* stats, const double* scores, const double* base, int rows, double* out, void* stream);
int dlsg_log_softmax(const float* logits, float* out, int rows, int V, void* stream);
typedef struct {
    const float* logits; int64_t ld;
    const int64_t* last; const float* last_lp;
    int64_t* pred; float* new_lp; int64_t* back; int64_t* rows;
    int32_t* ended_count;
    int32_t B, k, V, end, first, pad_;
} dlsg_beam_select_args;
int dlsg_beam_select(const dlsg_beam_select_args* a, void* stream);
int dlsg_beam_select_hist(const dlsg_beam_select_args* a, const int64_t* hist_in, int64_t* hist_out, int L, int t,
                          int no_repeat_ngram, int min_len, void* stream);
#define DLSG_ENS_MAX 8
int dlsg_beam_select_ens(const dlsg_beam_select_args* a, const float* const* logits, const int64_t* ld, const float* w,
                         const float* logw, int M, int mode, const int64_t* hist_in, int64_t* hist_out, int L, int t,
                         int no_repeat_ngram, int min_len, void* stream);
int dlsg_beam_select_groups(const dlsg_beam_select_args* a, const float* const* logits, const int64_t* ld, const float* w,
                            const float* logw, int M, int mode, const int64_t* hist_in, int64_t* hist_out, int L, int t,
                            int no_repeat_ngram, int min_len, int groups, float diversity, void* stream);
int dlsg_beam_select_gumbel(const dlsg_beam_select_args* a, const int64_t* hist_in, int64_t* hist_out, int L, int t,
                            int no_repeat_ngram, int min_len, float temperature, uint64_t seed, const uint64_t* seed_ptr,
// ... 99 lines not shown
```

Before: 5083 clips/s.

## Fold small launches and skip zero-filling gradient blocks stored first

Adds batched multi-source mean_rows forward/backward kernels, a decoder prologue kernel that fuses zeroing the state arena, writing start/caption ids and embedding lookup, and merges the dQC/dLC zero allocations. The gradient-arena zero fill is replaced by a range-fill that skips blocks the backward pass overwrites on first write, with the plan recorded on the first step and checked on later steps. The aim is fewer tiny kernel launches and less memset traffic inside the graph-replayed train step, at the cost of more complex bookkeeping and a runtime check that fails if the write order changes.

```diff
diff --git a/d-lsg-video-caption_amd/csrc/rowops.hip b/d-lsg-video-caption_amd/csrc/rowops.hip
--- a/d-lsg-video-caption_amd/csrc/rowops.hip
+++ b/d-lsg-video-caption_amd/csrc/rowops.hip
@@ -448,6 +448,31 @@
     }
 }
 
+struct MeanRowsPack { const float* src[DLSG_MEAN_ROWS_MAXMULTI]; float* dst[DLSG_MEAN_ROWS_MAXMULTI]; int64_t ld[DLSG_MEAN_ROWS_MAXMULTI];
+                      int32_t P[DLSG_MEAN_ROWS_MAXMULTI]; };
+__global__ void mean_rows_fwd_multi_kernel(const MeanRowsPack pk, int H) {
+    const int i = blockIdx.z, P = pk.P[i];
+    const int b = blockIdx.y;
+    const int h = blockIdx.x * blockDim.x + threadIdx.x;
+    if (h >= H) return;
+    const float* x = pk.src[i];
+    float s = 0.f;
+    for (int p = 0; p < P; ++p) s += x[((int64_t)b * P + p) * H + h];
+    pk.dst[i][(int64_t)b * pk.ld[i] + h] = s / P;
+}
+__global__ void mean_rows_bwd_multi_kernel(const MeanRowsPack pk, int H, int accum) {
+    const int i = blockIdx.z, P = pk.P[i];
+    const int b = blockIdx.y;
+    const int h = blockIdx.x * blockDim.x + threadIdx.x;
+    if (h >= H) return;
+    const float g = pk.src[i][(int64_t)b * pk.ld[i] + h] / P;
+    float* dx = pk.dst[i];
+    for (int p = 0; p < P; ++p) {
+        float* d = dx + ((int64_t)b * P + p) * H + h;
+        *d = accum ? *d + g : g;
+    }
+}
+
 template <bool VEC>
 __global__ __launch_bounds__(256) void rows_repeat_kernel(const float* __restrict__ x, float* __restrict__ y, int n, int64_t row,
                                                           int pieces) {
@@ -606,6 +631,43 @@
 }
 __global__ void fill_kernel(float* __restrict__ dst, int64_t n, float v) {
     for (int64_t i = (int64_t)blockIdx.x * blockDim.x + threadIdx.x; i < n; i += (int64_t)gridDim.x * blockDim.x) dst[i] = v;
+}
+
+__global__ __launch_bounds__(256) void fill_ranges_kernel(float* __restrict__ dst, const int64_t* __restrict__ tab, float v) {
+    const int64_t off = tab[2 * (int64_t)blockIdx.x], cnt = tab[2 * (int64_t)blockIdx.x + 1];
+    float* d = dst + off;
+    int64_t head = (int64_t)((16 - (reinterpret_cast<uintptr_t>(d) & 15)) & 15) >> 2;
+    if (head > cnt) head = cnt;
+    const int64_t n4 = (cnt - head) >> 2;
+    const int64_t tail0 = head + 4 * n4;
+    if ((int64_t)threadIdx.x < head) d[threadIdx.x] = v;
+    f32x4* d4 = reinterpret_cast<f32x4*>(d + head);
+    const f32x4 v4 = {v, v, v, v};
+    for (int64_t i = threadIdx.x; i < n4; i += 256) d4[i] = v4;
+    if (tail0 + threadIdx.x < cnt) d[tail0 + threadIdx.x] = v;
+}
+
+__global__ __launch_bounds__(256) void dec_prologue_kernel(float* __restrict__ zst, int64_t zn, int nrow_blocks, int64_t* __restrict__ ids,
+                                                           int L, int B, int64_t start_id, const int64_t* __restrict__ captions,
+                                                           int64_t ldc, const float* __restrict__ E, float* __restrict__ we, int W, float p,
+                                                           uint64_t seed, uint32_t site, const uint64_t* seed_ptr) {
+    if ((int)blockIdx.x >= nrow_blocks) {
+        const int64_t nb = gridDim.x - nrow_blocks, b0 = (int)blockIdx.x - nrow_blocks;
+        const int64_t n4 = zn >> 2;
+        f32x4* z4 = reinterpret_cast<f32x4*>(zst);
+        const f32x4 zero = {0.f, 0.f, 0.f, 0.f};
+        for (int64_t i = b0 * 256 + threadIdx.x; i < n4; i += nb * 256) z4[i] = zero;
+        if (b0 == 0 && 4 * n4 + threadIdx.x < zn) zst[4 * n4 + threadIdx.x] = 0.f;
+        return;
+    }
+    const int r = blockIdx.x, slot = r / B, b = r - slot * B;
+    const bool word = captions && slot >= 1 && slot < L;
+    const int64_t id = slot == 0 ? start_id : word ? captions[(int64_t)b * ldc + slot - 1] : 0;
+    if (threadIdx.x == 0) ids[r] = id;
+    if (E && (slot == 0 || word)) {
+        if (seed_ptr) seed += *seed_ptr;
+        embed_row(E, id, we, (int64_t)W, W, r, p, seed, site, (int64_t)0, 256);
+    }
 }
 
 template <bool WEIGHTED>
@@ -940,6 +1002,33 @@
     DLSG_CHECK_LAUNCH();
     return DLSG_OK;
 }
+static int mean_rows_pack(MeanRowsPack& pk, const float* const* src, float* const* dst, const int64_t* ld, const int32_t* P, int count,
+                          int B, int H) {
+    if (!src || !dst || !ld || !P || count < 1 || count > DLSG_MEAN_ROWS_MAXMULTI || B < 0 || H < 1) return DLSG_EINVAL;
+    for (int i = 0; i < count; ++i) {
+        if (!src[i] || !dst[i] || P[i] < 1) return DLSG_EINVAL;
+        pk.src[i] = src[i]; pk.dst[i] = dst[i]; pk.ld[i] = ld[i]; pk.P[i] = P[i];
+    }
+    return DLSG_OK;
+}
+extern "C" int dlsg_mean_rows_fwd_multi(const float* const* x, float* const* out, const int64_t* ldo, const int32_t* P, int count, int B,
+                                        int H, void* stream) {
+    MeanRowsPack pk;
+    if (mean_rows_pack(pk, x, out, ldo, P, count, B, H) != DLSG_OK) return DLSG_EINVAL;
+    if (B == 0) return DLSG_OK;
+    hipLaunchKernelGGL(mean_rows_fwd_multi_kernel, dim3((H + 255) / 256, B, count), dim3(256), 0, ST(stream), pk, H);
+    DLSG_CHECK_LAUNCH();
+    return DLSG_OK;
+}
+extern "C" int dlsg_mean_rows_bwd_multi(const float* const* dout, const int64_t* lddo, float* const* dx, const int32_t* P, int count,
+                                        int B, int H, int accum, void* stream) {
+    MeanRowsPack pk;
+    if (mean_rows_pack(pk, dout, dx, lddo, P, count, B, H) != DLSG_OK) return DLSG_EINVAL;
+    if (B == 0) return DLSG_OK;
+    hipLaunchKernelGGL(mean_rows_bwd_multi_kernel, dim3((H + 255) / 256, B, count), dim3(256), 0, ST(stream), pk, H, accum);
+    DLSG_CHECK_LAUNCH();
+    return DLSG_OK;
+}
 extern "C" int dlsg_rows_repeat(const float* x, float* y, int B, int n, int64_t row, void* stream) {
     if (B < 0 || n < 1 || row < 0) return DLSG_EINVAL;
     if (B == 0 || row == 0) return DLSG_OK;
@@ -1014,6 +1103,28 @@
     DLSG_CHECK_LAUNCH();
     return DLSG_OK;
 }
+extern "C" int dlsg_fill_ranges(float* dst, const int64_t* table, int nblocks, float value, void* stream) {
+    if (nblocks < 0 || (nblocks > 0 && (!dst || !table))) return DLSG_EINVAL;
+    if (nblocks == 0) return DLSG_OK;
+    hipLaunchKernelGGL(fill_ranges_kernel, dim3(nblocks), dim3(256), 0, ST(stream), dst, table, value);
+    DLSG_CHECK_LAUNCH();
+    return DLSG_OK;
+}
+extern "C" int dlsg_dec_prologue(float* zst, int64_t zst_floats, int64_t* ids, int L, int B, int64_t start_id, const int64_t* captions,
+                                 int64_t ldc, const float* E, float* we, int W, float p, uint64_t seed, uint32_t site,
+                                 const uint64_t* seed_ptr, void* stream) {
+    if (L < 1 || B < 0 || zst_floats < 0 || !ids || (zst_floats > 0 && (!zst || (reinterpret_cast<uintptr_t>(zst) & 15)))) return DLSG_EINVAL;
+    if (E && (!we || W < 1)) return DLSG_EINVAL;
+    if (B == 0) return DLSG_OK;
+    if ((int64_t)(L + 1) * B > 0x3fffffff) return DLSG_EINVAL;
+    const int rows = (L + 1) * B;
+    const int64_t want = ((zst_floats >> 2) + 1023) / 1024;
+    const int fillb = zst_floats == 0 ? 0 : (int)(want < 1 ? 1 : want > 2048 ? 2048 : want);
+    hipLaunchKernelGGL(dec_prologue_kernel, dim3(rows + fillb), dim3(256), 0, ST(stream), zst, zst_floats, rows, ids, L, B, start_id,
+                       captions, ldc, E, we, W, p, seed, site, seed_ptr);
+    DLSG_CHECK_LAUNCH();
+    return DLSG_OK;
+}
 extern "C" int dlsg_permute_tb(const float* src, float* dst, int T, int B, int n, void* stream) {
     const int64_t total = (int64_t)T * B * n;
     if (total == 0) return DLSG_OK;
diff --git a/d-lsg-video-caption_amd/dlsg_amd/engine.py b/d-lsg-video-caption_amd/dlsg_amd/engine.py
--- a/d-lsg-video-caption_amd/dlsg_amd/engine.py
+++ b/d-lsg-video-caption_amd/dlsg_amd/engine.py
@@ -72,6 +72,10 @@
 DEEP_TN_CHUNKS = 8
 
 
+def _fold(ops):
+    return bool(getattr(ops, 'fold_small_launches', False))
+
+
 def _accum_flag(ops, gout):
     seen = getattr(ops, 'grad_written', None)
     if seen is None:
@@ -80,6 +84,9 @@
     if key in seen:
         return F_ACCUM
     seen.add(key)
+    stored = getattr(ops, 'grad_stored', None)
+    if stored is not None:
+        stored.append(gout)
     return 0
 
 
@@ -810,8 +817,11 @@
         assert gfeat.shape == (B, plan.G), (tuple(gfeat.shape), (B, plan.G))
     else:
         gfeat = _empty(ref, B, plan.G)
-        for i, g in enumerate(gsrc):
-            ops.mean_rows_fwd(g, gfeat[:, i * H:(i + 1) * H])
+        if _fold(ops) and 1 < len(gsrc) <= 4:
+            ops.mean_rows_fwd_multi(list(gsrc), [gfeat[:, i * H:(i + 1) * H] for i in range(len(gsrc))])
+        else:
+            for i, g in enumerate(gsrc):
+                ops.mean_rows_fwd(g, gfeat[:, i * H:(i + 1) * H])
     Wq = dec.query_lstm.weight_ih
     gq = _empty(ref, B, 4 * Q)
     lin(ops, gfeat, Wq[:, plan.q_glob[0]:plan.q_glob[1]], gq)
@@ -875,18 +885,18 @@
         skip_if=skip_if)
 
 
-def dec_alloc(dec, s, ref, B, L):
+def dec_alloc(dec, s, ref, B, L, zero=True):
     plan = s['plan']
     H, W, Q, D, ns = plan.H, plan.W, plan.Q, plan.D, plan.ns
     V = dec.vocab_size
     P = s['Kp'][0].shape[1]
-    zst = _zeros(ref, (L + 1) * B * (2 * D + 2 * Q))
+    zst = s['ZST'] = (_zeros if zero else _empty)(ref, (L + 1) * B * (2 * D + 2 * Q))
     o = 0
     for key, wd in (('LHP', D), ('QH', Q), ('QC', Q), ('LC', D)):
         s[key] = zst[o:o + (L + 1) * B * wd].view(L + 1, B, wd)
         o += (L + 1) * B * wd
     s['WE'] = _empty(ref, L + 1, B, W)
-    s['IDS'] = _zeros(ref, L + 1, B, dtype=torch.int64)
+    s['IDS'] = (_zeros if zero else _empty)(ref, L + 1, B, dtype=torch.int64)
     s['QCUR'] = _empty(ref, L, B, Q)
     s['ST_Q'] = _empty(ref, L, B, 2)
     s['CPRE'] = [_empty(ref, L, B, H) for _ in range(ns)]
@@ -900,22 +910,32 @@
     s['LOGITS'] = _empty(ref, L, B, V)
 
 
-def dec_begin(ops, dec, mems, sv, L, training, seed):
+def dec_begin(ops, dec, mems, sv, L, training, seed, captions=None, embed=False):
     s = dec_prepare(ops, dec, mems, sv, training, seed)
     ref = mems[0]
     B = ref.shape[0]
-    dec_alloc(dec, s, ref, B, L)
-    s['IDS'][0].fill_(dec.vocab('<start>'))
+    fold = _fold(ops)
+    assert fold or not (embed or captions is not None)
+    dec_alloc(dec, s, ref, B, L, zero=not fold)
     s['pw'] = dec.p_drop if training else 0.0
+    if fold:
+        if captions is not None and captions.stride(1) != 1:
+            captions = captions.contiguous()
+        ops.dec_prologue(s['ZST'], s['IDS'], dec.vocab('<start>'), captions=captions if L > 1 else None,
+                         E=dec.word_embed.weight if embed else None, we=s['WE'], p=s['pw'], seed=seed, site=SITE_WORD)
+    else:
+        s['IDS'][0].fill_(dec.vocab('<start>'))
     return s, ref, B, dec.word_embed.weight, s['IDS'], s['pw']
 
 
 def dec_fwd(ops, dec, mems, sv, captions, L, coins, training, seed, dev_coins=None):
-    s, ref, B, E, ids, pw = dec_begin(ops, dec, mems, sv, L, training, seed)
+    fold = _fold(ops) and dev_coins is not None
+    s, ref, B, E, ids, pw = dec_begin(ops, dec, mems, sv, L, training, seed, captions=captions if fold else None, embed=fold)
     if dev_coins is not None:
-        ops.embed_fwd(E, ids[0], s['WE'][0], p=pw, seed=seed, site=SITE_WORD, row0=0)
         pre = captions is not None and L > 1
-        if pre:
+        if not fold:
+            ops.embed_fwd(E, ids[0], s['WE'][0], p=pw, seed=seed, site=SITE_WORD, row0=0)
+        if pre and not fold:
             ids[1:L].copy_(captions[:, :L - 1].t())
             ops.embed_fwd(E, ids[1:L].reshape(-1), s['WE'][1:L].view((L - 1) * B, -1), p=pw, seed=seed, site=SITE_WORD, row0=B)
         fused_sample = pre and getattr(ops, 'dec_tail_sample_supported', None) is not None and \
@@ -968,13 +988,15 @@
 
 def dec_sample(ops, dec, mems, sv, L, training, seed, temperature, top_k=0, top_p=1.0, min_len=0, no_repeat_ngram=0):
     filtered = check_sample_options(L, top_k, top_p, min_len, no_repeat_ngram, dec.vocab_size)
-    s, ref, B, E, ids, pw = dec_begin(ops, dec, mems, sv, L, training, seed)
+    fold = _fold(ops)
+    s, ref, B, E, ids, pw = dec_begin(ops, dec, mems, sv, L, training, seed, embed=fold)
     s['LOGP'] = _empty(ref, L, B)
     s['LENS'] = torch.full((B,), L, dtype=torch.int64, device=ref.device)
     if filtered:
         s['KEPT'] = torch.empty(L, B, dtype=torch.int32, device=ref.device)
     end = dec.vocab('<end>')
-    ops.embed_fwd(E, ids[0], s['WE'][0], p=pw, seed=seed, site=SITE_WORD, row0=0)
+    if not fold:
+        ops.embed_fwd(E, ids[0], s['WE'][0], p=pw, seed=seed, site=SITE_WORD, row0=0)
     for t in range(L):
         dec_step(ops, dec, s, t, ref, training, seed, B)
         dec_logits(ops, dec, s, t, t + 1)
@@ -1026,8 +1048,12 @@
 
     dGQ = _empty(ref, L, B, 4 * Q)
     dGL = _empty(ref, L, B, 4 * D)
-    dQC = _zeros(ref, B, Q)
-    dLC = _zeros(ref, B, D)
+    if _fold(ops):
+        dC = _zeros(ref, B * (Q + D))
+        dQC, dLC = dC[:B * Q].view(B, Q), dC[B * Q:].view(B, D)
+    else:
+        dQC = _zeros(ref, B, Q)
+        dLC = _zeros(ref, B, D)
     dLHrec = _empty(ref, B, D)
     P = s['Kp'][0].shape[1]
     dCPRE = [_empty(ref, L, B, H) for _ in range(ns)]
diff --git a/d-lsg-video-caption_amd/dlsg_amd/hip.py b/d-lsg-video-caption_amd/dlsg_amd/hip.py
--- a/d-lsg-video-caption_amd/dlsg_amd/hip.py
+++ b/d-lsg-video-caption_amd/dlsg_amd/hip.py
@@ -96,6 +96,7 @@
 class HipOps(object):
 
     name = 'hip'
+    fold_small_launches = True
 
     def __init__(self):
         self.lib = load_library()
@@ -927,6 +928,24 @@
         self._check(self.lib.dlsg_mean_rows_bwd(_p(dout), i64(dout.stride(0)), _p(dx), B, P, H, int(accum), self._stream()),
                     'mean_rows_bwd')
 
+    @staticmethod
+    def _mean_rows_arrays(srcs, dsts, lds, Ps):
+        n = len(srcs)
+        return ((C.c_void_p * n)(*[t.data_ptr() for t in srcs]), (C.c_void_p * n)(*[t.data_ptr() for t in dsts]),
+                (C.c_int64 * n)(*lds), (C.c_int32 * n)(*Ps), n)
+
+    def mean_rows_fwd_multi(self, xs, outs):
+        B, _, H = xs[0].shape
+        assert all(x.is_contiguous() and x.shape[0] == B and x.shape[2] == H for x in xs) and all(o.stride(1) == 1 for o in outs)
+        a = self._mean_rows_arrays(xs, outs, [o.stride(0) for o in outs], [x.shape[1] for x in xs])
+        self._check(self.lib.dlsg_mean_rows_fwd_multi(*a, B, H, self._stream()), 'mean_rows_fwd_multi')
+
+    def mean_rows_bwd_multi(self, douts, dxs, accum=False):
+        B, _, H = dxs[0].shape
+        assert all(x.is_contiguous() and x.shape[0] == B and x.shape[2] == H for x in dxs) and all(d.stride(1) == 1 for d in douts)
+        src, dst, ld, P, n = self._mean_rows_arrays(douts, dxs, [d.stride(0) for d in douts], [x.shape[1] for x in dxs])
+        self._check(self.lib.dlsg_mean_rows_bwd_multi(src, ld, dst, P, n, B, H, int(accum), self._stream()), 'mean_rows_bwd_multi')
+
     def rows_repeat(self, x, y, n):
         B = x.shape[0]
         assert x.is_contiguous() and y.is_contiguous() and y.shape[0] == B * n and y.shape[1:] == x.shape[1:], (x.shape, y.shape, n)
@@ -957,6 +976,22 @@
         sd, sp = _seed(seed)
         self._check(self.lib.dlsg_embed_bwd(_p(dout), i64(dout.stride(0)), _p(ids), _p(dE), rows, W, f32(p), u64(sd),
                                             u32(site), i64(row0), sp, self._stream()), 'embed_bwd')
+
+    def dec_prologue(self, zst, ids, start_id, captions=None, E=None, we=None, p=0.0, seed=0, site=0):
+        L1, B = ids.shape
+        assert ids.is_contiguous() and ids.dtype == torch.int64 and zst.is_contiguous() and zst.dtype == torch.float32
+        ldc = 0
+        if captions is not None:
+            assert captions.dtype == torch.int64 and captions.shape[0] == B and (L1 < 3 or (captions.shape[1] >= L1 - 2 and captions.stride(1) == 1))
+            ldc = captions.stride(0)
+        W = 0
+        if E is not None:
+            W = E.shape[1]
+            assert E.is_contiguous() and we.is_contiguous() and we.shape == (L1, B, W)
+        sd, sp = _seed(seed)
+        self._check(self.lib.dlsg_dec_prologue(_p(zst), i64(zst.numel()), _p(ids), L1 - 1, B, i64(start_id), _p(captions), i64(ldc),
+                                               _p(E), _p(we) if E is not None else None, W, f32(p), u64(sd), u32(site), sp,
+                                               self._stream()), 'dec_prologue')
 
     def argmax(self, logits, ids):
         rows, V = logits.shape
@@ -1006,6 +1041,24 @@
     def fill(self, t, value):
         assert t.is_contiguous()
         self._check(self.lib.dlsg_fill(_p(t), i64(t.numel()), f32(value), self._stream()), 'fill')
+
+    FILL_PIECE = 16384
+
+    def fill_table(self, ranges, numel, device):
+        rows = []
+        for off, cnt in ranges:
+            if not (0 <= int(off) and 0 <= int(cnt) and int(off) + int(cnt) <= int(numel)):
+                raise ValueError('fill range (%d, %d) outside a buffer of %d floats' % (off, cnt, numel))
+            for o in range(0, int(cnt), self.FILL_PIECE):
+                rows.append((int(off) + o, min(self.FILL_PIECE, int(cnt) - o)))
+        tab = host_to_device(rows, torch.int64, device) if rows else torch.empty(0, 2, dtype=torch.int64, device=device)
+        tab.fill_numel = int(numel)
+        return tab
+
+    def fill_ranges(self, t, table, value=0.0):
+        assert t.is_contiguous() and t.dtype == torch.float32 and table.dtype == torch.int64 and table.is_contiguous()
+        assert table.fill_numel <= t.numel(), (table.fill_numel, t.numel())
+        self._check(self.lib.dlsg_fill_ranges(_p(t), _p(table), table.shape[0], f32(value), self._stream()), 'fill_ranges')
 
     def crit_embed_mix(self, proj_tm, ids, W, bias, eps, h):
         ng, B, L, _ = h.shape
diff --git a/d-lsg-video-caption_amd/dlsg_amd/model.py b/d-lsg-video-caption_amd/dlsg_amd/model.py
--- a/d-lsg-video-caption_amd/dlsg_amd/model.py
+++ b/d-lsg-video-caption_amd/dlsg_amd/model.py
@@ -127,6 +127,14 @@
         ops.sk_cu_budget = self.sk_backward_cu_budget if backward else 0
         if backward:
             ops.grad_written = set()
+
+    _fill_table = None
+
+    def _zero_grads(self):
+        if self._fill_table is not None:
+            self.ops.fill_ranges(self._gflat, self._fill_table, 0.0)
+        else:
+            self.ops.fill(self._gflat, 0.0)
 
     merge_weight_grads = True
     _defer_ok = True
@@ -339,7 +347,7 @@
         n = int(seq_per_clip)
         self._gemm_policy(True)
         G = self._G
-        ops.fill(self._gflat, 0.0)
+        self._zero_grads()
         if self.merge_weight_grads and self._defer_ok:
             sv['tn_defer'] = []
         collect = hasattr(ops, 'colsum_flush')
@@ -362,8 +370,11 @@
         bucket('decoder')
         dob, dmo = dmems
         if n == 1:
-            ops.mean_rows_bwd(dgfeat[:, :H], dob, accum=True)
-            ops.mean_rows_bwd(dgfeat[:, H:], dmo, accum=True)
+            if E._fold(ops):
+                ops.mean_rows_bwd_multi([dgfeat[:, :H], dgfeat[:, H:]], [dob, dmo], accum=True)
+            else:
+                ops.mean_rows_bwd(dgfeat[:, :H], dob, accum=True)
+                ops.mean_rows_bwd(dgfeat[:, H:], dmo, accum=True)
         else:
             folded = []
             for i, dm in enumerate(dmems):
@@ -442,7 +453,7 @@
         ops = self.ops
         self._gemm_policy(True)
         G = self._G
-        ops.fill(self._gflat, 0.0)
+        self._zero_grads()
         frames = sv['frames']
         B, T, F = frames.shape
         dmems, dgfeat = E.dec_bwd(ops, self.decoder, sv, G, dlogits_tm, seed, training, None)
@@ -492,7 +503,7 @@
         ops, enc = self.ops, self.encoder
         self._gemm_policy(True)
         G = self._G
-        ops.fill(self._gflat, 0.0)
+        self._zero_grads()
         frames, regions = sv['frames'], sv['regions']
         B, T, F = frames.shape
         dmems, dgfeat = E.dec_bwd(ops, self.decoder, sv, G, dlogits_tm, seed, training, None)
@@ -503,6 +514,38 @@
                      training, seed)
         if on_bucket:
             on_bucket(('decoder', 'linear_baseline', 'encoder.obj_encoder', 'encoder.motion_pre_encoder', 'encoder.motion_encoder'))
+
+
+def _stored_spans(stored, arena):
+    base, tot, spans = arena.data_ptr(), arena.numel(), []
+    for g in stored:
+        off = (g.data_ptr() - base) // 4
+        if g.is_contiguous() and g.dtype == torch.float32 and 0 <= off and off + g.numel() <= tot and g.numel():
+            spans.append((off, g.numel()))
+    spans.sort()
+    out = []
+    for off, cnt in spans:
+        if out and off < out[-1][0] + out[-1][1]:
+            if off + cnt > out[-1][0] + out[-1][1]:
+                out[-1] = (out[-1][0], off + cnt - out[-1][0])
+            continue
+        out.append((off, cnt))
+    return out
+
+
+def _complement(spans, tot):
+    out, at = [], 0
+    for off, cnt in spans:
+        if off > at:
+            out.append((at, off - at))
+        at = off + cnt
+    if at < tot:
+        out.append((at, tot - at))
+    return out
+
+
+def _covered(spans, want):
+    return frozenset(w for w in want if any(o <= w[0] and w[0] + w[1] <= o + c for o, c in spans))
 
 
 def _h2d(values, dtype, device):
@@ -581,6 +624,7 @@
         self.rehearse_cotenant = None
         self.rehearse_ranks = int(rehearse_ranks)
         self._works = []
+        self._fill_plans = {}
         self._graphs = None
         self._contact_checked = False
         self._hook_mode, self._hook_sv = False, None
@@ -917,8 +961,39 @@
             g = extra_dlogits(s['LOGITS'], sv)
             V = dl.shape[-1]
             ops.copy2d(g.contiguous().view(-1, V), dl.view(-1, V), accum=True)
-        model._engine_backward(sv, dl, None, None, None, training, seed, on_bucket=on_bucket, seq_per_clip=seq_per_clip)
+        key = self._fill_key(frames, regions, captions, dev_coins, extra_dlogits, seq_weights, seq_per_clip)
+        if key is None:
+            model._engine_backward(sv, dl, None, None, None, training, seed, on_bucket=on_bucket, seq_per_clip=seq_per_clip)
+            return loss
+        plan = self._fill_plans.get(key)
+        ops.grad_stored = []
+        model._fill_table = plan[0] if plan else None
+        try:
+            model._engine_backward(sv, dl, None, None, None, training, seed, on_bucket=on_bucket, seq_per_clip=seq_per_clip)
+        finally:
+            stored, ops.grad_stored, model._fill_table = ops.grad_stored, None, None
+        spans = _stored_spans(stored, model._gflat)
+        if plan is None:
+            if len(self._fill_plans) >= 8:
+                self._fill_plans.clear()
+            tot = model._gflat.numel()
+            self._fill_plans[key] = (ops.fill_table(_complement(spans, tot), tot, model._gflat.device), frozenset(spans))
+        elif not plan[1] <= _covered(spans, plan[1]):
+            raise RuntimeError('Trainer: a gradient block that this form of the step stored first on its first schedule was not '
+                               'stored first now, and the arena fill had left it out -- the gradients of this step are wrong '
+                               '(set HipOps.fold_small_launches = False and report the step\'s options)')
         return loss
+
+    def _fill_key(self, frames, regions, captions, dev_coins, extra_dlogits, seq_weights, seq_per_clip):
+        model = self.model
+        ops = model.ops
+        if not E._fold(ops) or not hasattr(model, '_zero_grads') or self.world_size > 1 or self.rehearse_ranks > 1 or \
+                model._flush_at_buckets or extra_dlogits is not None or seq_weights is not None or seq_per_clip != 1 or \
+                self.teacher is not None or (self.use_graphs and self._hook_mode):
+            return None
+        return (model._gflat.data_ptr(), model._gflat.numel(), tuple(frames.shape), tuple(regions.shape), tuple(captions.shape),
+                model.training, dev_coins is None, model.gemm_precision, model.merge_weight_grads, model._defer_ok,
+                model.fused_o2v, bool(getattr(ops, 'stream_k', False)), bool(getattr(model, 'stream_k_in_backward', True)))
 
     def _hyper(self):
         b1, b2 = self.betas
diff --git a/include/dlsg.h b/include/dlsg.h
--- a/include/dlsg.h
+++ b/include/dlsg.h
@@ -305,12 +305,20 @@
 
 int dlsg_mean_rows_fwd(const float* x, float* out, int64_t ldo, int B, int P, int H, void* stream);
 int dlsg_mean_rows_bwd(const float* dout, int64_t lddo, float* dx, int B, int P, int H, int accum, void* stream);
+#define DLSG_MEAN_ROWS_MAXMULTI 4
+int dlsg_mean_rows_fwd_multi(const float* const* x, float* const* out, const int64_t* ldo, const int32_t* P, int count, int B, int H,
+                             void* stream);
+int dlsg_mean_rows_bwd_multi(const float* const* dout, const int64_t* lddo, float* const* dx, const int32_t* P, int count, int B, int H,
+                             int accum, void* stream);
 int dlsg_rows_repeat(const float* x, float* y, int B, int n, int64_t row, void* stream);
 int dlsg_clip_fold(const float* dmem, const float* dg, int64_t lddg, float* dx, int B, int n, int P, int H, int accum, void* stream);
 int dlsg_embed_fwd(const float* E, const int64_t* ids, float* out, int64_t ldo, int rows, int W, float p, uint64_t seed,
                    uint32_t site, int64_t row0, const uint64_t* seed_ptr, void* stream);
 int dlsg_embed_bwd(const float* dout, int64_t lddo, const int64_t* ids, float* dE, int rows, int W, float p,
                    uint64_t seed, uint32_t site, int64_t row0, const uint64_t* seed_ptr, void* stream);
+int dlsg_dec_prologue(float* zst, int64_t zst_floats, int64_t* ids, int L, int B, int64_t start_id, const int64_t* captions,
+                      int64_t ldc, const float* E, float* we, int W, float p, uint64_t seed, uint32_t site,
+                      const uint64_t* seed_ptr, void* stream);
 int dlsg_select_embed(const float* logits, int64_t ld, int V, const int64_t* captions, int L, int t, const int32_t* coins,
                       const float* E, int64_t* ids_out, float* out, int64_t ldo, int rows, int W, float p, uint64_t seed,
                       uint32_t site, int64_t row0, const uint64_t* seed_ptr, int prefilled, void* stream);
@@ -327,6 +335,7 @@
 int dlsg_dropout(const float* x, int64_t ldx, float* y, int64_t ldy, int rows, int n, float p, uint64_t seed,
                  uint32_t site, const uint64_t* seed_ptr, void* stream);
 int dlsg_fill(float* dst, int64_t n, float value, void* stream);
+int dlsg_fill_ranges(float* dst, const int64_t* table, int nblocks, float value, void* stream);
 int dlsg_gather_rows(const float* src, int64_t lds, const int64_t* idx, float* dst, int64_t ldd, int rows, int n, void* stream);
 int dlsg_permute_tb(const float* src, float* dst, int T, int B, int n, void* stream);
 
```

New measurement: 5108 clips/s (median of 6 runs). About the same (+0.5%).
